# debbiemarkslab/BEAR

Hardware: AMD Instinct MI355X
Metric: k-mer contexts/sec (DM-marginal+grad h), k=13 (higher is better)
Workload: dtype f64

## Files before the change

bear_amd/csrc/bear_hip.hip:

```cpp
#include "bear_host.h"
#include "kernels_finalize.h"
#include "kernels_rows.h"
#include "kernels_sorted.h"
#include "kernels_plan.h"
#include "kernels_synth.h"
#include "kernels_refmix.h"
#include "kernels_mixplan.h"
#include "kernels_sample.h"
#include "kernels_shuffle.h"
#include "kernels_refplan.h"

#ifdef PLN_STAMPS
#define PLN_DBG_ARG , ws->dbg
#else
#define PLN_DBG_ARG
#endif

thread_local int g_last_hip_error = 0;

extern "C" {

int bear_abi_version(void) { return BEAR_ABI_VERSION; }

const char *bear_strerror(int status) {
  switch (status) {
    case BEAR_OK: return "ok";
    case BEAR_ERR_INVALID_ARG: return "invalid argument (null or misaligned pointer, bad flag)";
    case BEAR_ERR_NO_DEVICE: return "no usable HIP device";
    case BEAR_ERR_WRONG_DEVICE: return "current HIP device differs from the workspace device";
    case BEAR_ERR_HIP: return "HIP runtime call failed (see bear_last_hip_error)";
    case BEAR_ERR_NOMEM: return "out of memory";
    case BEAR_ERR_IO: return "file could not be opened or read";
    case BEAR_ERR_PARSE: return "malformed count-table row";
    default: return "unknown bear status";
  }
}

int bear_last_hip_error(void) { return g_last_hip_error; }

static int dm_kernels_setup() {
  int st = allow_dynamic_lds({BEAR_KFN(dm_prior_sorted_kernel<0>), BEAR_KFN(dm_prior_sorted_kernel<1>), BEAR_KFN(dm_prior_sorted_kernel<9>)},
                             sizeof(srt_lds_n));
  if (st == BEAR_OK) st = allow_dynamic_lds({BEAR_KFN(dm_ref_sorted_kernel)}, sizeof(srt_lds_r));
  if (st == BEAR_OK)
    st = allow_dynamic_lds({BEAR_KFN(dm_prior_plan_kernel<false, false>), BEAR_KFN(dm_prior_plan_kernel<true, false>),
                            BEAR_KFN(dm_prior_plan_kernel<true, true>)},
                           sizeof(pln_lds_n));
  if (st == BEAR_OK)
    st = allow_dynamic_lds({BEAR_KFN(dm_prior_plan_grad_kernel<false, false>), BEAR_KFN(dm_prior_plan_grad_kernel<true, true>),
                            BEAR_KFN(dm_refmix_plan_grad_kernel<false>), BEAR_KFN(dm_refmix_plan_grad_kernel<true>)},
                           sizeof(pln_lds_g));
  if (st == BEAR_OK) st = allow_dynamic_lds({BEAR_KFN(dm_prior_plan_grad_inplace_kernel)}, sizeof(pln_lds_gi));
  if (st == BEAR_OK) st = allow_dynamic_lds({BEAR_KFN(dm_ref_plan_kernel<false>), BEAR_KFN(dm_ref_plan_kernel<true>)}, sizeof(pln_lds_r));
  return st;
}

static void ws_release(bear_ws *ws) {
  (void)hipFree(ws->partials);
  (void)hipFree(ws->logtab);
  (void)hipFree(ws->dbg);
  (void)hipFree(ws->eval_partials);
  (void)hipFree(ws->eval_out);
  (void)hipFree(ws->lin_partials);
  (void)hipFree(ws->linw_partials);
  (void)hipFree(ws->linw_packed);
  (void)hipFree(ws->lin_accum);
  (void)hipFree(ws->cnn_partials);
  (void)hipFree(ws->cnnw_partials);
  (void)hipFree(ws->arrive);
  delete ws;
}

static int ws_setup(bear_ws *ws) {
  HIP_TRY(hipMalloc(&ws->partials, sizeof(double) * BEAR_MAX_OUT * (size_t)ws->max_blocks));
  HIP_TRY(hipMalloc(&ws->logtab, sizeof(double) * 2 * BEAR_LOGTAB_N));
  HIP_TRY(hipMalloc(&ws->dbg, sizeof(unsigned long long) * 48 * (size_t)ws->max_blocks));
  HIP_TRY(hipMalloc(&ws->arrive, sizeof(unsigned long long) * BEAR_ARRIVE_WORDS));
  HIP_TRY(hipMemset(ws->arrive, 0, sizeof(unsigned long long) * BEAR_ARRIVE_WORDS));
  double tab[2 * BEAR_LOGTAB_N];
  for (int i = 0; i < BEAR_LOGTAB_N; ++i) {
    const double r = 1.0 / ((BEAR_LOGTAB_N + i + 0.5) / (2.0 * BEAR_LOGTAB_N));
    tab[2 * i] = r;
    tab[2 * i + 1] = -log(r);
  }
  HIP_TRY(hipMemcpy(ws->logtab, tab, sizeof(tab), hipMemcpyHostToDevice));
  int st = dm_kernels_setup();
  if (st == BEAR_OK) st = linear_ws_setup(ws);
  if (st == BEAR_OK) st = cnn_ws_setup(ws);
  if (st == BEAR_OK) st = eval_ws_setup(ws);
  return st;
}

int bear_ws_create(int device, bear_ws **out) {
  if (!out) return BEAR_ERR_INVALID_ARG;
  *out = nullptr;
  int count = 0;
  if (hipGetDeviceCount(&count) != hipSuccess || count <= 0) return BEAR_ERR_NO_DEVICE;
  if (device < 0 || device >= count) return BEAR_ERR_INVALID_ARG;
  int prev = 0;
  HIP_TRY(hipGetDevice(&prev));
  HIP_TRY(hipSetDevice(device));
  hipDeviceProp_t prop;
  const hipError_t e = hipGetDeviceProperties(&prop, device);
  bear_ws *ws = e == hipSuccess ? new (std::nothrow) bear_ws() : nullptr;
  int st = ws ? BEAR_OK : BEAR_ERR_NOMEM;
  if (e != hipSuccess) {
    g_last_hip_error = (int)e;
    st = BEAR_ERR_HIP;
  }
  if (ws) {
    ws->device = device;
    ws->num_cu = prop.multiProcessorCount;
    ws->max_blocks = ws->num_cu * 8;
    ws->eval_blocks = ws->num_cu * 8;
    st = ws_setup(ws);
    if (st != BEAR_OK) {
      ws_release(ws);
      ws = nullptr;
    }
  }
  (void)hipSetDevice(prev);
  *out = ws;
  return st;
}

int bear_ws_destroy(bear_ws *ws) {
  if (!ws) return BEAR_OK;
  int prev = 0;
  (void)hipGetDevice(&prev);
  (void)hipSetDevice(ws->device);
  ws_release(ws);
  (void)hipSetDevice(prev);
  return BEAR_OK;
}

int bear_deterministic_build(void) {
#ifdef BEAR_DET_BUILD
  return 1;
#else
  return 0;
#endif
}

static int grid_rows(const bear_ws *ws, uint64_t n_rows) { return grid_capped((n_rows + BEAR_TILE_ROWS - 1) / BEAR_TILE_ROWS, ws_blocks(ws, 2)); }
static int grid_sorted(const bear_ws *ws, uint64_t n_rows) { return grid_capped((n_rows + SRT_TILE - 1) / SRT_TILE, ws_blocks(ws, 2)); }
static int grid_dense(const bear_ws *ws, uint64_t n_rows) {
  return grid_capped((n_rows + DPR_TILE_ROWS - 1) / DPR_TILE_ROWS, ws_blocks(ws, DPR_BLOCKS_PER_CU));
}

int bear_dm_prior_f64(bear_ws *ws, const uint32_t *counts, const double *prior, uint64_t n_rows,
                      double h_signed, double eps, int train_ar, double *out, double *grad_prior,
                      void *stream) {
  int st = check_ws(ws);
  if (st != BEAR_OK) return st;
  if (!out || (n_rows && (!counts || !prior))) return BEAR_ERR_INVALID_ARG;
  if (misaligned(counts) || misaligned(prior) || misaligned(grad_prior) || misaligned8(out)) return BEAR_ERR_INVALID_ARG;
  hipStream_t s = static_cast<hipStream_t>(stream);
  const bear_params prm = params_net(h_signed, eps);
  int grid = grid_rows(ws, n_rows);
  if (!train_ar && !grad_prior) {
    grid = grid_sorted(ws, n_rows);
    const char *dbg = getenv("BEAR_DEBUG_STOP");
    const int stop = dbg ? atoi(dbg) : 0;
    const double2 *lt = reinterpret_cast<const double2 *>(ws->logtab);
    if (stop == 1)
      hipLaunchKernelGGL(dm_prior_sorted_kernel<1>, dim3(grid), dim3(SRT_THREADS), sizeof(srt_lds_n), s, counts, prior, n_rows, prm, lt, ws->partials, ws->dbg);
    else if (stop == 9)
      hipLaunchKernelGGL(dm_prior_sorted_kernel<9>, dim3(grid), dim3(SRT_THREADS), sizeof(srt_lds_n), s, counts, prior, n_rows, prm, lt, ws->partials, ws->dbg);
    else
      hipLaunchKernelGGL(dm_prior_sorted_kernel<0>, dim3(grid), dim3(SRT_THREADS), sizeof(srt_lds_n), s, counts, prior, n_rows, prm, lt, ws->partials, ws->dbg);
  } else {
#define PRIOR_LAUNCH(AR, GRAD)                                                                                                          \
  hipLaunchKernelGGL((dm_prior_kernel<AR, GRAD>), dim3(grid), dim3(BEAR_THREADS), 0, s, counts, prior, n_rows, prm, grad_prior, \
                     reinterpret_cast<const double2 *>(ws->logtab), ws->partials)
    BEAR_DISPATCH_2(train_ar, grad_prior, PRIOR_LAUNCH);
#undef PRIOR_LAUNCH
  }
  HIP_TRY(hipGetLastError());
  hipLaunchKernelGGL(finalize_kernel, dim3(1), dim3(256), 0, s, ws->partials, grid, 2, out);
  HIP_TRY(hipGetLastError());
  return BEAR_OK;
}

int bear_dm_ref_f64(bear_ws *ws, const uint32_t *train, const uint32_t *ref, uint64_t n_rows,
                    double h_signed, double tau_signed, double nu_signed, double eps, int train_ar,
                    double *out, void *stream) {
  int st = check_ws(ws);
  if (st != BEAR_OK) return st;
  if (!out || (n_rows && (!train || !ref))) return BEAR_ERR_INVALID_ARG;
  if (misaligned(train) || misaligned(ref) || misaligned8(out)) return BEAR_ERR_INVALID_ARG;
  hipStream_t s = static_cast<hipStream_t>(stream);
  const bear_params prm = params_ref(h_signed, tau_signed, nu_signed, eps);
  const double2 *lt = reinterpret_cast<const double2 *>(ws->logtab);
  int grid = grid_rows(ws, n_rows);
  if (train_ar || getenv("BEAR_ROWS_KERNEL")) {
#define REF_LAUNCH(AR) hipLaunchKernelGGL((dm_ref_kernel<AR>), dim3(grid), dim3(BEAR_THREADS), 0, s, train, ref, n_rows, prm, lt, ws->partials)
    BEAR_DISPATCH_1(train_ar, REF_LAUNCH);
#undef REF_LAUNCH
  } else {
    grid = grid_sorted(ws, n_rows);
    hipLaunchKernelGGL(dm_ref_sorted_kernel, dim3(grid), dim3(SRT_THREADS), sizeof(srt_lds_r), s, train, ref, n_rows, prm, lt, ws->partials);
  }
  HIP_TRY(hipGetLastError());
  hipLaunchKernelGGL(finalize_kernel, dim3(1), dim3(256), 0, s, ws->partials, grid, 4, out);
  HIP_TRY(hipGetLastError());
  return BEAR_OK;
}

static void plan_free(bear_plan *p) {
  if (!p) return;
  (void)hipFree(p->tiles);
  (void)hipFree(p->stream);
  (void)hipFree(p->heavy_col);
  (void)hipFree(p->heavy_row);
  (void)hipFree(p->heavy_stop);
  (void)hipFree(p->hist);
  (void)hipFree(p->live);
  for (int k = 0; k < p->n_cnn_levels; ++k) bear_level_free(&p->cnn_levels[k]);
  for (int k = 0; k <= CNN_MAX_LAG; ++k)
    for (int q = 0; q < p->n_cnn_win[k]; ++q) bear_window_free(&p->cnn_win[k][q]);
  (void)hipFree(p->live2);
  (void)hipFree(p->tiles_p);
  (void)hipFree(p->tiles_u);
  (void)hipFree(p->ref_items);
  (void)hipFree(p->hist0_base);
  (void)hipFree(p->heavy0);
  (void)hipFree(p->sum0);
  delete p;
}

int bear_plan_create(bear_ws *ws, const uint32_t *counts, uint64_t n_rows, int ncol, bear_plan **out) {
  if (!out) return BEAR_ERR_INVALID_ARG;
  *out = nullptr;
  int st = check_ws(ws);
  if (st != BEAR_OK) return st;
  if ((ncol != 4 && ncol != 5) || (n_rows && !counts) || misaligned(counts)) return BEAR_ERR_INVALID_ARG;
  bear_plan *p = new (std::nothrow) bear_plan();
  if (!p) return BEAR_ERR_NOMEM;
  memset(p, 0, sizeof(*p));
  p->device = ws->device;
  p->ncol = ncol;
  p->n_rows = n_rows;
  p->counts = counts;
  hipError_t e = hipMalloc(&p->hist, sizeof(unsigned long long) * (2 * SRT_NKEY + PLN_NBIG + 1));
  if (e == hipSuccess) e = hipMemset(p->hist, 0, sizeof(unsigned long long) * (2 * SRT_NKEY + PLN_NBIG + 1));
  if (e != hipSuccess) {
    g_last_hip_error = (int)e;
    plan_free(p);
    return BEAR_ERR_HIP;
  }
  if (n_rows == 0) {
    *out = p;
    return BEAR_OK;
  }
  const uint64_t n_quads = (n_rows + PLN_QUAD - 1) / PLN_QUAD;
  uint8_t *d_quad = nullptr, *h_quad = nullptr;
  unsigned long long *d_cnt = nullptr;
  std::vector<pln_tile> tiles;
  e = hipMalloc(&d_quad, 3 * n_quads);
  if (e == hipSuccess) e = hipMalloc(&d_cnt, sizeof(unsigned long long) * 9);
  if (e == hipSuccess) e = hipMemset(d_cnt, 0, sizeof(unsigned long long) * 9);
  if (e == hipSuccess) {
    const int grid = grid_capped((n_quads + 255) / 256, (uint64_t)ws->num_cu * 8);
    hipLaunchKernelGGL(plan_scan_kernel, dim3(grid), dim3(256), 0, 0, counts, n_rows, ncol, d_quad, d_cnt, p->hist);
    e = hipGetLastError();
  }
  unsigned long long h_cnt[3] = {0, 0, 0}, h_total[3] = {0, 0, 0};
  if (e == hipSuccess) e = hipMemcpy(h_cnt, d_cnt, sizeof(h_cnt), hipMemcpyDeviceToHost);
  if (e == hipSuccess) e = hipMemcpy(h_total, d_cnt + 6, sizeof(h_total), hipMemcpyDeviceToHost);
  for (int k = 0; k < 3; ++k) p->count_total[k] = p->count_bound[k] = (double)h_total[k];
  uint64_t off16 = 0, n_tiles = 0;
  const char *cut_env = getenv("BEAR_PLAN_CUT");
  const bool host_cut = cut_env && cut_env[0] == 'h';
  if (e == hipSuccess && host_cut) {
    h_quad = (uint8_t *)malloc(3 * n_quads);
    if (!h_quad) e = hipErrorOutOfMemory;
    if (e == hipSuccess) e = hipMemcpy(h_quad, d_quad, 3 * n_quads, hipMemcpyDeviceToHost);
  }
  if (e == hipSuccess && host_cut) {
    uint64_t q = 0;
    while (q < n_quads) {
      uint32_t items = 0, rows = 0, hcol = 0, hrow = 0;
      const uint64_t q0 = q;
      while (q < n_quads && rows + PLN_QUAD <= PLN_RMAX && items + h_quad[q] <= PLN_NI_CUT) {
        items += h_quad[q];
        hcol += h_quad[n_quads + q];
        hrow += h_quad[2 * n_quads + q];
        rows += PLN_QUAD;
        ++q;
      }
      pln_tile ti;
      memset(&ti, 0, sizeof(ti));
      ti.row0 = q0 * PLN_QUAD;
      if (ti.row0 + rows > n_rows) rows = (uint32_t)(n_rows - ti.row0);
      const uint32_t hc = hcol < PLN_HCAP ? hcol : PLN_HCAP;
      const uint32_t hr = ncol == 5 ? (hrow < PLN_HCAP ? hrow : PLN_HCAP) : 0u;
      ti.rows_items = (rows << 16) | items;
      ti.off16 = (uint32_t)off16;
      ti.hc_hr = (hc << 16) | hr;
      ti.blk16 = pln_block_layout(rows, items, hc, hr).end / 16;
      off16 += ti.blk16;
      if (off16 > 0xffffffffull) {
        e = hipErrorOutOfMemory;
        break;
      }
      tiles.push_back(ti);
    }
    n_tiles = tiles.size();
  }
  free(h_quad);
  if (e == hipSuccess && !host_cut) {
    const uint32_t chunk = plan_cut_chunk(n_quads);
    const uint64_t n_chunks = (n_quads + chunk - 1) / chunk;
    uint32_t *d_walk = nullptr;
    uint16_t *d_step = nullptr;
    uint64_t *d_entry = nullptr;
    unsigned long long *d_meta = nullptr, h_meta[3] = {0, 0, 0};
    e = hipMalloc(&d_walk, sizeof(uint32_t) * n_chunks * PLN_CUT_SPAN);
    if (e == hipSuccess) e = hipMalloc(&d_step, sizeof(uint16_t) * n_quads);
    if (e == hipSuccess) e = hipMalloc(&d_entry, sizeof(uint64_t) * 2 * n_chunks);
    if (e == hipSuccess) e = hipMalloc(&d_meta, sizeof(h_meta));
    if (e == hipSuccess) e = hipMemset(d_meta, 0, sizeof(h_meta));
    if (e == hipSuccess) {
      const uint64_t wb = (n_chunks * PLN_CUT_SPAN + 255) / 256;
      hipLaunchKernelGGL(plan_cut_step_kernel, dim3((unsigned)((n_chunks + 255) / 256)), dim3(256), 0, 0, d_quad, n_quads, n_chunks, chunk, d_step);
      hipLaunchKernelGGL(plan_cut_walk_kernel, dim3((unsigned)wb), dim3(256), 0, 0, d_step, n_quads, n_chunks, chunk, d_walk);
      hipLaunchKernelGGL(plan_cut_chain_kernel, dim3(1), dim3(1), 0, 0, d_walk, n_chunks, chunk, d_entry, d_entry + n_chunks, d_meta);
      e = hipGetLastError();
    }
    if (e == hipSuccess) e = hipMemcpy(h_meta, d_meta, sizeof(unsigned long long), hipMemcpyDeviceToHost);
    n_tiles = h_meta[0];
    if (e == hipSuccess) e = hipMalloc(&p->tiles, sizeof(pln_tile) * (n_tiles + PLN_DESC_PAD));
    if (e == hipSuccess) e = hipMemset(p->tiles, 0, sizeof(pln_tile) * (n_tiles + PLN_DESC_PAD));
    if (e == hipSuccess) {
      hipLaunchKernelGGL(plan_cut_write_kernel, dim3((unsigned)((n_chunks + 255) / 256)), dim3(256), 0, 0, d_quad, n_quads, n_rows, ncol,
                         n_chunks, chunk, d_entry, d_entry + n_chunks, p->tiles);
      hipLaunchKernelGGL(plan_cut_offsets_kernel, dim3(1), dim3(1024), 0, 0, p->tiles, n_tiles, d_meta);
      e = hipGetLastError();
    }
    if (e == hipSuccess) e = hipMemcpy(h_meta, d_meta, sizeof(h_meta), hipMemcpyDeviceToHost);
    if (e == hipSuccess && h_meta[2]) e = hipErrorOutOfMemory;
    off16 = h_meta[1];
    (void)hipFree(d_walk);
    (void)hipFree(d_step);
    (void)hipFree(d_entry);
    (void)hipFree(d_meta);
  }
  (void)hipFree(d_quad);
  p->n_tiles = n_tiles;
  const uint64_t stream_bytes = off16 * 16 + 1024;
  for (int k = 0; k < 3; ++k) p->n_heavy[k] = h_cnt[k];
  if (host_cut) {
    if (e == hipSuccess) e = hipMalloc(&p->tiles, sizeof(pln_tile) * (tiles.size() + PLN_DESC_PAD));
    if (e == hipSuccess) e = hipMemset(p->tiles, 0, sizeof(pln_tile) * (tiles.size() + PLN_DESC_PAD));
    if (e == hipSuccess) e = hipMemcpy(p->tiles, tiles.data(), sizeof(pln_tile) * tiles.size(), hipMemcpyHostToDevice);
  }
  if (e == hipSuccess) e = hipMalloc(&p->stream, stream_bytes);
  if (e == hipSuccess) e = hipMemset(p->stream, 0, stream_bytes);
  if (e == hipSuccess && h_cnt[0]) e = hipMalloc(&p->heavy_col, sizeof(pln_heavy_col) * h_cnt[0]);
  if (e == hipSuccess && h_cnt[1]) e = hipMalloc(&p->heavy_row, sizeof(pln_heavy_row) * h_cnt[1]);
  if (e == hipSuccess && h_cnt[2]) e = hipMalloc(&p->heavy_stop, sizeof(uint64_t) * h_cnt[2]);
  if (e == hipSuccess) {
    const uint64_t nt = n_tiles;
    const int grid = grid_capped(nt, (uint64_t)ws->num_cu * 2);
    hipLaunchKernelGGL(plan_fill_kernel, dim3(grid), dim3(1024), 0, 0, counts, n_rows, ncol, p->tiles, nt, p->stream,
                       p->heavy_col, p->heavy_row, p->heavy_stop, d_cnt + 3);
    e = hipGetLastError();
  }
  const uint64_t live_bytes = ncol == 5 ? sizeof(uint16_t) * PLN_LIVE_STRIDE * (n_tiles + 1) : 0;
  if (e == hipSuccess && live_bytes) e = hipMalloc(&p->live, live_bytes);
  if (e == hipSuccess && live_bytes) e = hipMemset(p->live, 0, live_bytes);
  if (e == hipSuccess && live_bytes) {
    const uint64_t nt = n_tiles;
    const int grid = grid_capped(nt, (uint64_t)ws->num_cu * 2);
    hipLaunchKernelGGL(plan_live_kernel, dim3(grid), dim3(1024), 0, 0, p->tiles, nt, p->stream, p->live);
    e = hipGetLastError();
  }
  if (e == hipSuccess) e = hipDeviceSynchronize();
  unsigned long long h_used[3] = {0, 0, 0};
  if (e == hipSuccess) e = hipMemcpy(h_used, d_cnt + 3, sizeof(h_used), hipMemcpyDeviceToHost);
  for (int k = 0; k < 3; ++k) p->n_heavy[k] = h_used[k];
#ifdef BEAR_DET_BUILD
  const uint64_t sort_from = 2;
#else
  const uint64_t sort_from = 1u << 16;
#endif
  if (e == hipSuccess) {
    int cst = h_used[0] >= sort_from ? bear_canonical_order(p->heavy_col, h_used[0], 16, 0) : BEAR_OK;
    if (cst == BEAR_OK && h_used[1] >= sort_from) cst = bear_canonical_order(p->heavy_row, h_used[1], 16, 0);
    if (cst == BEAR_OK && h_used[2] >= sort_from) cst = bear_canonical_order(p->heavy_stop, h_used[2], 8, 0);
    if (cst != BEAR_OK) e = cst == BEAR_ERR_NOMEM ? hipErrorOutOfMemory : hipErrorUnknown;
  }
  p->n_live_rows = n_rows;
  if (e == hipSuccess && ncol == 5) {
    unsigned long long h_hist[SRT_NKEY];
    e = hipMemcpy(h_hist, p->hist, sizeof(h_hist), hipMemcpyDeviceToHost);
    unsigned long long live_rows = h_cnt[1];
    for (int k = 0; k < SRT_NKEY; ++k) live_rows += h_hist[k];
    p->n_live_rows = live_rows;
  }
  (void)hipFree(d_cnt);
  if (e != hipSuccess) {
    g_last_hip_error = (int)e;
    plan_free(p);
    return e == hipErrorOutOfMemory ? BEAR_ERR_NOMEM : BEAR_ERR_HIP;
  }
  p->bytes = stream_bytes + live_bytes + sizeof(pln_tile) * n_tiles + sizeof(pln_heavy_col) * h_cnt[0] +
             sizeof(pln_heavy_row) * h_cnt[1] + sizeof(uint64_t) * h_cnt[2];
  *out = p;
  return BEAR_OK;
}

int bear_plan_destroy(bear_plan *plan) {
  if (!plan) return BEAR_OK;
  int prev = 0;
  (void)hipGetDevice(&prev);
  (void)hipSetDevice(plan->device);
  plan_free(plan);
  (void)hipSetDevice(prev);
  return BEAR_OK;
}

uint64_t bear_plan_bytes(const bear_plan *plan) { return plan ? plan->bytes : 0; }

int bear_plan_create_auto(bear_ws *ws, const uint32_t *counts, uint64_t n_rows, int *rowwise, bear_plan **out) {
  if (rowwise) *rowwise = 0;
  int st = bear_plan_create(ws, counts, n_rows, 5, out);
  if (st != BEAR_OK) return st;
  bear_plan *p = *out;
  const double cells = p->count_total[1], listed = (double)p->n_heavy[0];
  if (!(cells > 0.0) || listed * 2.0 <= cells) return BEAR_OK;
  (void)hipFree(p->tiles);
  (void)hipFree(p->stream);
  (void)hipFree(p->heavy_col);
  (void)hipFree(p->heavy_row);
  (void)hipFree(p->heavy_stop);
  (void)hipFree(p->live);
  p->tiles = nullptr;
  p->stream = nullptr;
  p->heavy_col = nullptr;
  p->heavy_row = nullptr;
  p->heavy_stop = nullptr;
  p->live = nullptr;
  p->n_tiles = 0;
  p->n_heavy[0] = p->n_heavy[1] = p->n_heavy[2] = 0;
  p->ncol = PLAN_ROWS;
  p->bytes = sizeof(unsigned long long) * (2 * SRT_NKEY + PLN_NBIG + 1);
  if (rowwise) *rowwise = 1;
  return BEAR_OK;
}
static int launch_prior_rows(bear_ws *ws, const bear_plan *plan, const double *prior, const bear_params &prm, const double *theta,
                             int train_ar, double *out, double *grad_prior, hipStream_t s) {
  const int grid = grid_dense(ws, plan->n_rows);
  const double2 *lt = reinterpret_cast<const double2 *>(ws->logtab);
  const bear_step_io io = ws_io(ws, theta, BEAR_THETA_NET, out);
#define ROWS_LAUNCH(AR, GRAD) \
  hipLaunchKernelGGL((dm_prior_rows_kernel<AR, GRAD>), dim3(grid), dim3(BEAR_THREADS), 0, s, plan->counts, prior, plan->n_rows, prm, grad_prior, lt, \
                     ws->partials, io)
  BEAR_DISPATCH_2(train_ar, grad_prior, ROWS_LAUNCH);
#undef ROWS_LAUNCH
  HIP_TRY(hipGetLastError());
  return BEAR_OK;
}

uint64_t bear_plan_tile_count(const bear_plan *plan) { return plan ? plan->n_tiles : 0; }

int bear_plan_tile_info(const bear_plan *plan, uint64_t first, uint64_t count, uint64_t *row0, uint32_t *rows, uint32_t *items,
                        uint64_t *stream_offset) {
  if (!plan || first + count > plan->n_tiles || (count && (!row0 || !rows || !items || !stream_offset))) return BEAR_ERR_INVALID_ARG;
  if (!count) return BEAR_OK;
  std::vector<pln_tile> h(count);
  int prev = 0;
  (void)hipGetDevice(&prev);
  (void)hipSetDevice(plan->device);
  const hipError_t e = hipMemcpy(h.data(), plan->tiles + first, sizeof(pln_tile) * count, hipMemcpyDeviceToHost);
  (void)hipSetDevice(prev);
  if (e != hipSuccess) {
    g_last_hip_error = (int)e;
    return BEAR_ERR_HIP;
  }
  for (uint64_t k = 0; k < count; ++k) {
    row0[k] = h[k].row0;
    rows[k] = h[k].rows_items >> 16;
    items[k] = h[k].rows_items & 0xffffu;
    stream_offset[k] = (uint64_t)h[k].off16 * 16;
  }
  return BEAR_OK;
}

int bear_plan_create_ref(bear_ws *ws, const uint32_t *train, const uint32_t *ref, uint64_t n_rows, bear_plan **out) {
  if (!out) return BEAR_ERR_INVALID_ARG;
  *out = nullptr;
  if ((n_rows && !ref) || misaligned(ref)) return BEAR_ERR_INVALID_ARG;
  bear_plan *p = nullptr;
  int st = bear_plan_create(ws, train, n_rows, 4, &p);
  if (st != BEAR_OK) return st;
  p->ref = ref;
  if (p->count_total[1] > 0.0 && (double)p->n_heavy[0] * 2.0 > p->count_total[1]) {
    (void)hipFree(p->tiles);
    (void)hipFree(p->stream);
    (void)hipFree(p->heavy_col);
    (void)hipFree(p->heavy_row);
    (void)hipFree(p->heavy_stop);
    p->tiles = nullptr;
    p->stream = nullptr;
    p->heavy_col = nullptr;
    p->heavy_row = nullptr;
    p->heavy_stop = nullptr;
    p->n_tiles = 0;
    p->n_heavy[0] = p->n_heavy[1] = p->n_heavy[2] = 0;
    p->rows_ref = 1;
    p->bytes = sizeof(unsigned long long) * (2 * SRT_NKEY + PLN_NBIG + 1);
    *out = p;
    return BEAR_OK;
  }
  unsigned long long *d_meta = nullptr;
  hipError_t e = hipMalloc(&d_meta, sizeof(unsigned long long) * 72);
  if (e == hipSuccess) e = hipMemset(d_meta, 0, sizeof(unsigned long long) * 72);
  if (e == hipSuccess) e = hipMalloc(&p->sum0, sizeof(double));
  if (e == hipSuccess) e = hipMemset(p->sum0, 0, sizeof(double));
  p->hist0_base = d_meta;
  unsigned long long h_meta[72];
  memset(h_meta, 0, sizeof(h_meta));
  const int grid = grid_capped((n_rows + 1023) / 1024, (uint64_t)ws->num_cu * 8);
  if (e == hipSuccess && n_rows) {
    hipLaunchKernelGGL(rpl_build_kernel, dim3(grid), dim3(256), 0, 0, train, ref, n_rows, 0, d_meta, d_meta + 32, d_meta + 64, p->sum0,
                       static_cast<rpl_item *>(nullptr), static_cast<uint32_t *>(nullptr));
    e = hipGetLastError();
    if (e == hipSuccess) e = hipMemcpy(h_meta, d_meta, sizeof(h_meta), hipMemcpyDeviceToHost);
  }
  if (e == hipSuccess) {
    unsigned long long run = 0, cur[RPL_NKEY];
    for (int k = 0; k < RPL_NKEY; ++k) {
      cur[k] = run;
      run += h_meta[k];
    }
    p->n_ref_items = run;
    p->n_heavy0 = h_meta[64];
    if (run) e = hipMalloc(&p->ref_items, sizeof(rpl_item) * run);
    if (e == hipSuccess && p->n_heavy0) e = hipMalloc(&p->heavy0, sizeof(uint32_t) * p->n_heavy0);
    if (e == hipSuccess) e = hipMemcpy(d_meta, cur, sizeof(cur), hipMemcpyHostToDevice);
    if (e == hipSuccess) e = hipMemset(d_meta + 64, 0, sizeof(unsigned long long));
    if (e == hipSuccess && n_rows && (run || p->n_heavy0)) {
      hipLaunchKernelGGL(rpl_build_kernel, dim3(grid), dim3(256), 0, 0, train, ref, n_rows, 1, d_meta, d_meta + 32, d_meta + 64, p->sum0,
                         p->ref_items, p->heavy0);
      e = hipGetLastError();
    }
    if (e == hipSuccess) e = hipDeviceSynchronize();
#ifdef BEAR_DET_BUILD
    for (int k = 0; k < RPL_NKEY && e == hipSuccess; ++k)
      if (bear_canonical_order(p->ref_items + cur[k], h_meta[k], 16, 0) != BEAR_OK) e = hipErrorUnknown;
    if (e == hipSuccess && bear_canonical_order(p->heavy0, p->n_heavy0, 4, 0) != BEAR_OK) e = hipErrorUnknown;
#endif
  }
  if (e != hipSuccess) {
    g_last_hip_error = (int)e;
    plan_free(p);
    return e == hipErrorOutOfMemory ? BEAR_ERR_NOMEM : BEAR_ERR_HIP;
  }
  p->hist0 = d_meta + 32;
  p->bytes += sizeof(rpl_item) * p->n_ref_items + sizeof(uint32_t) * p->n_heavy0 + sizeof(unsigned long long) * 72;
  *out = p;
  return BEAR_OK;
}

static int launch_prior_plan(bear_ws *ws, const bear_plan *plan, const double *prior, uint64_t n_rows, const bear_params &prm,
                             const double *theta, int train_ar, int prior_normalized, double *out, hipStream_t s) {
  const int grid = grid_plan(ws, plan->n_tiles);
  const double2 *lt = reinterpret_cast<const double2 *>(ws->logtab);
  const bear_step_io io = ws_io(ws, theta, BEAR_THETA_NET, out);
  if (train_ar)
    hipLaunchKernelGGL((dm_prior_plan_kernel<true, true>), dim3(grid), dim3(PLN_THREADS), sizeof(pln_lds_n), s, prior, n_rows, prm,
                       plan_view(plan), lt, ws->partials, io PLN_DBG_ARG);
  else if (prior_normalized)
    hipLaunchKernelGGL((dm_prior_plan_kernel<true, false>), dim3(grid), dim3(PLN_THREADS), sizeof(pln_lds_n), s, prior, n_rows, prm,
                       plan_view(plan), lt, ws->partials, io PLN_DBG_ARG);
  else
    hipLaunchKernelGGL((dm_prior_plan_kernel<false, false>), dim3(grid), dim3(PLN_THREADS), sizeof(pln_lds_n), s, prior, n_rows, prm,
                       plan_view(plan), lt, ws->partials, io PLN_DBG_ARG);
  HIP_TRY(hipGetLastError());
  return BEAR_OK;
}

int bear_dm_prior_plan_f64(bear_ws *ws, const bear_plan *plan, const uint32_t *counts, const double *prior,
                           uint64_t n_rows, double h_signed, double eps, int train_ar, int prior_normalized,
                           double *out, void *stream) {
  int st = check_ws(ws);
  if (st != BEAR_OK) return st;
  if (!plan || !out || (n_rows && (!counts || !prior))) return BEAR_ERR_INVALID_ARG;
  if (check_plan_step(ws, plan, counts, n_rows, 5, true) != BEAR_OK || misaligned(prior) || misaligned8(out)) return BEAR_ERR_INVALID_ARG;
  const bear_params prm = params_net(h_signed, eps);
  if (plan_is_rows(plan)) return launch_prior_rows(ws, plan, prior, prm, nullptr, train_ar, out, nullptr, static_cast<hipStream_t>(stream));
  return launch_prior_plan(ws, plan, prior, n_rows, prm, nullptr, train_ar, prior_normalized, out, static_cast<hipStream_t>(stream));
}

int launch_prior_plan_grad(bear_ws *ws, const bear_plan *plan, const double *prior, const bear_params &prm,
                                  const double *theta, int train_ar, int prior_normalized, double *out, double *grad_prior,
                                  hipStream_t s) {
  const int grid = grid_plan(ws, plan->n_tiles);
  const double2 *lt = reinterpret_cast<const double2 *>(ws->logtab);
  const pln_view pv = plan_view(plan);
  const bear_step_io io = ws_io(ws, theta, BEAR_THETA_NET, out);
  if (train_ar)
    hipLaunchKernelGGL((dm_prior_plan_grad_kernel<true, true>), dim3(grid), dim3(PLN_THREADS), sizeof(pln_lds_g), s, prior, prm, pv, lt,
                       grad_prior, ws->partials, io);
  else if (prior_normalized)
    hipLaunchKernelGGL(dm_prior_plan_grad_inplace_kernel, dim3(grid), dim3(PLN_THREADS), sizeof(pln_lds_gi), s, prior, prm, pv, lt,
                       grad_prior, ws->partials, io);
  else
    hipLaunchKernelGGL((dm_prior_plan_grad_kernel<false, false>), dim3(grid), dim3(PLN_THREADS), sizeof(pln_lds_g), s, prior, prm, pv, lt,
                       grad_prior, ws->partials, io);
  HIP_TRY(hipGetLastError());
  auto fixup_grid = [&](uint64_t nh) { return grid_capped((nh + 255) / 256, (uint64_t)ws->num_cu * 8); };
#define FIXUP(NORM, AR, ROWS, N) \
  hipLaunchKernelGGL((dm_prior_grad_fixup_kernel<NORM, AR, ROWS>), dim3(fixup_grid(N)), dim3(256), 0, s, prior, prm, pv, lt, grad_prior, io)
  if (pv.n_heavy_row && !train_ar) {
    if (prior_normalized) FIXUP(true, false, true, pv.n_heavy_row);
    else FIXUP(false, false, true, pv.n_heavy_row);
  }
  if (pv.n_heavy_col) {
    if (train_ar) FIXUP(true, true, false, pv.n_heavy_col);
    else if (prior_normalized) FIXUP(true, false, false, pv.n_heavy_col);
    else FIXUP(false, false, false, pv.n_heavy_col);
  }
#undef FIXUP
  HIP_TRY(hipGetLastError());
  return BEAR_OK;
}

int bear_dm_prior_plan_grad_f64(bear_ws *ws, const bear_plan *plan, const uint32_t *counts, const double *prior,
                                uint64_t n_rows, double h_signed, double eps, int train_ar, int prior_normalized,
                                double *out, double *grad_prior, void *stream) {
  int st = check_ws(ws);
  if (st != BEAR_OK) return st;
  if (!plan || !out || !grad_prior || (n_rows && (!counts || !prior))) return BEAR_ERR_INVALID_ARG;
  if (check_plan_step(ws, plan, counts, n_rows, 5, true) != BEAR_OK) return BEAR_ERR_INVALID_ARG;
  if (misaligned(prior) || misaligned(grad_prior) || misaligned8(out)) return BEAR_ERR_INVALID_ARG;
  const bear_params prm = params_net(h_signed, eps);
  if (plan_is_rows(plan)) return launch_prior_rows(ws, plan, prior, prm, nullptr, train_ar, out, grad_prior, static_cast<hipStream_t>(stream));
  return launch_prior_plan_grad(ws, plan, prior, prm, nullptr, train_ar, prior_normalized, out, grad_prior,
                                static_cast<hipStream_t>(stream));
}

int bear_dm_prior_plan_dev_f64(bear_ws *ws, const bear_plan *plan, const uint32_t *counts, const double *prior, uint64_t n_rows,
                               const double *h_signed_dev, double eps, int train_ar, int prior_normalized, double *out,
                               double *grad_prior, void *stream) {
  int st = check_ws(ws);
  if (st != BEAR_OK) return st;
  if (!plan || !out || !h_signed_dev || (n_rows && (!counts || !prior))) return BEAR_ERR_INVALID_ARG;
  if (check_plan_step(ws, plan, counts, n_rows, 5, true) != BEAR_OK) return BEAR_ERR_INVALID_ARG;
  if (misaligned(prior) || misaligned(grad_prior) || misaligned8(out)) return BEAR_ERR_INVALID_ARG;
  hipStream_t s = static_cast<hipStream_t>(stream);
  const bear_params only_eps = params_eps(eps);
  if (plan_is_rows(plan)) return launch_prior_rows(ws, plan, prior, only_eps, h_signed_dev, train_ar, out, grad_prior, s);
  if (grad_prior) return launch_prior_plan_grad(ws, plan, prior, only_eps, h_signed_dev, train_ar, prior_normalized, out, grad_prior, s);
  return launch_prior_plan(ws, plan, prior, n_rows, only_eps, h_signed_dev, train_ar, prior_normalized, out, s);
}

int bear_dm_refmix_plan_grad_f64(bear_ws *ws, const bear_plan *plan, const uint32_t *counts, const double *net_rows,
                                 const double *ref_rows, uint64_t n_rows, const double *h_signed_dev, const double *tau_signed_dev,
                                 const double *net_weight_signed_dev, double eps, int train_ar, double *out, double *grad_net_rows,
                                 void *stream) {
  int st = check_ws(ws);
  if (st != BEAR_OK) return st;
  if (!plan || !out || !h_signed_dev || !tau_signed_dev || !net_weight_signed_dev) return BEAR_ERR_INVALID_ARG;
  if (n_rows && (!counts || !net_rows || !ref_rows || !grad_net_rows)) return BEAR_ERR_INVALID_ARG;
  if (check_plan_step(ws, plan, counts, n_rows, 5) != BEAR_OK) return BEAR_ERR_INVALID_ARG;
  if (misaligned(net_rows) || misaligned(ref_rows) || misaligned(grad_net_rows) || misaligned8(out) || misaligned8(h_signed_dev) ||
      misaligned8(tau_signed_dev) || misaligned8(net_weight_signed_dev) || !(eps >= 0.0))
    return BEAR_ERR_INVALID_ARG;
  hipStream_t s = static_cast<hipStream_t>(stream);
  const int grid = grid_plan(ws, plan->n_tiles);
  const double2 *lt = reinterpret_cast<const double2 *>(ws->logtab);
  const pln_view pv = plan_view(plan);
  const bear_step_io io = ws_io(ws, nullptr, BEAR_THETA_REF, out);
#define MIX_LAUNCH(AR)                                                                                                            \
  hipLaunchKernelGGL(dm_refmix_plan_grad_kernel<AR>, dim3(grid), dim3(PLN_THREADS), sizeof(pln_lds_g), s, net_rows, ref_rows, \
                     h_signed_dev, tau_signed_dev, net_weight_signed_dev, eps, pv, lt, grad_net_rows, ws->partials, io)
  BEAR_DISPATCH_1(train_ar, MIX_LAUNCH);
#undef MIX_LAUNCH
  HIP_TRY(hipGetLastError());
  if (pv.n_heavy_col + pv.n_heavy_row) {
    const uint64_t nh = pv.n_heavy_col + pv.n_heavy_row;
    const int g2 = grid_capped((nh + 255) / 256, (uint64_t)ws->num_cu * 4);
#define MIX_FIXUP(AR)                                                                                                      \
  hipLaunchKernelGGL(dm_refmix_fixup_kernel<AR>, dim3(g2), dim3(256), 0, s, net_rows, ref_rows, h_signed_dev, tau_signed_dev, \
                     net_weight_signed_dev, eps, pv, lt, grad_net_rows)
    BEAR_DISPATCH_1(train_ar, MIX_FIXUP);
#undef MIX_FIXUP
    HIP_TRY(hipGetLastError());
  }
  return BEAR_OK;
}


static int launch_ref_plan(bear_ws *ws, const bear_plan *plan, const uint32_t *ref, uint64_t n_rows, const bear_params &prm,
                           const double *theta, int train_ar, double *out, hipStream_t s, const bear_apply_io &apply = NO_APPLY) {
  const double2 *lt = reinterpret_cast<const double2 *>(ws->logtab);
  const bear_step_io io = ws_io(ws, theta, BEAR_THETA_REF, out);
  int grid;
  if (plan->rows_ref) {
    if (plan->ref != ref) return BEAR_ERR_INVALID_ARG;
    grid = grid_dense(ws, n_rows);
#define REF_ROWS(AR) \
  hipLaunchKernelGGL(dm_ref_rows_kernel<AR>, dim3(grid), dim3(BEAR_THREADS), 0, s, plan->counts, ref, n_rows, prm, lt, ws->partials, io, apply)
    BEAR_DISPATCH_1(train_ar, REF_ROWS);
#undef REF_ROWS
  } else if (plan->ref) {
    if (plan->ref != ref) return BEAR_ERR_INVALID_ARG;
    rpl_view rv;
    rv.items = plan->ref_items;
    rv.n_items = plan->n_ref_items;
    rv.hist0 = plan->hist0;
    rv.heavy0 = plan->heavy0;
    rv.n_heavy0 = plan->n_heavy0;
    rv.sum0 = plan->sum0;
    const uint64_t units = (plan->n_ref_items + 63) / 64, want = (units + 3) / 4 + 2, cap = (uint64_t)ws->num_cu * (units > 131072 ? 6 : 4);
    grid = grid_capped(want, cap);
#define REF_ITEMS(AR) \
  hipLaunchKernelGGL(dm_ref_items_kernel<AR>, dim3(grid), dim3(256), 0, s, prm, rv, plan_view(plan), lt, ws->partials, io, apply)
    BEAR_DISPATCH_1(train_ar, REF_ITEMS);
#undef REF_ITEMS
  } else {
    grid = grid_plan(ws, plan->n_tiles);
#define REF_PLAN(AR)                                                                                                                     \
  hipLaunchKernelGGL(dm_ref_plan_kernel<AR>, dim3(grid), dim3(PLN_THREADS), sizeof(pln_lds_r), s, ref, n_rows, prm, plan_view(plan), lt, \
                     ws->partials, io, apply)
    BEAR_DISPATCH_1(train_ar, REF_PLAN);
#undef REF_PLAN
  }
  HIP_TRY(hipGetLastError());
  return BEAR_OK;
}

int bear_dm_ref_plan_f64(bear_ws *ws, const bear_plan *plan, const uint32_t *train, const uint32_t *ref,
                         uint64_t n_rows, double h_signed, double tau_signed, double nu_signed, double eps,
                         int train_ar, double *out, void *stream) {
  int st = check_ws(ws);
  if (st != BEAR_OK) return st;
  if (!plan || !out || (n_rows && (!train || !ref))) return BEAR_ERR_INVALID_ARG;
  if (check_plan_step(ws, plan, train, n_rows, 4) != BEAR_OK || misaligned(ref) || misaligned8(out)) return BEAR_ERR_INVALID_ARG;
  return launch_ref_plan(ws, plan, ref, n_rows, params_ref(h_signed, tau_signed, nu_signed, eps), nullptr, train_ar, out,
                         static_cast<hipStream_t>(stream));
}

static int ref_reduce(bear_ws *ws, const bear_plan *plan, const uint32_t *train, const uint32_t *ref, uint64_t n_rows, const double *theta,
                      double eps, int train_ar, double *packed, hipStream_t s, const bear_apply_io &apply) {
  int st = check_ws(ws);
  if (st != BEAR_OK) return st;
  if (!plan || !packed || !theta || !n_rows || !train || !ref) return BEAR_ERR_INVALID_ARG;
  if (check_plan_step(ws, plan, train, n_rows, 4) != BEAR_OK || misaligned(ref) || misaligned8(packed)) return BEAR_ERR_INVALID_ARG;
  return launch_ref_plan(ws, plan, ref, n_rows, params_eps(eps), theta, train_ar, packed, s, apply);
}

int bear_ref_train_reduce_f64(bear_ws *ws, const bear_plan *plan, const uint32_t *train, const uint32_t *ref, uint64_t n_rows,
                              const double *theta, double eps, int train_ar, double *packed, void *stream) {
  return ref_reduce(ws, plan, train, ref, n_rows, theta, eps, train_ar, packed, static_cast<hipStream_t>(stream), NO_APPLY);
}

int bear_ref_train_step_f64(bear_ws *ws, const bear_plan *plan, const uint32_t *train, const uint32_t *ref, uint64_t n_rows,
                            double *theta, double *adam_m, double *adam_v, double *adam_t, double eps, int train_ar,
                            double learning_rate, double scale, double *out, double *loss_buf, uint64_t loss_cap, void *stream) {
  if (!adam_m || !adam_v || !adam_t) return BEAR_ERR_INVALID_ARG;
  hipStream_t s = static_cast<hipStream_t>(stream);
  if (two_launch_step()) {
    int st = ref_reduce(ws, plan, train, ref, n_rows, theta, eps, train_ar, out, s, NO_APPLY);
    if (st != BEAR_OK) return st;
    return launch_train_apply(theta, 3, out, adam_m, adam_v, adam_t, learning_rate, scale, train_ar, loss_buf, loss_cap, s);
  }
  return ref_reduce(ws, plan, train, ref, n_rows, theta, eps, train_ar, out, s,
                    make_apply(theta, 3, adam_m, adam_v, adam_t, learning_rate, scale, train_ar, loss_buf, loss_cap));
}

int bear_dm_items_f64(bear_ws *ws, const double *x, const uint32_t *c, uint64_t n, int path, double *D, double *P,
                      void *stream) {
  int st = check_ws(ws);
  if (st != BEAR_OK) return st;
  if (n == 0) return BEAR_OK;
  if (!x || !c || !D || !P || path < 0 || path > 2) return BEAR_ERR_INVALID_ARG;
  uint64_t blocks = (n + 255) / 256;
  if (blocks > 0x7fffffffull) return BEAR_ERR_INVALID_ARG;
  hipLaunchKernelGGL(dm_items_kernel, dim3((unsigned)blocks), dim3(256), 0, static_cast<hipStream_t>(stream), x, c, n, path,
                     reinterpret_cast<const double2 *>(ws->logtab), D, P);
  HIP_TRY(hipGetLastError());
  return BEAR_OK;
}

int bear_plan_count_total(const bear_plan *plan, double *total, double *bound) {
// ... 189 lines not shown
```

bear_amd/csrc/bear_host.h:

```cpp
#pragma once
#include <hip/hip_runtime.h>
#include <math.h>
#include <stdint.h>
#include <stdlib.h>
#include <string.h>

#include <initializer_list>
#include <new>
#include <vector>

#include "bear_common.h"
#include "bear_levels.h"
#include "plan_common.h"

#define BEAR_INTERNAL __attribute__((visibility("hidden")))

static inline int check_ws(const bear_ws *ws) {
  if (!ws) return BEAR_ERR_INVALID_ARG;
  int dev = -1;
  if (hipGetDevice(&dev) != hipSuccess) return BEAR_ERR_NO_DEVICE;
  if (dev != ws->device) return BEAR_ERR_WRONG_DEVICE;
  return BEAR_OK;
}

static inline bool misaligned(const void *p) { return (reinterpret_cast<uintptr_t>(p) & 15u) != 0; }
static inline bool misaligned8(const void *p) { return (reinterpret_cast<uintptr_t>(p) & 7u) != 0; }
static inline bool wide_width_ok(int width) { return width == 5 || width == 21; }

#define BEAR_DISPATCH_2(a, b, F) \
  do {                           \
    if (a) {                     \
      if (b) F(true, true);      \
      else F(true, false);       \
    } else {                     \
      if (b) F(false, true);     \
      else F(false, false);      \
    }                            \
  } while (0)

#define BEAR_DISPATCH_1(a, F) \
  do {                        \
    if (a) F(true);           \
    else F(false);            \
  } while (0)

static inline bear_params params_eps(double eps) {
  bear_params prm;
  memset(&prm, 0, sizeof(prm));
  prm.eps = eps;
  return prm;
}
static inline bear_params params_net(double h_signed, double eps) {
  bear_params prm = params_eps(eps);
  prm.inv_h = 1.0 / exp(h_signed);
  return prm;
}
static inline bear_params params_ref(double h_signed, double tau_signed, double nu_signed, double eps) {
  bear_params prm = params_net(h_signed, eps);
  const double tau = exp(tau_signed), nw = exp(nu_signed);
  prm.E = exp(-tau);
  prm.tauE = tau * prm.E;
  prm.tau = tau;
  prm.V = 1.0 / (nw + 1.0);
  prm.nw = nw;
  return prm;
}

static inline int grid_capped(uint64_t work, uint64_t cap) {
  const uint64_t g = work < cap ? work : cap;
  return g < 1 ? 1 : (int)g;
}
static inline uint64_t ws_blocks(const bear_ws *ws, int per_cu) {
  const uint64_t g = (uint64_t)ws->num_cu * per_cu;
  return g > (uint64_t)ws->max_blocks ? (uint64_t)ws->max_blocks : g;
}

static inline int grid_plan(const bear_ws *ws, uint64_t n_tiles) { return grid_capped(n_tiles, ws_blocks(ws, PLN_BLOCKS_PER_CU)); }

#define BEAR_KFN(...) reinterpret_cast<const void *>(__VA_ARGS__)
static inline int allow_dynamic_lds(std::initializer_list<const void *> kernels, size_t bytes) {
  for (const void *fn : kernels) HIP_TRY(hipFuncSetAttribute(fn, hipFuncAttributeMaxDynamicSharedMemorySize, (int)bytes));
  return BEAR_OK;
}

static inline bear_arrival ws_arrival(bear_ws *ws) {
  if (++ws->epoch == 0u) ws->epoch = 1u;
  return bear_arrival{ws->arrive, ws->epoch};
}

static inline bear_step_io ws_io(bear_ws *ws, const double *theta, int kind, double *out) {
  const bear_arrival a = ws_arrival(ws);
  bear_step_io io;
  io.theta = theta;
  io.kind = kind;
  io.epoch = a.epoch;
  io.out = out;
  io.arrive_word = a.word;
  return io;
}

static inline bool bear_deterministic() {
#ifdef BEAR_DET_BUILD
  return true;
#else
  const char *e = getenv("BEAR_AMD_DETERMINISTIC");
  return e && e[0] && e[0] != '0';
#endif
}

static const bear_apply_io NO_APPLY = {};

static inline bear_apply_io make_apply(double *theta, int n_theta, double *adam_m, double *adam_v, double *adam_t, double learning_rate,
                                       double scale, int train_ar, double *loss_buf, uint64_t loss_cap) {
  bear_apply_io A;
  A.theta = theta;
  A.m = adam_m;
  A.v = adam_v;
  A.t_state = adam_t;
  A.loss_buf = loss_buf;
  A.loss_cap = (unsigned long long)loss_cap;
  A.lr = learning_rate;
  A.scale = scale;
  A.n_theta = n_theta;
  A.train_ar = train_ar;
  return A;
}

static inline bool two_launch_step() {
  const char *e = getenv("BEAR_AMD_TWO_LAUNCH_STEP");
  return e && e[0] && e[0] != '0';
}

struct rpl_item;
struct bear_plan {
  int device;
  int ncol;
  uint64_t n_rows;
  const uint32_t *counts;
  pln_tile *tiles;
  unsigned char *stream;
  pln_heavy_col *heavy_col;
  pln_heavy_row *heavy_row;
  uint64_t *heavy_stop;
  unsigned long long *hist;
  uint16_t *live;
  uint64_t n_tiles;
  uint64_t n_heavy[3];
  int rows_ref;
  uint64_t n_live_rows;
  double count_total[3];
  double count_bound[3];
  uint64_t bytes;
  bear_level_dev cnn_levels[CNN_MAX_LAG];
  int n_cnn_levels, cnn_lag, cnn_fw;
  bear_window_dev cnn_win[CNN_MAX_LAG + 1][CNN_MAX_WIN];
  int n_cnn_win[CNN_MAX_LAG + 1];
  int n_cnn_windows;
  const uint64_t *cnn_codes;
  uint16_t *live2;
  pln_tile *tiles_p, *tiles_u;
  uint64_t n_tiles_p, n_tiles_u;
  const uint64_t *pair_codes;
  int pair_lag;
  const uint32_t *ref;
  rpl_item *ref_items;
  uint64_t n_ref_items, n_heavy0;
  unsigned long long *hist0;
  unsigned long long *hist0_base;
  uint32_t *heavy0;
  double *sum0;
};

static inline pln_view plan_view(const bear_plan *p) {
  pln_view v;
  v.tiles = p->tiles;
  v.stream = p->stream;
  v.heavy_col = p->heavy_col;
  v.heavy_row = p->heavy_row;
  v.heavy_stop = p->heavy_stop;
  v.hist = p->hist;
  v.hist_big = p->hist + 2 * SRT_NKEY;
  v.big_in_hist = 1;
  v.live = p->live;
  v.live2 = p->live2;
  v.subset = 0;
  v.n_tiles = p->n_tiles;
  v.n_heavy_col = p->n_heavy[0];
  v.n_heavy_row = p->n_heavy[1];
  v.n_heavy_stop = p->n_heavy[2];
  return v;
}

#define PLAN_ROWS 15
static inline bool plan_is_rows(const bear_plan *p) { return p->ncol == PLAN_ROWS; }
static inline int check_plan_step(const bear_ws *ws, const bear_plan *plan, const uint32_t *counts, uint64_t n_rows, int ncol,
                                  bool or_rows = false) {
  if (plan->ncol != ncol && !(or_rows && plan_is_rows(plan))) return BEAR_ERR_INVALID_ARG;
  if (plan->counts != counts || plan->n_rows != n_rows || plan->device != ws->device) return BEAR_ERR_INVALID_ARG;
  return BEAR_OK;
}

BEAR_INTERNAL int linear_ws_setup(bear_ws *ws);
BEAR_INTERNAL int cnn_ws_setup(bear_ws *ws);
BEAR_INTERNAL int eval_ws_setup(bear_ws *ws);

extern "C" {
BEAR_INTERNAL int launch_prior_plan_grad(bear_ws *ws, const bear_plan *plan, const double *prior, const bear_params &prm,
                                         const double *theta, int train_ar, int prior_normalized, double *out, double *grad_prior,
                                         hipStream_t s);
BEAR_INTERNAL int launch_train_apply(double *theta, int n_theta, const double *packed, double *adam_m, double *adam_v, double *adam_t,
                                     double learning_rate, double scale, int train_ar, double *loss_buf, uint64_t loss_cap, hipStream_t s);
}
```

bear_amd/csrc/kernels_plan.h:

```cpp
#pragma once
#include "plan_common.h"

__global__ __launch_bounds__(256) void plan_scan_kernel(const uint32_t *__restrict__ counts, uint64_t n_rows, int ncol,
                                                        uint8_t *__restrict__ quad_light,
                                                        unsigned long long *__restrict__ heavy_counts,
                                                        unsigned long long *__restrict__ hist) {
  __shared__ uint32_t s_heavy[3];
  __shared__ uint32_t s_hist[2 * SRT_NKEY];
  __shared__ uint32_t s_big[PLN_NBIG + 1];
  __shared__ unsigned long long s_total, s_cells;
  __shared__ uint32_t s_cmax;
  unsigned long long my_total = 0ull;
  uint32_t my_cells = 0u, my_cmax = 0u;
  if (threadIdx.x == 0) {
    s_total = s_cells = 0ull;
    s_cmax = 0u;
  }
  if (threadIdx.x < 3) s_heavy[threadIdx.x] = 0;
  if (threadIdx.x < 2 * SRT_NKEY) s_hist[threadIdx.x] = 0;
  for (uint32_t k = threadIdx.x; k <= PLN_NBIG; k += 256) s_big[k] = 0;
  __syncthreads();
  const uint64_t n_quads = (n_rows + PLN_QUAD - 1) / PLN_QUAD;
  for (uint64_t g = (uint64_t)blockIdx.x * 256 + threadIdx.x; g < n_quads; g += (uint64_t)gridDim.x * 256) {
    uint32_t light = 0, qhc = 0, qhr = 0;
    for (uint64_t r = PLN_QUAD * g; r < PLN_QUAD * g + PLN_QUAD && r < n_rows; ++r) {
      uint32_t nsat = 0, hcol = 0;
#pragma unroll
      for (int b = 0; b < 5; ++b) {
        const uint32_t c = counts[r * 5 + b];
        const uint32_t s = nsat + c;
        nsat = s < nsat ? 0xffffffffu : s;
        my_total += c;
        my_cells += c != 0u;
        my_cmax = c > my_cmax ? c : my_cmax;
        if (b < ncol) {
          light += (c != 0 && c <= SRT_CL);
          hcol += (c > SRT_CL);
        }
      }
      qhc += hcol;
      qhr += nsat > SRT_CL;
      if (hcol) atomicAdd(&s_heavy[0], hcol);
      if (nsat > SRT_CL) {
        atomicAdd(&s_heavy[1], 1u);
        if (nsat <= PLN_NBIG) atomicAdd(&s_big[nsat], 1u);
      } else if (nsat != 0) atomicAdd(&s_hist[nsat - 1], 1u);
      const uint32_t c4 = counts[r * 5 + 4];
      if (ncol == 4 && c4 > SRT_CL) atomicAdd(&s_heavy[2], 1u);
      else if (ncol == 4 && c4 != 0) atomicAdd(&s_hist[SRT_NKEY + c4 - 1], 1u);
    }
    quad_light[g] = (uint8_t)light;
    quad_light[n_quads + g] = (uint8_t)qhc;
    quad_light[2 * n_quads + g] = (uint8_t)qhr;
  }
  if (my_total) {
    atomicAdd(&s_total, my_total);
    atomicAdd(&s_cells, (unsigned long long)my_cells);
    atomicMax(&s_cmax, my_cmax);
  }
  __syncthreads();
  if (threadIdx.x == 0 && s_total) {
    atomicAdd(&heavy_counts[6], s_total);
    atomicAdd(&heavy_counts[7], s_cells);
    atomicMax(&heavy_counts[8], (unsigned long long)s_cmax);
  }
  if (threadIdx.x < 3 && s_heavy[threadIdx.x]) atomicAdd(&heavy_counts[threadIdx.x], (unsigned long long)s_heavy[threadIdx.x]);
  if (threadIdx.x < 2 * SRT_NKEY && s_hist[threadIdx.x]) atomicAdd(&hist[threadIdx.x], (unsigned long long)s_hist[threadIdx.x]);
  for (uint32_t k = threadIdx.x; k <= PLN_NBIG; k += 256)
    if (s_big[k]) atomicAdd(&hist[2 * SRT_NKEY + k], (unsigned long long)s_big[k]);
}

#define PLN_CUT_CHUNK_MAX 8192
static inline uint32_t plan_cut_chunk(uint64_t n_quads) { return n_quads <= 50000000ull ? 2048u : (uint32_t)PLN_CUT_CHUNK_MAX; }
#define PLN_CUT_SPAN (PLN_RMAX / PLN_QUAD)

__device__ __forceinline__ uint64_t plan_cut_one(const uint8_t *__restrict__ quad, uint64_t n_quads, uint64_t q0, uint32_t *items,
                                                 uint32_t *hcol, uint32_t *hrow) {
  uint32_t it = 0, hc = 0, hr = 0, rows = 0;
  uint64_t q = q0;
  while (q < n_quads && rows + PLN_QUAD <= PLN_RMAX && it + quad[q] <= PLN_NI_CUT) {
    it += quad[q];
    if (hcol) {
      hc += quad[n_quads + q];
      hr += quad[2 * n_quads + q];
    }
    rows += PLN_QUAD;
    ++q;
  }
  *items = it;
  if (hcol) {
    *hcol = hc;
    *hrow = hr;
  }
  return q;
}
__global__ __launch_bounds__(256) void plan_cut_step_kernel(const uint8_t *__restrict__ quad, uint64_t n_quads, uint64_t n_chunks,
                                                            uint32_t chunk, uint16_t *__restrict__ step) {
  const uint64_t k = (uint64_t)blockIdx.x * 256 + threadIdx.x;
  if (k >= n_chunks) return;
  const uint64_t q0 = k * chunk, q_end = q0 + chunk < n_quads ? q0 + chunk : n_quads;
  uint64_t r = q0;
  uint32_t items = 0;
  for (uint64_t q = q0; q < q_end; ++q) {
    if (r < q) {
      r = q;
      items = 0;
    }
    while (r < n_quads && (uint32_t)(r - q + 1) * PLN_QUAD <= PLN_RMAX && items + quad[r] <= PLN_NI_CUT) items += quad[r++];
    step[q] = (uint16_t)(r - q);
    items -= quad[q];
  }
}
__global__ __launch_bounds__(256) void plan_cut_walk_kernel(const uint16_t *__restrict__ step, uint64_t n_quads, uint64_t n_chunks,
                                                            uint32_t chunk, uint32_t *__restrict__ walk) {
  const uint64_t id = (uint64_t)blockIdx.x * 256 + threadIdx.x;
  if (id >= n_chunks * PLN_CUT_SPAN) return;
  const uint64_t k = id / PLN_CUT_SPAN, j = id - k * PLN_CUT_SPAN, end = (k + 1) * chunk;
  uint64_t q = k * chunk + j;
  uint32_t cnt = 0;
  while (q < end && q < n_quads) {
    q += step[q];
    ++cnt;
  }
  walk[id] = (uint32_t)(q >= end ? q - end : 0) | (cnt << 16);
}
static_assert(PLN_CUT_CHUNK_MAX < 65536 && PLN_CUT_SPAN < 65536 && PLN_CUT_SPAN <= 2048, "walk table: 16-bit fields; a tile is shorter than a chunk");
__global__ void plan_cut_chain_kernel(const uint32_t *__restrict__ walk, uint64_t n_chunks, uint32_t chunk, uint64_t *__restrict__ entry,
                                      uint64_t *__restrict__ base, unsigned long long *__restrict__ meta) {
  if (blockIdx.x || threadIdx.x) return;
  uint64_t j = 0, tiles = 0;
  for (uint64_t k = 0; k < n_chunks; ++k) {
    entry[k] = k * chunk + j;
    base[k] = tiles;
    const uint32_t w = walk[k * PLN_CUT_SPAN + j];
    tiles += w >> 16;
    j = w & 0xffffu;
  }
  meta[0] = tiles;
}
__global__ __launch_bounds__(256) void plan_cut_write_kernel(const uint8_t *__restrict__ quad, uint64_t n_quads, uint64_t n_rows, int ncol,
                                                             uint64_t n_chunks, uint32_t chunk, const uint64_t *__restrict__ entry,
                                                             const uint64_t *__restrict__ base, pln_tile *__restrict__ tiles) {
  const uint64_t k = (uint64_t)blockIdx.x * 256 + threadIdx.x;
  if (k >= n_chunks) return;
  const uint64_t end = (k + 1) * chunk;
  uint64_t q = entry[k], t = base[k];
  while (q < end && q < n_quads) {
    uint32_t items, hcol, hrow;
    const uint64_t q1 = plan_cut_one(quad, n_quads, q, &items, &hcol, &hrow);
    pln_tile ti;
    ti.row0 = q * PLN_QUAD;
    uint32_t rows = (uint32_t)(q1 - q) * PLN_QUAD;
    if (ti.row0 + rows > n_rows) rows = (uint32_t)(n_rows - ti.row0);
    const uint32_t hc = hcol < PLN_HCAP ? hcol : PLN_HCAP;
    const uint32_t hr = ncol == 5 ? (hrow < PLN_HCAP ? hrow : PLN_HCAP) : 0u;
    ti.rows_items = (rows << 16) | items;
    ti.off16 = 0;
    ti.hc_hr = (hc << 16) | hr;
    ti.blk16 = pln_block_layout(rows, items, hc, hr).end / 16;
    ti.pad = 0;
    tiles[t++] = ti;
    q = q1;
  }
}
__global__ __launch_bounds__(1024) void plan_cut_offsets_kernel(pln_tile *__restrict__ tiles, uint64_t n_tiles,
                                                                unsigned long long *__restrict__ meta) {
  __shared__ unsigned long long part[1024];
  const uint64_t per = (n_tiles + 1023) / 1024, lo = per * threadIdx.x, hi = lo + per < n_tiles ? lo + per : n_tiles;
  unsigned long long s = 0;
  for (uint64_t t = lo; t < hi; ++t) s += tiles[t].blk16;
  part[threadIdx.x] = s;
  __syncthreads();
  if (threadIdx.x == 0) {
    unsigned long long run = 0;
    for (int k = 0; k < 1024; ++k) {
      const unsigned long long v = part[k];
      part[k] = run;
      run += v;
    }
    meta[1] = run;
    meta[2] = run > 0xffffffffull ? 1ull : 0ull;
  }
  __syncthreads();
  unsigned long long off = part[threadIdx.x];
  for (uint64_t t = lo; t < hi; ++t) {
    tiles[t].off16 = (uint32_t)off;
    off += tiles[t].blk16;
  }
}

__global__ __launch_bounds__(1024) void plan_fill_kernel(const uint32_t *__restrict__ counts, uint64_t n_rows, int ncol,
                                                         const pln_tile *__restrict__ tiles, uint64_t n_tiles,
                                                         unsigned char *__restrict__ stream,
                                                         pln_heavy_col *__restrict__ heavy_col,
                                                         pln_heavy_row *__restrict__ heavy_row,
                                                         uint64_t *__restrict__ heavy_stop,
                                                         unsigned long long *__restrict__ cursors) {
  constexpr int RPT = (PLN_RMAX + 1023) / 1024;
  __shared__ uint32_t hist[SRT_NHIST];
  __shared__ uint32_t offs[SRT_NHIST];
  __shared__ uint32_t scan[16];
  __shared__ uint16_t sorted[PLN_NI + 64];
  __shared__ uint32_t s_hc, s_hr;
#ifdef BEAR_DET_BUILD
  __shared__ uint32_t comp[PLN_NI];
  static_assert((PLN_NI & (PLN_NI - 1)) == 0 && PLN_NI <= 2048, "bitonic sort over the tile's items: PLN_NI / 2 pairs, at most one per thread");
  __shared__ unsigned long long hkey[PLN_HCAP], htmp[PLN_HCAP];
#endif
  const uint32_t tid = threadIdx.x, rep = tid & (SRT_REP - 1);
  for (uint64_t t = blockIdx.x; t < n_tiles; t += gridDim.x) {
    const pln_tile ti = tiles[t];
    const uint32_t rows = ti.rows_items >> 16, n_light = ti.rows_items & 0xffffu;
    const uint32_t hc_cap = ti.hc_hr >> 16, hr_cap = ti.hc_hr & 0xffffu;
    const pln_layout L = pln_block_layout(rows, n_light, hc_cap, hr_cap);
    unsigned char *blk = stream + (size_t)ti.off16 * 16;
    uint16_t *E = reinterpret_cast<uint16_t *>(blk);
    uint8_t *nrow = blk + L.nrow;
    uint16_t *items = reinterpret_cast<uint16_t *>(blk + L.items);
    uint16_t *hoff = reinterpret_cast<uint16_t *>(blk + L.hoff);
    uint32_t *hcnt = reinterpret_cast<uint32_t *>(blk + L.hcnt);
    uint16_t *hrow = reinterpret_cast<uint16_t *>(blk + L.hrow);
    double *hn = reinterpret_cast<double *>(blk + L.hn);
    if (tid < SRT_NHIST) hist[tid] = 0;
    if (tid == 0) {
      s_hc = 0;
      s_hr = 0;
    }
    __syncthreads();
#ifdef BEAR_DET_BUILD
    uint32_t det_hc[RPT], det_hr[RPT];
    {
      uint32_t base_c = 0, base_r = 0;
#pragma unroll
      for (int k = 0; k < RPT; ++k) {
        const uint32_t lr = tid + 1024u * k;
        uint32_t nc = 0, nr = 0;
        if (lr < rows) {
          double n = 0.0;
          for (int b = 0; b < 5; ++b) {
            const uint32_t cv = counts[(ti.row0 + lr) * 5 + b];
            n += (double)cv;
            nc += (b < ncol && cv > SRT_CL) ? 1u : 0u;
          }
          nr = n > (double)SRT_CL ? 1u : 0u;
        }
        const uint32_t packed = nc | (nr << 16);
        const int lane = tid & 63, wave = tid >> 6;
        uint32_t incl = packed;
#pragma unroll
        for (int off = 1; off < 64; off <<= 1) {
          const uint32_t o = (uint32_t)__shfl_up((int)incl, off, 64);
          if (lane >= off) incl += o;
        }
        __syncthreads();
        if (lane == 63) scan[wave] = incl;
        __syncthreads();
        uint32_t before = 0, total = 0;
        for (int w = 0; w < 16; ++w) {
          if (w < wave) before += scan[w];
          total += scan[w];
        }
        const uint32_t excl = before + incl - packed;
        det_hc[k] = base_c + (excl & 0xffffu);
        det_hr[k] = base_r + (excl >> 16);
        base_c += total & 0xffffu;
        base_r += total >> 16;
      }
      __syncthreads();
      if (tid == 0) {
        s_hc = base_c;
        s_hr = base_r;
      }
    }
#endif
    uint32_t c[RPT][5], rank[RPT][5];
#pragma unroll
    for (int k = 0; k < RPT; ++k) {
      const uint32_t lr = tid + 1024u * k;
#pragma unroll
      for (int b = 0; b < 5; ++b) {
        c[k][b] = 0;
        rank[k][b] = 0;
      }
      if (lr < rows) {
        const uint64_t r = ti.row0 + lr;
        double n = 0.0;
#pragma unroll
        for (int b = 0; b < 5; ++b) {
          c[k][b] = counts[r * 5 + b];
          n += (double)c[k][b];
        }
        nrow[lr] = n < 1.0 ? (uint8_t)0 : (n <= (double)SRT_CL ? (uint8_t)n : (uint8_t)255);
        if (n > (double)SRT_CL) {
#ifdef BEAR_DET_BUILD
          const uint32_t k2 = hr_cap ? det_hr[k] : 0xffffffffu;
#else
          const uint32_t k2 = hr_cap ? atomicAdd(&s_hr, 1u) : 0xffffffffu;
#endif
          if (k2 < hr_cap) {
            hrow[k2] = (uint16_t)lr;
            hn[k2] = n;
          } else {
            const unsigned long long q = atomicAdd(&cursors[1], 1ull);
            heavy_row[q].row = r;
            heavy_row[q].n = n;
          }
        }
        if (ncol == 4 && c[k][4] > SRT_CL) heavy_stop[atomicAdd(&cursors[2], 1ull)] = c[k][4];
#pragma unroll
        for (int b = 0; b < 5; ++b) {
          if (b >= ncol) c[k][b] = 0;
          if (c[k][b] > SRT_CL) {
#ifdef BEAR_DET_BUILD
            const uint32_t k2 = hc_cap ? det_hc[k]++ : 0xffffffffu;
#else
            const uint32_t k2 = hc_cap ? atomicAdd(&s_hc, 1u) : 0xffffffffu;
#endif
            if (k2 < hc_cap) {
              hoff[k2] = (uint16_t)(lr * 5 + b);
              hcnt[k2] = c[k][b];
            } else {
              const unsigned long long q = atomicAdd(&cursors[0], 1ull);
              heavy_col[q].off = r * 5 + b;
              heavy_col[q].c = c[k][b];
            }
            c[k][b] = 0;
          }
          if (c[k][b] != 0) rank[k][b] = atomicAdd(&hist[(c[k][b] - 1) * SRT_REP + rep], 1u);
        }
      } else if (lr < ((rows + 15u) & ~15u)) {
        nrow[lr] = 0;
      }
    }
    __syncthreads();
    {
      const uint32_t v = tid < SRT_NHIST ? hist[tid] : 0u;
      const int lane = tid & 63, wave = tid >> 6;
      uint32_t incl = v;
#pragma unroll
      for (int off = 1; off < 64; off <<= 1) {
        uint32_t o = (uint32_t)__shfl_up((int)incl, off, 64);
        if (lane >= off) incl += o;
      }
      if (lane == 63) scan[wave] = incl;
      __syncthreads();
      uint32_t base = 0;
      for (int w = 0; w < wave; ++w) base += scan[w];
      if (tid < SRT_NHIST) offs[tid] = base + incl - v;
    }
    __syncthreads();
    if (tid < 30) E[tid] = (uint16_t)(tid < SRT_CL ? offs[tid * SRT_REP] : n_light);
    if (tid == 30) E[30] = (uint16_t)hc_cap;
    if (tid == 31) E[31] = (uint16_t)hr_cap;
#pragma unroll
    for (int k = 0; k < RPT; ++k)
#pragma unroll
      for (int b = 0; b < 5; ++b)
        if (c[k][b] != 0) sorted[offs[(c[k][b] - 1) * SRT_REP + rep] + rank[k][b]] = (uint16_t)((tid + 1024u * k) * 5 + b);
    __syncthreads();
#ifdef BEAR_DET_BUILD
    {
      for (uint32_t i = tid; i < PLN_NI; i += 1024) {
        uint32_t key = 0;
        for (uint32_t q = 1; q < SRT_CL; ++q) key += offs[q * SRT_REP] <= i ? 1u : 0u;
        comp[i] = i < n_light ? (key << 16) | sorted[i] : 0xffffffffu;
      }
      __syncthreads();
      for (uint32_t size = 2; size <= PLN_NI; size <<= 1)
        for (uint32_t stride = size >> 1; stride > 0; stride >>= 1) {
          const uint32_t lo = 2u * tid - (tid & (stride - 1u)), hi = lo + stride;
          if (tid < PLN_NI / 2) {
            const bool up = (lo & size) == 0u;
            const uint32_t a = comp[lo], bq = comp[hi];
            if ((a > bq) == up) {
              comp[lo] = bq;
              comp[hi] = a;
            }
          }
          __syncthreads();
        }
      for (uint32_t i = tid; i < n_light; i += 1024) sorted[i] = (uint16_t)(comp[i] & 0xffffu);
      __syncthreads();
      const uint32_t nhc = s_hc < hc_cap ? s_hc : hc_cap, nhr = s_hr < hr_cap ? s_hr : hr_cap;
      if (tid < nhc) hkey[tid] = ((unsigned long long)hoff[tid] << 32) | hcnt[tid];
      __syncthreads();
      if (tid < nhc) {
        uint32_t r = 0;
        for (uint32_t q = 0; q < nhc; ++q) r += hkey[q] < hkey[tid] ? 1u : 0u;
        htmp[r] = hkey[tid];
      }
      __syncthreads();
      if (tid < nhc) {
        hoff[tid] = (uint16_t)(htmp[tid] >> 32);
        hcnt[tid] = (uint32_t)htmp[tid];
      }
      __syncthreads();
      if (tid < nhr) hkey[tid] = ((unsigned long long)hrow[tid] << 48) | tid;
      if (tid < nhr) htmp[tid] = (unsigned long long)__double_as_longlong(hn[tid]);
      __syncthreads();
      uint32_t r = 0;
      unsigned long long mine = 0ull, myn = 0ull;
      if (tid < nhr) {
        for (uint32_t q = 0; q < nhr; ++q) r += hkey[q] < hkey[tid] ? 1u : 0u;
        mine = hkey[tid];
        myn = htmp[tid];
      }
      __syncthreads();
      if (tid < nhr) {
        hrow[r] = (uint16_t)(mine >> 48);
        hn[r] = __longlong_as_double((long long)myn);
      }
      __syncthreads();
    }
#endif
    const uint32_t padded = (n_light + 63u) & ~63u;
    for (uint32_t i = tid; i < padded; i += 1024) items[i] = i < n_light ? sorted[i] : (uint16_t)PLN_SENTINEL;
    __syncthreads();
  }
}

__global__ __launch_bounds__(1024) void plan_live_kernel(const pln_tile *__restrict__ tiles, uint64_t n_tiles,
                                                         const unsigned char *__restrict__ stream, uint16_t *__restrict__ live) {
  constexpr int RPT = (PLN_RMAX + 1023) / 1024;
  __shared__ uint32_t cnt[RPT * 16];
  const uint32_t tid = threadIdx.x, lane = tid & 63, wave = tid >> 6;
  for (uint64_t t = blockIdx.x; t < n_tiles; t += gridDim.x) {
    const pln_tile ti = tiles[t];
    const uint32_t rows = ti.rows_items >> 16;
    const uint8_t *nrow = stream + (size_t)ti.off16 * 16 + 64;
    uint16_t *out = live + t * PLN_LIVE_STRIDE;
    unsigned long long mask[RPT];
#pragma unroll
    for (int k = 0; k < RPT; ++k) {
      const uint32_t lr = tid + 1024u * k;
      mask[k] = __builtin_amdgcn_ballot_w64(lr < rows && nrow[lr] != 0);
      if (lane == 0) cnt[k * 16 + wave] = (uint32_t)__builtin_popcountll(mask[k]);
    }
    __syncthreads();
    uint32_t total = 0;
#pragma unroll
    for (int k = 0; k < RPT; ++k) {
      uint32_t base = total;
      for (int w = 0; w < 16; ++w) {
        const uint32_t c = cnt[k * 16 + w];
        if (w < (int)wave) base += c;
        total += c;
      }
      if ((mask[k] >> lane) & 1ull) out[1 + base + (uint32_t)__builtin_popcountll(mask[k] & ((1ull << lane) - 1ull))] = (uint16_t)(tid + 1024u * k);
    }
    if (tid == 0) out[0] = (uint16_t)total;
    __syncthreads();
  }
}

template <bool NORM, bool AR>
__global__ __launch_bounds__(PLN_THREADS, 4) void dm_prior_plan_kernel(const double *__restrict__ prior,
                                                                                    uint64_t n_rows, bear_params prm_arg,
                                                                                    pln_view pv,
                                                                                    const double2 *__restrict__ logtab_g,
                                                                                    double *__restrict__ partials,
                                                                                    const bear_step_io io
#ifdef PLN_STAMPS
                                                                                    , unsigned long long *__restrict__ dbg
#endif
                                                                                    ) {
  extern __shared__ __attribute__((aligned(16))) unsigned char srt_smem[];
  pln_lds_n &S = *reinterpret_cast<pln_lds_n *>(srt_smem);
  const bear_params prm = bear_params_of(prm_arg, io);
  const uint32_t tid = threadIdx.x, lane = tid & 63, wave = srt_uniform(tid >> 6);
  const double u = prm.inv_h, eps = prm.eps, eps5 = 5.0 * prm.eps;
  double acc[2] = {0.0, 0.0};

  if (tid < BEAR_LOGTAB_N) S.logtab[tid] = logtab_g[tid];
  if (tid < SRT_NKEY) {
    const bear_dp o = srt_general_fast(u + eps5, (double)(tid + 1), logtab_g);
    S.tabD[tid] = o.D;
    S.tabP[tid] = o.P;
  }
  if (tid < PLN_NBUF) {
    S.buf[tid].pri[PLN_SENTINEL] = 1.0;
    S.ticket[tid] = PLN_TICKET_START(PLN_WAVES - PLN_DMA_WAVES);
    S.sum_fail[tid] = 0xffffffffu;
  }

  const bool dma_wave = wave >= PLN_WAVES - PLN_DMA_WAVES;
  const uint32_t dw = wave - (PLN_WAVES - PLN_DMA_WAVES);
  constexpr bool GEN = !NORM && !AR;
  constexpr bool NT = GEN && PLN_GEN_NT;
  auto stage = [&](const pln_tile &ti, uint32_t b, bool with_nrow) {
    const uint32_t rows = ti.rows_items >> 16;
    if (rows == 0) return;
    const uint32_t pbytes = (rows * 40u) & ~15u, bbytes = ti.blk16 * 16u;
    const unsigned char *psrc = reinterpret_cast<const unsigned char *>(prior + ti.row0 * 5);
    const unsigned char *bsrc = pv.stream + (size_t)ti.off16 * 16;
    if (GEN && dw == 0 && lane == 0) S.nrow_in[b] = with_nrow ? 1u : 0u;
    if (!GEN || with_nrow) {
      for (uint32_t pc = dw; (pc << 10) < bbytes; pc += PLN_DMA_WAVES) pln_dma_piece<NT>(S.buf[b].blk, bsrc, bbytes, pc, lane);
    } else {
      const uint32_t items0 = pln_block_layout(rows, ti.rows_items & 0xffffu, ti.hc_hr >> 16, ti.hc_hr & 0xffffu).items;
      if (dw == PLN_DMA_WAVES - 1) pln_dma_piece<NT>(S.buf[b].blk, bsrc, 64u, 0u, lane);
      for (uint32_t pc = dw; (pc << 10) < bbytes - items0; pc += PLN_DMA_WAVES)
        pln_dma_piece<NT>(S.buf[b].blk + items0, bsrc + items0, bbytes - items0, pc, lane);
    }
    for (uint32_t pc = dw; (pc << 10) < pbytes; pc += PLN_DMA_WAVES) pln_dma_piece<NT>(S.buf[b].pri, psrc, pbytes, pc, lane);
    if (dw == 0 && ((rows * 40u) & 15u)) {
      const __attribute__((address_space(4))) double *tail =
          (const __attribute__((address_space(4))) double *)(uintptr_t)(prior + (ti.row0 + rows) * 5 - 1);
      const double v = *tail;
      if (lane == 0) S.buf[b].pri[rows * 5 - 1] = v;
    }
  };

  constexpr uint32_t PF_INSTR = (NORM || AR || PLN_GEN_PREFETCH) ? PLN_PREFETCH_KIB / 8u : 0u;
  auto prefetch_behind = [&](const pln_tile &ti) -> uint32_t {
    const uint32_t rows = ti.rows_items >> 16;
    if (PF_INSTR == 0 || rows == 0) return 0u;
    const uint64_t end_bytes = n_rows * 40ull, base = (ti.row0 + rows) * 40ull;
    const uint32_t m = srt_uniform((uint32_t)(uintptr_t)S.pf_scratch);
    uint32_t issued = 0;
    for (uint32_t k = dw; k < PF_INSTR; k += PLN_DMA_WAVES) {
      uint64_t off = base + ((uint64_t)(k * 64u + lane) << 7);
      if (off + 4u > end_bytes) off = end_bytes - 4u;
      const unsigned char *g = reinterpret_cast<const unsigned char *>(prior) + off;
      uint32_t keep_m0;
      asm volatile("s_mov_b32 %0, m0\n\ts_mov_b32 m0, %2\n\ts_nop 0\n\tglobal_load_lds_dword %1, off\n\ts_mov_b32 m0, %0"
                   : "=&s"(keep_m0)
                   : "v"(g), "s"(m)
                   : "memory");
      ++issued;
    }
    return issued;
  };
  uint32_t pf_young = 0;
#ifdef PLN_STAMPS
  unsigned long long tph[8] = {0, 0, 0, 0, 0, 0, 0, 0}, t_prev = __builtin_amdgcn_s_memtime();
  int prev_kind = 0;
#define PLN_STAMP(k)                                              \
  {                                                               \
    const unsigned long long now = __builtin_amdgcn_s_memtime();  \
    tph[k] += now - t_prev;                                       \
    t_prev = now;                                                 \
  }
#else
#define PLN_STAMP(k)
#endif
  static_assert(PLN_NBUF == 2, "the DMA-wave protocol below is written for a two-slot ring");
  const uint64_t G = gridDim.x;
  const uint64_t first = (pv.n_tiles * (uint64_t)blockIdx.x) / G, count = (pv.n_tiles * ((uint64_t)blockIdx.x + 1)) / G - first;
  auto fetch_desc = [&](uint64_t j0) {
    if (dw == 0 && j0 < count)
      pln_dma_piece(S.desc[(j0 >> 5) & 1u], pv.tiles + first + j0, PLN_DESC_CHUNK * (uint32_t)sizeof(pln_tile), 0u, lane);
  };
  if (dma_wave) {
    __builtin_amdgcn_s_setprio(3);
    fetch_desc(0);
    fetch_desc(PLN_DESC_CHUNK);
    srt_wait_dma();
  }
  __syncthreads();
  pln_tile cur = pln_desc(S.desc, 0, count), nxt = pln_desc(S.desc, 1, count);
  if (dma_wave) stage(cur, 0, !PLN_GEN_NROW_ON_DEMAND);
  uint32_t slot = 0;
  for (uint64_t j = 0; j < count; ++j) {
#ifdef PLN_STAMPS
    PLN_STAMP(prev_kind)
    prev_kind = 4;
#endif
    if (dma_wave) pln_wait_all_but(pf_young);
    PLN_STAMP(1)
    srt_sync();
    PLN_STAMP(2)
    const pln_tile nn = pln_desc(S.desc, j + 2, count);
    if (dma_wave) {
      if ((j & (PLN_DESC_CHUNK - 1)) == 0 && j != 0) fetch_desc(j + PLN_DESC_CHUNK);
      stage(nxt, slot ^ 1u, !GEN || !PLN_GEN_NROW_ON_DEMAND || srt_uniform(S.sum_fail[slot ^ 1u]) == (uint32_t)j);
      pf_young = prefetch_behind(nxt);
      cur = nxt;
      nxt = nn;
      slot ^= 1u;
      continue;
    }
    PLN_STAMP(3)

    const pln_buf_n &B = S.buf[slot];
    const uint32_t rows = cur.rows_items >> 16, n_light = cur.rows_items & 0xffffu;
    const uint32_t hc = cur.hc_hr >> 16, hr = cur.hc_hr & 0xffffu;
    const pln_layout L = pln_block_layout(rows, n_light, hc, hr);
    const uint16_t *E = reinterpret_cast<const uint16_t *>(B.blk);
    const uint8_t *nrow = B.blk + L.nrow;
    const uint16_t *items = reinterpret_cast<const uint16_t *>(B.blk + L.items);
    if (tid == 0) S.ticket[(slot + 1) % PLN_NBUF] = PLN_TICKET_START(PLN_WAVES - PLN_DMA_WAVES);
    const uint32_t n_hcu = (hc + 63u) >> 6, n_hru = AR ? 0u : (hr + 63u) >> 6, n_heavy = n_hcu + n_hru;
    const uint32_t n_units = (n_light + 63u) >> 6;
    const uint32_t n_work = n_heavy + n_units;
    static_assert(PLN_CHUNK == 128, "two adjacent contexts per lane");
    for (uint32_t c = wave; GEN && c * PLN_CHUNK < rows; c += PLN_WAVES - PLN_DMA_WAVES) {
      const uint32_t row0c = c * PLN_CHUNK + 2u * lane;
      const uint32_t rr = row0c < rows ? row0c : 0u;
      const double2 *src = reinterpret_cast<const double2 *>(&B.pri[rr * 5]);
      const double2 v0 = src[0], v1 = src[1], v2 = src[2], v3 = src[3], v4 = src[4];
      const double S5[2] = {((v0.x + v0.y) + (v1.x + v1.y)) + v2.x, ((v2.y + v3.x) + (v3.y + v4.x)) + v4.y};
      bool bad[2];
#pragma unroll
      for (int q = 0; q < 2; ++q) bad[q] = row0c + q < rows && !(__builtin_fabs(S5[q] - 1.0) <= SRT_SUM1_TOL);
      if (__builtin_amdgcn_ballot_w64(bad[0] || bad[1])) {
        if (lane == 0) S.sum_fail[slot] = (uint32_t)(j + 1);
        uint32_t nn_[2];
        if (!PLN_GEN_NROW_ON_DEMAND || srt_uniform(S.nrow_in[slot])) {
#pragma unroll
          for (int q = 0; q < 2; ++q) nn_[q] = bad[q] ? (uint32_t)nrow[rr + q] : 0u;
        } else {
          const uint8_t *g = pv.stream + (size_t)cur.off16 * 16 + L.nrow;
#pragma unroll
          for (int q = 0; q < 2; ++q) nn_[q] = bad[q] ? (uint32_t)g[rr + q] : 0u;
        }
#pragma unroll
        for (int q = 0; q < PLN_CHUNK / 64; ++q) {
          const uint32_t own = nn_[q] == 255u ? 0u : nn_[q];
          if (__builtin_amdgcn_ballot_w64(own != 0)) {
            uint32_t cm = own;
#pragma unroll
            for (int off = 32; off > 0; off >>= 1) {
              const uint32_t o2 = (uint32_t)__shfl_xor((int)cm, off, 64);
              cm = o2 > cm ? o2 : cm;
            }
            const double xa[1] = {own ? __builtin_fma(S5[q], u, eps5) : 1.0};
            const uint32_t ca[1] = {own};
            bear_dp o[1];
            srt_light<1>(xa, ca, 0u, srt_uniform(cm), S.logtab, o);
            if (own) {
              acc[0] += S.tabD[own - 1] - o[0].D;
              acc[1] = __builtin_fma(xa[0] - eps5, o[0].P, __builtin_fma(-u, S.tabP[own - 1], acc[1]));
            }
          }
        }
      }
    }
    PLN_FOR_UNITS_F(w, &S.ticket[slot], n_work, wave, PLN_WAVES - PLN_DMA_WAVES) {
#ifdef PLN_STAMPS
      {
        const unsigned long long now = __builtin_amdgcn_s_memtime();
        tph[prev_kind] += now - t_prev;
        t_prev = now;
        prev_kind = w < n_heavy ? 5 : 6;
      }
#endif
      if (w < n_hcu) {
        const uint32_t i = w * 64u + lane;
        if (i < hc) {
          const uint32_t off = reinterpret_cast<const uint16_t *>(B.blk + L.hoff)[i];
          const double cnt = (double)reinterpret_cast<const uint32_t *>(B.blk + L.hcnt)[i];
          if (AR) {
            acc[0] = __builtin_fma(cnt, bear_log_tab(B.pri[off] + eps, S.logtab), acc[0]);
          } else {
            const double x = __builtin_fma(B.pri[off], u, eps);
            const bear_dp o = srt_general_fast(x, cnt, S.logtab);
            acc[0] += o.D;
            acc[1] = __builtin_fma(eps - x, o.P, acc[1]);
          }
        }
        continue;
      }
      if (w < n_heavy) {
        const uint32_t i = (w - n_hcu) * 64u + lane;
        if (i < hr) {
          const double *f = &B.pri[(uint32_t)reinterpret_cast<const uint16_t *>(B.blk + L.hrow)[i] * 5u];
          const double A = NORM ? u + eps5 : __builtin_fma(((f[0] + f[1]) + (f[2] + f[3])) + f[4], u, eps5);
          const bear_dp o = srt_general_fast(A, reinterpret_cast<const double *>(B.blk + L.hn)[i], S.logtab);
          acc[0] -= o.D;
          acc[1] = __builtin_fma(A - eps5, o.P, acc[1]);
        }
        continue;
      }
      {
        const uint32_t un = n_heavy + n_units - 1u - w;
        uint32_t cmin, cmax;
        const uint32_t ci[1] = {pln_unit_counts(E, n_light, un, lane, &cmin, &cmax)};
        const uint32_t off = items[un * 64u + lane];
        if (AR) {
          acc[0] = __builtin_fma((double)ci[0], bear_log_tab(B.pri[off] + eps, S.logtab), acc[0]);
          continue;
        }
        const double x[1] = {__builtin_fma(B.pri[off], u, eps)};
        bear_dp o[1];
        srt_light<1>(x, ci, cmin, cmax, S.logtab, o);
        acc[0] += o[0].D;
        acc[1] = __builtin_fma(eps - x[0], o[0].P, acc[1]);
        continue;
      }
    }
    cur = nxt;
    nxt = nn;
    slot ^= 1u;
  }
  srt_wait_dma();
#ifdef PLN_STAMPS
  if (lane == 0 && dbg) {
    for (int k = 0; k < 8; ++k) dbg[((size_t)blockIdx.x * PLN_WAVES + wave) * 8 + k] = tph[k];
  }
#endif
  const uint64_t gtid = (uint64_t)blockIdx.x * PLN_THREADS + tid, gsz = (uint64_t)gridDim.x * PLN_THREADS;
  for (uint64_t i = gtid; i < pv.n_heavy_col; i += gsz) {
    const pln_heavy_col h = pv.heavy_col[i];
    if (AR) {
      acc[0] = __builtin_fma((double)h.c, bear_log_tab(prior[h.off] + eps, S.logtab), acc[0]);
      continue;
    }
    const double x = __builtin_fma(prior[h.off], u, eps);
    const bear_dp o = srt_general_fast(x, (double)h.c, S.logtab);
    acc[0] += o.D;
    acc[1] = __builtin_fma(eps - x, o.P, acc[1]);
  }
  for (uint64_t i = gtid; !AR && i < pv.n_heavy_row; i += gsz) {
    const pln_heavy_row h = pv.heavy_row[i];
    const double *f = prior + h.row * 5;
    const double A = __builtin_fma(((f[0] + f[1]) + (f[2] + f[3])) + f[4], u, eps5);
    const bear_dp o = srt_general_fast(A, h.n, S.logtab);
    acc[0] -= o.D;
    acc[1] = __builtin_fma(A - eps5, o.P, acc[1]);
  }
  if (!AR && blockIdx.x == 0 && tid < SRT_CL) {
    const double m = (double)pv.hist[tid];
    acc[0] -= m * S.tabD[tid];
    acc[1] = __builtin_fma(u * m, S.tabP[tid], acc[1]);
  }
  __syncthreads();
  block_finish<2>(acc, partials, io);
}

struct pln_buf_r {
  uint32_t ref[PLN_RMAX * 5 + 4];
  __attribute__((aligned(16))) unsigned char blk[PLN_BLOCK_MAX];
};
#define PLN_RSLOT 3
struct pln_lds_r {
  pln_buf_r buf[PLN_RSLOT];
  double2 logtab[BEAR_LOGTAB_N];
  double tabD[2][SRT_NKEY];
  double tabP[2][SRT_NKEY];
  uint32_t meta[PLN_RSLOT][2];
  uint32_t ticket[PLN_RSLOT];
  uint32_t landed[PLN_RSLOT];
  uint32_t left[PLN_RSLOT];
};

template <bool AR>
__global__ __launch_bounds__(PLN_THREADS, 4) void dm_ref_plan_kernel(const uint32_t *__restrict__ ref,
                                                                                  uint64_t n_rows, bear_params prm_arg,
                                                                                  pln_view pv,
                                                                                  const double2 *__restrict__ logtab_g,
                                                                                  double *__restrict__ partials,
                                                                                  const bear_step_io io, const bear_apply_io apply) {
  extern __shared__ __attribute__((aligned(16))) unsigned char srt_smem[];
// ... 555 lines not shown
```

bear_amd/kernels.py:

```python
import ctypes
import warnings

import numpy as np
import torch

from . import _lib

EPSILON = 1e-7


class _Handle:
    _destroy = None

    def _create(self, name, *args, after=()):
        h = ctypes.c_void_p()
        _lib.call(name, *args, ctypes.byref(h), *after)
        self._h = h

    def __del__(self):
        h, self._h = getattr(self, "_h", None), None
        if h:
            try:
                getattr(_lib.lib(), self._destroy)(h)
            except Exception:
                pass


class Workspace(_Handle):
    _destroy = "bear_ws_destroy"

    def __init__(self, device=None):
        if not torch.cuda.is_available():
            raise RuntimeError("bear_amd requires an MI355X (HIP) device; there is no CPU fallback")
        self.device = torch.device("cuda", torch.cuda.current_device() if device is None else torch.device(device).index or 0)
        self._create("bear_ws_create", self.device.index)

    @property
    def handle(self):
        return self._h


_default_ws = {}


def default_workspace(device, for_capture=False):
    idx = torch.device(device).index
    if idx is None:
        idx = torch.cuda.current_device()
    stream = torch.cuda.current_stream(idx)
    key = (idx, 0 if (for_capture or stream == torch.cuda.default_stream(idx) or torch.cuda.is_current_stream_capturing())
           else stream.cuda_stream)
    ws = _default_ws.get(key)
    if ws is None:
        ws = _default_ws[key] = Workspace(torch.device("cuda", idx))
    return ws


def _ptr(t):
    return ctypes.c_void_p(t.data_ptr()) if t is not None else ctypes.c_void_p(0)


def _stream():
    return ctypes.c_void_p(torch.cuda.current_stream().cuda_stream)


def _launch(device, name, *args):
    with torch.cuda.device(device):
        _lib.call(name, *args, _stream())


WIDE_WIDTHS = (5, 21)


def _check_rows(t, dtype, name, width=5, n=None, clone=True):
    if width is None and t.dim() == 2:
        width = t.shape[1]
    if not (t.is_cuda and t.dtype == dtype and t.dim() == 2 and t.shape[1] == width and t.is_contiguous()
            and (n is None or t.shape[0] == n)):
        raise ValueError(f"{name} must be a contiguous CUDA tensor of shape [{'N' if n is None else n}, {width or 'W'}] and dtype {dtype}")
    if width not in WIDE_WIDTHS:
        raise ValueError(f"{name}: rows of width {width}; the kernels take {WIDE_WIDTHS}")
    if t.data_ptr() % 16:
        if not clone:
            raise ValueError(f"{name} must be 16-byte aligned")
        t = t.clone()
    return t


def counts_dtype():
    return torch.int32


def dm_prior(counts, prior, h_signed, eps=EPSILON, train_ar=False, want_grad=False, out=None, ws=None):
    counts = _check_rows(counts, torch.int32, "counts")
    prior = _check_rows(prior, torch.float64, "prior")
    if counts.shape[0] != prior.shape[0]:
        raise ValueError("counts and prior must have the same number of rows")
    ws = ws or default_workspace(counts.device)
    if out is None:
        out = torch.empty(2, dtype=torch.float64, device=counts.device)
    grad = torch.empty_like(prior) if want_grad else None
    _launch(counts.device, "bear_dm_prior_f64", ws.handle, _ptr(counts), _ptr(prior), counts.shape[0], float(h_signed), float(eps),
            int(bool(train_ar)), _ptr(out), _ptr(grad))
    return out, grad


def dm_prior_wide(counts, prior, h_signed_dev, eps=EPSILON, train_ar=False, want_grad=False, out=None, ws=None):
    counts = _check_rows(counts, torch.int32, "counts", None)
    width = counts.shape[1]
    prior = _check_rows(prior, torch.float64, "prior", width)
    if counts.shape[0] != prior.shape[0]:
        raise ValueError("counts and prior must have the same number of rows")
    if h_signed_dev is not None:
        _f64_vec(h_signed_dev, 1, "h_signed_dev")
    elif not train_ar:
        raise ValueError("h_signed_dev is needed in BEAR mode")
    ws = ws or default_workspace(counts.device)
    if out is None:
        out = torch.empty(2, dtype=torch.float64, device=counts.device)
    grad = torch.empty_like(prior) if want_grad else None
    _launch(counts.device, "bear_dm_prior_wide_f64", ws.handle, _ptr(counts), _ptr(prior), counts.shape[0], width, _ptr(h_signed_dev),
            float(eps), int(bool(train_ar)), _ptr(out), _ptr(grad))
    return out, grad


REF_WIDE_TILE = {21: 256, 5: 512}
REFMIX_WIDE_TILE = {21: 128, 5: 512}
REF_WIDE_BLOCKS_PER_CU = 3
REFMIX_WIDE_BLOCKS_PER_CU = 3


def _check_ref_wide(train, ref):
    train = _check_rows(train, torch.int32, "train", None)
    ref = _check_rows(ref, torch.int32, "ref", train.shape[1])
    if train.shape[0] != ref.shape[0]:
        raise ValueError("train and ref must have the same number of rows")
    return train, ref


def dm_ref_wide(train, ref, h_signed, tau_signed, nu_signed, eps=EPSILON, train_ar=False, out=None, ws=None):
    train, ref = _check_ref_wide(train, ref)
    ws = ws or default_workspace(train.device)
    if out is None:
        out = torch.empty(4, dtype=torch.float64, device=train.device)
    _f64_vec(out, 4, "out")
    _launch(train.device, "bear_dm_ref_wide_f64", ws.handle, _ptr(train), _ptr(ref), train.shape[0], train.shape[1], float(h_signed),
            float(tau_signed), float(nu_signed), float(eps), int(bool(train_ar)), _ptr(out))
    return out


def ref_train_reduce_wide(train, ref, theta, packed, eps=EPSILON, train_ar=False, ws=None):
    train, ref = _check_ref_wide(train, ref)
    _f64_vec(theta, 3, "theta")
    _f64_vec(packed, 4, "packed")
    ws = ws or default_workspace(train.device)
    _launch(train.device, "bear_ref_train_reduce_wide_f64", ws.handle, _ptr(train), _ptr(ref), train.shape[0], train.shape[1], _ptr(theta),
            float(eps), int(bool(train_ar)), _ptr(packed))


def ref_train_step_wide(train, ref, theta, adam_m, adam_v, adam_t, learning_rate, scale, out, loss_buf=None, eps=EPSILON, train_ar=False,
                        ws=None):
    train, ref = _check_ref_wide(train, ref)
    for t, n, name in ((theta, 3, "theta"), (adam_m, 3, "adam_m"), (adam_v, 3, "adam_v"), (adam_t, 1, "adam_t"), (out, 4, "out")):
        _f64_vec(t, n, name)
    if loss_buf is not None:
        _f64_vec(loss_buf, loss_buf.numel(), "loss_buf")
    ws = ws or default_workspace(train.device)
    _launch(train.device, "bear_ref_train_step_wide_f64", ws.handle, _ptr(train), _ptr(ref), train.shape[0], train.shape[1], _ptr(theta),
            _ptr(adam_m), _ptr(adam_v), _ptr(adam_t), float(eps), int(bool(train_ar)), float(learning_rate), float(scale), _ptr(out),
            *_loss(loss_buf))


def dm_refmix_wide_dev(counts, net_rows, ref, h_signed_dev, tau_signed_dev, net_weight_signed_dev, eps=EPSILON, out=None, train_ar=False,
                       ws=None):
    counts, ref = _check_ref_wide(counts, ref)
    net_rows = _check_rows(net_rows, torch.float64, "net_rows", counts.shape[1])
    if net_rows.shape[0] != counts.shape[0]:
        raise ValueError("counts and net_rows must have the same number of rows")
    _check_scalar_param(h_signed_dev=h_signed_dev, tau_signed_dev=tau_signed_dev, net_weight_signed_dev=net_weight_signed_dev)
    ws = ws or default_workspace(counts.device)
    if out is None:
        out = torch.empty(4, dtype=torch.float64, device=counts.device)
    _f64_vec(out, 4, "out")
    grad = torch.empty_like(net_rows)
    _launch(counts.device, "bear_dm_refmix_wide_grad_f64", ws.handle, _ptr(counts), _ptr(net_rows), _ptr(ref), counts.shape[0],
            counts.shape[1], _ptr(h_signed_dev), _ptr(tau_signed_dev), _ptr(net_weight_signed_dev), float(eps), int(bool(train_ar)),
            _ptr(out), _ptr(grad))
    return out, grad


def dm_ref(train, ref, h_signed, tau_signed, nu_signed, eps=EPSILON, train_ar=False, out=None, ws=None):
    train = _check_rows(train, torch.int32, "train")
    ref = _check_rows(ref, torch.int32, "ref")
    if train.shape[0] != ref.shape[0]:
        raise ValueError("train and ref must have the same number of rows")
    ws = ws or default_workspace(train.device)
    if out is None:
        out = torch.empty(4, dtype=torch.float64, device=train.device)
    _launch(train.device, "bear_dm_ref_f64", ws.handle, _ptr(train), _ptr(ref), train.shape[0], float(h_signed), float(tau_signed),
            float(nu_signed), float(eps), int(bool(train_ar)), _ptr(out))
    return out


class Plan(_Handle):
    _destroy = "bear_plan_destroy"

    def __init__(self, counts, ncol, ws=None, ref=None, rows_if_dense=False):
        counts = _check_rows(counts, torch.int32, "counts")
        self.counts = counts
        self.ncol = int(ncol)
        self.ref = None
        self.rowwise = False
        self.ws = ws or default_workspace(counts.device)
        with torch.cuda.device(counts.device):
            torch.cuda.current_stream().synchronize()
            if ref is not None:
                if self.ncol != 4:
                    raise ValueError("a reference-aware plan needs ncol = 4")
                self.ref = ref = _check_rows(ref, torch.int32, "ref", n=counts.shape[0], clone=False)
                self._create("bear_plan_create_ref", self.ws.handle, _ptr(counts), _ptr(ref), counts.shape[0])
            elif rows_if_dense:
                if self.ncol != 5:
                    raise ValueError("rows_if_dense: five-column plans")
                rw = ctypes.c_int(0)
                self._create("bear_plan_create_auto", self.ws.handle, _ptr(counts), counts.shape[0], ctypes.byref(rw))
                self.rowwise = bool(rw.value)
            else:
                self._create("bear_plan_create", self.ws.handle, _ptr(counts), counts.shape[0], self.ncol)

    @property
    def nbytes(self):
        return int(_lib.lib().bear_plan_bytes(self._h))

    def _optional(self, name, *args):
        with torch.cuda.device(self.counts.device):
            st = getattr(_lib.lib(), name)(self._h, *args, _stream())
            if st == _lib.ERR_NOMEM:
                torch.cuda.empty_cache()
                st = getattr(_lib.lib(), name)(self._h, *args, _stream())
        if st != _lib.ERR_NOMEM:
            _lib.check(st, name)
        return st == 0

    def pair_contexts(self, kmer_index, lag):
        _check_codes(kmer_index)
        if kmer_index.shape[0] != self.counts.shape[0] or kmer_index.data_ptr() % 16:
            raise ValueError("kmer_index: one 16-byte aligned index word per row of the plan's count slab")
        ok = ctypes.c_int(0)
        if not self._optional("bear_plan_pair_contexts", _ptr(kmer_index), int(lag), ctypes.byref(ok)):
            warnings.warn("bear_plan_pair_contexts: out of device memory, the linear step keeps its plain lists")
            self.paired_codes = None
            return False
        self.paired_codes = kmer_index if ok.value else None
        return bool(ok.value)

    def count_total(self):
        a, b = (ctypes.c_double * 3)(), (ctypes.c_double * 3)()
        _lib.call("bear_plan_count_total", self._h, a, b)
        return list(a), list(b)

    def set_count_bound(self, bound):
        _lib.call("bear_plan_set_count_bound", self._h, (ctypes.c_double * 3)(*[float(x) for x in bound]))

    def pair_info(self):
        a, b = ctypes.c_uint64(0), ctypes.c_uint64(0)
        _lib.lib().bear_plan_pair_info(self._h, ctypes.byref(a), ctypes.byref(b))
        return int(a.value), int(b.value)

    def attach_cnn_levels(self, kmer_code, lag, filter_width):
        _check_codes(kmer_code)
        if kmer_code.shape[0] != self.counts.shape[0] or kmer_code.data_ptr() % 16:
            raise ValueError("kmer_code: one 16-byte aligned packed context per row of the plan's count slab")
        n = ctypes.c_int(0)
        if not self._optional("bear_plan_attach_cnn_levels", _ptr(kmer_code), int(lag), int(filter_width), ctypes.byref(n)):
            warnings.warn("bear_plan_attach_cnn_levels: out of device memory, the convolutional step runs without prefix levels")
            self.cnn_codes = None
            return 0
        self.cnn_codes = kmer_code if (n.value or self.cnn_window_rows()) else None
        return int(n.value)

    def cnn_window_rows(self):
        n = int(_lib.lib().bear_plan_cnn_window_rows(self._h, None, None, None, 0))
        if n <= 0:
            return []
        rows, pos, lev = (ctypes.c_uint64 * n)(), (ctypes.c_int * n)(), (ctypes.c_int * n)()
        _lib.lib().bear_plan_cnn_window_rows(self._h, rows, pos, lev, n)
        return [(int(lev[q]), int(pos[q]), int(rows[q])) for q in range(n)]

    def cnn_level_rows(self, with_letters=False):
        n = int(_lib.lib().bear_plan_cnn_level_rows(self._h, None, None, 0))
        if n <= 0:
            return ([], []) if with_letters else []
        rows, letters = (ctypes.c_uint64 * n)(), (ctypes.c_int * n)()
        _lib.lib().bear_plan_cnn_level_rows(self._h, rows, letters, n)
        return ([int(r) for r in rows], [int(x) for x in letters]) if with_letters else [int(r) for r in rows]

    def tiles(self):
        n = int(_lib.lib().bear_plan_tile_count(self._h))
        row0, rows, items, off = np.empty(n, np.uint64), np.empty(n, np.uint32), np.empty(n, np.uint32), np.empty(n, np.uint64)
        _lib.call("bear_plan_tile_info", self._h, 0, n, row0.ctypes.data, rows.ctypes.data, items.ctypes.data, off.ctypes.data)
        return row0, rows, items, off


def _check_planned(plan, ncol, rows, dtype, name):
    if plan.ncol != ncol:
        raise ValueError(f"a plan with ncol={ncol} is needed, this one has ncol={plan.ncol}")
    _check_rows(rows, dtype, name, n=plan.counts.shape[0], clone=False)


def dm_prior_planned(plan, prior, h_signed, eps=EPSILON, out=None, normalized=False, want_grad=False, train_ar=False):
    counts = plan.counts
    _check_planned(plan, 5, prior, torch.float64, "prior")
    if out is None:
        out = torch.empty(2, dtype=torch.float64, device=counts.device)
    if want_grad:
        grad = torch.empty_like(prior)
        _launch(counts.device, "bear_dm_prior_plan_grad_f64", plan.ws.handle, plan._h, _ptr(counts), _ptr(prior), counts.shape[0],
                float(h_signed), float(eps), int(bool(train_ar)), int(bool(normalized)), _ptr(out), _ptr(grad))
        return out, grad
    _launch(counts.device, "bear_dm_prior_plan_f64", plan.ws.handle, plan._h, _ptr(counts), _ptr(prior), counts.shape[0], float(h_signed),
            float(eps), int(bool(train_ar)), int(bool(normalized)), _ptr(out))
    return out


def dm_ref_planned(plan, ref, h_signed, tau_signed, nu_signed, eps=EPSILON, out=None, train_ar=False):
    train = plan.counts
    _check_planned(plan, 4, ref, torch.int32, "ref")
    if out is None:
        out = torch.empty(4, dtype=torch.float64, device=train.device)
    _launch(train.device, "bear_dm_ref_plan_f64", plan.ws.handle, plan._h, _ptr(train), _ptr(ref), train.shape[0], float(h_signed),
            float(tau_signed), float(nu_signed), float(eps), int(bool(train_ar)), _ptr(out))
    return out


def dm_items(x, c, path=0, ws=None):
    if not (x.is_cuda and x.dtype == torch.float64 and x.is_contiguous() and c.is_cuda and c.dtype == torch.int32
            and c.is_contiguous() and x.shape == c.shape and x.dim() == 1):
        raise ValueError("x: contiguous CUDA float64 [n]; c: contiguous CUDA int32 [n]")
    ws = ws or default_workspace(x.device)
    D, P = torch.empty_like(x), torch.empty_like(x)
    _launch(x.device, "bear_dm_items_f64", ws.handle, _ptr(x), _ptr(c), x.shape[0], int(path), _ptr(D), _ptr(P))
    return D, P


LINEAR_MAX_LAG = 21


def pack_kmers(codes):
    if not (codes.is_cuda and codes.dtype == torch.int8 and codes.dim() == 2 and codes.is_contiguous()):
        raise ValueError("codes must be a contiguous CUDA int8 tensor [n, lag]")
    out = torch.empty(codes.shape[0], dtype=torch.int64, device=codes.device)
    _launch(codes.device, "bear_pack_kmers_u64", _ptr(codes), codes.shape[0], codes.shape[1], _ptr(out))
    return out


def linear_index(kmer_code, lag):
    _check_codes(kmer_code)
    out = torch.empty_like(kmer_code)
    _launch(kmer_code.device, "bear_linear_index_u64", _ptr(kmer_code), kmer_code.shape[0], int(lag), _ptr(out))
    return out


def dm_linear(plan, kmer_index, mat, h_signed, eps=EPSILON, train_ar=False, out=None):
    n = plan.counts.shape[0]
    kmer_code = kmer_index
    if not (kmer_code.is_cuda and kmer_code.dtype == torch.int64 and kmer_code.dim() == 1 and kmer_code.is_contiguous()
            and kmer_code.shape[0] == n):
        raise ValueError("kmer_index must be a contiguous CUDA int64 tensor [n_rows] (linear_index)")
    if kmer_code.data_ptr() % 16:
        kmer_code = kmer_code.clone()
    if not (mat.is_cuda and mat.dtype == torch.float64 and mat.dim() == 3 and mat.shape[1:] == (5, 5) and mat.is_contiguous()):
        raise ValueError("mat must be a contiguous CUDA float64 tensor [lag, 5, 5]")
    if out is None:
        out = torch.empty(2, dtype=torch.float64, device=mat.device)
    grad = torch.empty_like(mat)
    _launch(mat.device, "bear_dm_linear_f64", plan.ws.handle, plan._h, _ptr(plan.counts), _ptr(kmer_code), _ptr(mat), mat.shape[0], n,
            float(h_signed), float(eps), int(bool(train_ar)), _ptr(out), _ptr(grad))
    return out, grad


def _host_f64(values):
    if values is None or not np.size(values):
        return np.zeros(0), ctypes.c_void_p(0)
    a = np.ascontiguousarray(np.atleast_1d(np.asarray(values, dtype=np.float64)))
    return a, a.ctypes.data_as(ctypes.c_void_p)


def _evaluate(wide, test, prior, h, van_reg, train, eps, with_ar, noise_seed, row_base, ws):
    test = _check_rows(test, torch.int32, "test", None if wide else 5)
    n, width = test.shape
    if train is not None:
        train = _check_rows(train, torch.int32, "train", width)
    if prior is not None:
        prior = _check_rows(prior, torch.float64, "prior", width)
    for t in (train, prior):
        if t is not None and t.shape[0] != n:
            raise ValueError("test, train and prior must have the same number of rows")
    (hs, hp), (vs, vp) = _host_f64(h), _host_f64(van_reg)
    ws = ws or default_workspace(test.device)
    out = torch.empty(2 * (hs.size + vs.size) + 3, dtype=torch.float64, device=test.device)
    _launch(test.device, "bear_eval_wide_f64" if wide else "bear_eval_f64", ws.handle, _ptr(test), _ptr(train), _ptr(prior), n,
            *((width,) if wide else ()), hp, hs.size, int(bool(with_ar)), vp, vs.size, float(eps), int(noise_seed), int(row_base), _ptr(out))
    return out


def evaluate(test, prior, h, van_reg, train=None, eps=EPSILON, with_ar=True, noise_seed=0, row_base=0, ws=None):
    return _evaluate(False, test, prior, h, van_reg, train, eps, with_ar, noise_seed, row_base, ws)


def evaluate_wide(test, prior, h, van_reg, train=None, eps=EPSILON, with_ar=True, noise_seed=0, row_base=0, ws=None):
    return _evaluate(True, test, prior, h, van_reg, train, eps, with_ar, noise_seed, row_base, ws)


class EvalPlan(_Handle):
    _destroy = "bear_eval_plan_destroy"

    def __init__(self, test, train=None, ws=None):
        test = _check_rows(test, torch.int32, "test")
        if train is not None:
            train = _check_rows(train, torch.int32, "train")
            if train.shape[0] != test.shape[0]:
                raise ValueError("test and train must have the same number of rows")
        self.test, self.train = test, train
        self.ws = ws or default_workspace(test.device)
        with torch.cuda.device(test.device):
            self._create("bear_eval_plan_create", self.ws.handle, _ptr(test), _ptr(train), test.shape[0], after=(_stream(),))

    @property
    def nbytes(self):
        return int(_lib.lib().bear_eval_plan_bytes(self._h))


def evaluate_planned(plan, prior, h, van_reg, eps=EPSILON, with_ar=True, noise_seed=0, row_base=0, row_ids=None):
    test, train = plan.test, plan.train
    n = test.shape[0]
    if row_ids is not None and not (row_ids.is_cuda and row_ids.dtype == torch.int32 and row_ids.is_contiguous()
                                    and row_ids.shape == (n,) and row_ids.data_ptr() % 16 == 0):
        raise ValueError("row_ids must be a contiguous, 16-byte aligned CUDA int32 tensor [n_rows]")
    if prior is not None:
        _check_rows(prior, torch.float64, "prior", n=n, clone=False)
    (hs, hp), (vs, vp) = _host_f64(h), _host_f64(van_reg)
    if vs.size and not (1750.0 * float(eps) < 0.5 and (vs >= 0.0).all() and (vs <= 2.0 ** 30).all()):
        raise ValueError("a planned evaluation decides the vanilla models' arg-max on the integer counts: it needs 1750 eps < 0.5 "
                         "and 0 <= van_reg <= 2^30 (kernels.evaluate takes any values)")
    out = torch.empty(2 * (hs.size + vs.size) + 3, dtype=torch.float64, device=test.device)
    _launch(test.device, "bear_eval_plan_f64", plan.ws.handle, plan._h, _ptr(test), _ptr(train), _ptr(prior), n, hp, hs.size,
            int(bool(with_ar)), vp, vs.size, float(eps), int(noise_seed), int(row_base), _ptr(row_ids), _ptr(out))
    return out


def bmm(counts, alpha, ws=None):
    counts = _check_rows(counts, torch.int32, "counts")
    al, ap = _host_f64(alpha)
    ws = ws or default_workspace(counts.device)
    out = torch.empty(al.size, dtype=torch.float64, device=counts.device)
    _launch(counts.device, "bear_bmm_f64", ws.handle, _ptr(counts), counts.shape[0], ap, al.size, _ptr(out))
    return out


def synth_counts(seed, row0, n_rows, device, dense=False, want=("train", "test", "ref")):
    bufs = {k: torch.empty((n_rows, 5), dtype=torch.int32, device=device) for k in want}
    _launch(device, "bear_synth_counts_u32", int(seed), int(row0), int(n_rows), int(bool(dense)), _ptr(bufs.get("train")),
            _ptr(bufs.get("test")), _ptr(bufs.get("ref")))
    return bufs


def synth_prior(seed, row0, n_rows, device):
    prior = torch.empty((n_rows, 5), dtype=torch.float64, device=device)
    _launch(device, "bear_synth_prior_f64", int(seed), int(row0), int(n_rows), _ptr(prior))
    return prior


def synth_kmer_ids(seed, row0, n_rows, lag, device):
    lag = int(lag)
    if not 1 <= lag <= 31:
        raise ValueError("synth_kmer_ids: 1 <= lag <= 31")
    bits = 2 * lag
    if row0 < 0 or row0 + n_rows > (1 << bits):
        raise ValueError(f"rows [{row0}, {row0 + n_rows}) of a table of distinct {lag}-mers: only 4^{lag} = {1 << bits} exist")
    mask = (1 << bits) - 1
    x = torch.arange(int(row0), int(row0) + int(n_rows), dtype=torch.int64, device=device)
    s = (int(seed) * 0x9E3779B97F4A7C15 + 0x632BE59BD9B4E019) & ((1 << 62) - 1)
    for r in range(4):
        mul = ((s >> (7 * r)) | 1) & mask | 1
        add = (s >> (5 * r + 3)) & mask
        x = (x * mul + add) & mask
        x = x ^ (x >> max(1, bits // 2 + (r & 1)))
    return x


def synth_kmer_codes(seed, row0, n_rows, lag, device, sort=False):
    ids = synth_kmer_ids(seed, row0, n_rows, lag, device)
    if sort:
        ids = torch.sort(ids).values
    shifts = torch.arange(2 * (int(lag) - 1), -1, -2, dtype=torch.int64, device=ids.device)
    return ((ids[:, None] >> shifts[None, :]) & 3).to(torch.int8).contiguous()


def log_gamma(conc, n_samples, seed):
    if not (conc.is_cuda and conc.dtype == torch.float64 and conc.dim() == 1 and conc.is_contiguous()):
        raise ValueError("conc must be a contiguous CUDA float64 vector")
    out = torch.empty((int(n_samples), conc.shape[0]), dtype=torch.float64, device=conc.device)
    _launch(conc.device, "bear_log_gamma_f64", _ptr(conc), conc.shape[0], int(n_samples), int(seed) & (2 ** 64 - 1), _ptr(out))
    return out


def _logdir_sample(wide, counts, prior, h, vans, mc_samples, get_map, with_ar, seed, row_base, n_rows, device, width):
    n = None
    if counts is not None:
        counts = _check_rows(counts, torch.int32, "counts", width)
        n, device, width = counts.shape[0], counts.device, counts.shape[1]
    if prior is not None:
        prior = _check_rows(prior, torch.float64, "prior", width)
        if n is not None and prior.shape[0] != n:
            raise ValueError("counts and prior must have the same number of rows")
        n, device, width = prior.shape[0], prior.device, prior.shape[1]
    if n is None:
        if width not in WIDE_WIDTHS:
            raise ValueError(f"width {width}: the wide kernels take {WIDE_WIDTHS}")
        n, device = int(n_rows), torch.device(device or "cuda")
    (hs, hp), (vs, vp) = _host_f64(h), _host_f64(vans)
    mc = 1 if get_map else int(mc_samples)
    M = int(bool(with_ar)) + hs.size + vs.size
    out = torch.empty((n, width, M, mc), dtype=torch.float64, device=device)
    _launch(device, "bear_logdir_sample_wide_f64" if wide else "bear_logdir_sample_f64", _ptr(counts), _ptr(prior), n,
            *((int(width),) if wide else ()), hp, hs.size, int(bool(with_ar)), vp, vs.size, mc, int(bool(get_map)),
            int(seed) & (2 ** 64 - 1), int(row_base), _ptr(out))
    return out


def logdir_sample(counts, prior, h, vans, mc_samples, get_map=False, with_ar=False, seed=0, row_base=0, n_rows=None,
                  device=None):
    return _logdir_sample(False, counts, prior, h, vans, mc_samples, get_map, with_ar, seed, row_base, n_rows, device, 5)


def logdir_sample_wide(counts, prior, h, vans, mc_samples, get_map=False, with_ar=False, seed=0, row_base=0, n_rows=None,
                       device=None, width=None):
    return _logdir_sample(True, counts, prior, h, vans, mc_samples, get_map, with_ar, seed, row_base, n_rows, device, width)


def shuffle_rows(src, seed):
    if not (src.is_cuda and src.is_contiguous() and src.dim() >= 1):
        raise ValueError("src must be a contiguous CUDA tensor")
    dst = torch.empty_like(src)
    n = src.shape[0]
    row_bytes = src.element_size() * (src.numel() // n) if n else 0
    _launch(src.device, "bear_shuffle_rows", _ptr(src), _ptr(dst), n, row_bytes, int(seed) & (2 ** 64 - 1))
    return dst


def kmer_order(kmer_code, lag):
    _check_codes(kmer_code)
    n = kmer_code.shape[0]
    perm = torch.empty(n, dtype=torch.int32, device=kmer_code.device)
    nbytes = ctypes.c_uint64(kmer_order_scratch_bytes(n, lag))
    scratch = torch.empty(max(int(nbytes.value), 1), dtype=torch.uint8, device=kmer_code.device)
    _launch(kmer_code.device, "bear_kmer_order_u64", _ptr(kmer_code), n, int(lag), _ptr(perm), _ptr(scratch), ctypes.byref(nbytes))
    return perm


def kmer_order_scratch_bytes(n_rows, lag):
    nbytes = ctypes.c_uint64(0)
    _lib.call("bear_kmer_order_u64", None, int(n_rows), int(lag), None, None, ctypes.byref(nbytes), None)
    return int(nbytes.value)


def gather_rows(src, perm):
    if not (src.is_cuda and src.is_contiguous() and src.dim() >= 1 and perm.is_cuda and perm.dtype == torch.int32
            and perm.is_contiguous() and perm.shape == (src.shape[0],)):
        raise ValueError("src: contiguous CUDA tensor; perm: contiguous CUDA int32 [n_rows]")
    dst = torch.empty_like(src)
    n = src.shape[0]
    row_bytes = src.element_size() * (src.numel() // n) if n else 1
    _launch(src.device, "bear_gather_rows", _ptr(src), _ptr(perm), _ptr(dst), n, row_bytes)
    return dst


def shuffle_source_row(i, n_rows, seed):
    return int(_lib.lib().bear_shuffle_source_row(int(i), int(n_rows), int(seed) & (2 ** 64 - 1)))


CNN_NUM_FILTERS, CNN_LAYER1_WIDTH, CNN_MAX_LAG = 30, 16, 21


CNN_WIDE_MAX_LAG = 16


def cnn_supported(lag, alphabet_size, filter_width, num_filters, kmer_layer1_width):
    if not (num_filters == CNN_NUM_FILTERS and kmer_layer1_width == CNN_LAYER1_WIDTH):
        return False
    if alphabet_size == 20:
        return 1 <= filter_width <= lag <= CNN_WIDE_MAX_LAG
    return alphabet_size == 4 and 1 <= filter_width <= lag <= CNN_MAX_LAG


def _count(name, *args):
    n = getattr(_lib.lib(), name)(*args)
    _lib.check(min(n, 0), name)
    return n


def cnn_param_count(lag, filter_width):
    return _count("bear_cnn_param_count", int(lag), int(filter_width), CNN_NUM_FILTERS, CNN_LAYER1_WIDTH)


# ... 383 lines not shown
```

include/bear_hip.h:

```cpp
#ifndef BEAR_HIP_H
#define BEAR_HIP_H

#include <stdint.h>

#ifdef __cplusplus
extern "C" {
#endif

#define BEAR_ABI_VERSION 12
#define BEAR_ROW_WIDTH 5

typedef enum bear_status {
  BEAR_OK = 0,
  BEAR_ERR_INVALID_ARG = -1,
  BEAR_ERR_NO_DEVICE = -2,
  BEAR_ERR_WRONG_DEVICE = -3,
  BEAR_ERR_HIP = -4,
  BEAR_ERR_NOMEM = -5,
  BEAR_ERR_IO = -6,
  BEAR_ERR_PARSE = -7
} bear_status;

typedef struct bear_ws bear_ws;

int bear_abi_version(void);
const char *bear_strerror(int status);
int bear_last_hip_error(void);

int bear_ws_create(int device, bear_ws **out);
int bear_ws_destroy(bear_ws *ws);

int bear_dm_prior_f64(bear_ws *ws, const uint32_t *counts, const double *prior, uint64_t n_rows,
                      double h_signed, double eps, int train_ar, double *out, double *grad_prior,
                      void *stream);

int bear_dm_ref_f64(bear_ws *ws, const uint32_t *train, const uint32_t *ref, uint64_t n_rows,
                    double h_signed, double tau_signed, double nu_signed, double eps, int train_ar,
                    double *out, void *stream);

typedef struct bear_plan bear_plan;
int bear_plan_create(bear_ws *ws, const uint32_t *counts, uint64_t n_rows, int ncol, bear_plan **out);
int bear_plan_create_auto(bear_ws *ws, const uint32_t *counts, uint64_t n_rows, int *rowwise, bear_plan **out);
int bear_plan_destroy(bear_plan *plan);
uint64_t bear_plan_bytes(const bear_plan *plan);
uint64_t bear_plan_tile_count(const bear_plan *plan);
int bear_plan_tile_info(const bear_plan *plan, uint64_t first, uint64_t count, uint64_t *row0, uint32_t *rows, uint32_t *items,
                        uint64_t *stream_offset);
int bear_plan_create_ref(bear_ws *ws, const uint32_t *train, const uint32_t *ref, uint64_t n_rows, bear_plan **out);
int bear_dm_prior_plan_f64(bear_ws *ws, const bear_plan *plan, const uint32_t *counts, const double *prior,
                           uint64_t n_rows, double h_signed, double eps, int train_ar, int prior_normalized,
                           double *out, void *stream);
int bear_dm_prior_plan_grad_f64(bear_ws *ws, const bear_plan *plan, const uint32_t *counts, const double *prior,
                                uint64_t n_rows, double h_signed, double eps, int train_ar, int prior_normalized,
                                double *out, double *grad_prior, void *stream);
int bear_dm_ref_plan_f64(bear_ws *ws, const bear_plan *plan, const uint32_t *train, const uint32_t *ref,
                         uint64_t n_rows, double h_signed, double tau_signed, double nu_signed, double eps,
                         int train_ar, double *out, void *stream);

int bear_dm_prior_plan_dev_f64(bear_ws *ws, const bear_plan *plan, const uint32_t *counts, const double *prior, uint64_t n_rows,
                               const double *h_signed_dev, double eps, int train_ar, int prior_normalized, double *out,
                               double *grad_prior, void *stream);

int bear_plan_attach_cnn_levels(bear_plan *plan, const uint64_t *kmer_code, int lag, int filter_width, int *n_levels, void *stream);
int bear_plan_cnn_level_rows(const bear_plan *plan, uint64_t *rows_out, int *letters_out, int capacity);
int bear_plan_cnn_window_rows(const bear_plan *plan, uint64_t *rows_out, int *pos_out, int *level_out, int capacity);
int bear_cnn_forward_plan_f64(bear_ws *ws, const bear_plan *plan, const uint64_t *kmer_code, uint64_t n_rows, int lag, int filter_width,
                              int num_filters, int layer1_width, const double *params, double *prior, double *t1_save, void *stream);
int bear_train_apply_f64(double *theta, int n_theta, const double *packed, double *adam_m, double *adam_v, double *adam_t,
                         double learning_rate, double scale, int train_ar, double *loss_buf, uint64_t loss_cap, void *stream);
int bear_ref_train_reduce_f64(bear_ws *ws, const bear_plan *plan, const uint32_t *train, const uint32_t *ref, uint64_t n_rows,
                              const double *theta, double eps, int train_ar, double *packed, void *stream);
int bear_net_linear_train_reduce_f64(bear_ws *ws, const bear_plan *plan, const uint32_t *counts, const uint64_t *kmer_index, int lag,
                                     uint64_t n_rows, const double *theta, double eps, int train_ar, double *packed, void *stream);
int bear_cnn_reserve(bear_ws *ws, uint64_t n_rows, int lag, int filter_width, int num_filters, int layer1_width);
int bear_net_cnn_train_reduce_f64(bear_ws *ws, const bear_plan *plan, const uint32_t *counts, const uint64_t *kmer_code, uint64_t n_rows,
                                  int lag, int filter_width, int num_filters, int layer1_width, const double *theta, double *prior_buf,
                                  double *t1_buf, double *grad_rows_buf, double eps, int train_ar, double *packed, void *stream);
int bear_ref_train_step_f64(bear_ws *ws, const bear_plan *plan, const uint32_t *train, const uint32_t *ref, uint64_t n_rows,
                            double *theta, double *adam_m, double *adam_v, double *adam_t, double eps, int train_ar,
                            double learning_rate, double scale, double *out, double *loss_buf, uint64_t loss_cap, void *stream);
int bear_net_linear_train_step_f64(bear_ws *ws, const bear_plan *plan, const uint32_t *counts, const uint64_t *kmer_index, int lag,
                                   uint64_t n_rows, double *theta, double *adam_m, double *adam_v, double *adam_t, double *packed,
                                   double eps, int train_ar, double learning_rate, double scale, double *loss_buf,
                                   uint64_t loss_cap, void *stream);
int bear_net_cnn_train_step_f64(bear_ws *ws, const bear_plan *plan, const uint32_t *counts, const uint64_t *kmer_code, uint64_t n_rows,
                                int lag, int filter_width, int num_filters, int layer1_width, double *theta, double *adam_m,
                                double *adam_v, double *adam_t, double *prior_buf, double *t1_buf, double *grad_rows_buf,
                                double *packed, double eps, int train_ar, double learning_rate, double scale, double *loss_buf,
                                uint64_t loss_cap, void *stream);

int bear_pack_kmers_u64(const int8_t *codes, uint64_t n_rows, int lag, uint64_t *packed, void *stream);
int bear_linear_index_u64(const uint64_t *kmer_code, uint64_t n_rows, int lag, uint64_t *kmer_index, void *stream);
int bear_encode_kmers_i8(const uint8_t *ascii, uint64_t n_rows, int lag, int rna, int8_t *codes, void *stream);
int bear_dm_linear_f64(bear_ws *ws, const bear_plan *plan, const uint32_t *counts, const uint64_t *kmer_index,
                       const double *mat, int lag, uint64_t n_rows, double h_signed, double eps, int train_ar,
                       double *out, double *grad_mat, void *stream);
int bear_plan_pair_contexts(bear_plan *plan, const uint64_t *kmer_index, int lag, int *paired, void *stream);
int bear_plan_count_total(const bear_plan *plan, double *total, double *bound);
int bear_deterministic_build(void);
int bear_plan_set_count_bound(bear_plan *plan, const double *bound);
int bear_plan_pair_info(const bear_plan *plan, uint64_t *paired_tiles, uint64_t *plain_tiles);

int bear_linear_forward_f64(bear_ws *ws, const uint64_t *kmer_code, uint64_t n_rows, int lag, const double *mat, double *prior,
                            void *stream);
int bear_linear_backward_f64(bear_ws *ws, const uint64_t *kmer_code, uint64_t n_rows, int lag, const double *prior,
                             const double *grad_prior, double *grad_mat, void *stream);

#define LINEAR_WIDE_MAX_LAG 16
int bear_linear_forward_wide_f64(bear_ws *ws, const int8_t *codes, uint64_t n_rows, int lag, int width, const double *mat,
                                 double *prior, void *stream);
int bear_linear_backward_wide_f64(bear_ws *ws, const int8_t *codes, uint64_t n_rows, int lag, int width, const double *prior,
                                  const double *grad_prior, double *grad_mat, void *stream);

int bear_dm_linear_wide_f64(bear_ws *ws, const uint32_t *counts, const int8_t *codes, uint64_t n_rows, int lag, int width,
                            const double *mat, double h_signed, double eps, int train_ar, double *out, double *grad_mat, void *stream);
int bear_net_linear_train_reduce_wide_f64(bear_ws *ws, const uint32_t *counts, const int8_t *codes, uint64_t n_rows, int lag, int width,
                                          const double *theta, double eps, int train_ar, double *packed, void *stream);
int bear_net_linear_train_step_wide_f64(bear_ws *ws, const uint32_t *counts, const int8_t *codes, uint64_t n_rows, int lag, int width,
                                        double *theta, double *adam_m, double *adam_v, double *adam_t, double eps, int train_ar,
                                        double learning_rate, double scale, double *packed, double *loss_buf, uint64_t loss_cap,
                                        void *stream);

int bear_ref_mix_forward_f64(bear_ws *ws, const double *net_rows, const double *ref_rows, uint64_t n_rows, const double *tau_signed,
                             const double *net_weight_signed, double *prior, void *stream);
int bear_ref_mix_backward_f64(bear_ws *ws, const double *net_rows, const double *ref_rows, const double *grad_prior, uint64_t n_rows,
                              const double *tau_signed, const double *net_weight_signed, double *grad_net_rows, double *grad_scalars,
                              void *stream);

int bear_dm_refmix_plan_grad_f64(bear_ws *ws, const bear_plan *plan, const uint32_t *counts, const double *net_rows,
                                 const double *ref_rows, uint64_t n_rows, const double *h_signed_dev, const double *tau_signed_dev,
                                 const double *net_weight_signed_dev, double eps, int train_ar, double *out, double *grad_net_rows,
                                 void *stream);

int bear_cnn_param_count(int lag, int filter_width, int num_filters, int layer1_width);
int bear_cnn_forward_f64(bear_ws *ws, const uint64_t *kmer_code, uint64_t n_rows, int lag, int filter_width, int num_filters,
                         int layer1_width, const double *params, double *prior, double *t1_save, void *stream);
int bear_cnn_backward_f64(bear_ws *ws, const uint64_t *kmer_code, uint64_t n_rows, int lag, int filter_width, int num_filters,
                          int layer1_width, const double *params, const double *t1_save, const double *prior,
                          const double *grad_prior, double *grad_params, void *stream);

#define CNN_WIDE_MAX_LAG 16
int bear_cnn_param_count_wide(int lag, int filter_width, int num_filters, int layer1_width, int width);
int bear_cnn_forward_wide_f64(bear_ws *ws, const int8_t *codes, uint64_t n_rows, int lag, int filter_width, int num_filters,
                              int layer1_width, int width, const double *params, double *prior, double *t1_save, void *stream);
int bear_cnn_backward_wide_f64(bear_ws *ws, const int8_t *codes, uint64_t n_rows, int lag, int filter_width, int num_filters,
                               int layer1_width, int width, const double *params, const double *t1_save, const double *prior,
                               const double *grad_prior, double *grad_params, void *stream);

int bear_eval_f64(bear_ws *ws, const uint32_t *test, const uint32_t *train, const double *prior, uint64_t n_rows,
                  const double *h, int n_h, int with_ar, const double *van_reg, int n_van, double eps,
                  uint64_t noise_seed, uint64_t row_base, double *out, void *stream);

int bear_dm_prior_wide_f64(bear_ws *ws, const uint32_t *counts, const double *prior, uint64_t n_rows, int width,
                           const double *h_signed_dev, double eps, int train_ar, double *out, double *grad_prior, void *stream);
int bear_eval_wide_f64(bear_ws *ws, const uint32_t *test, const uint32_t *train, const double *prior, uint64_t n_rows, int width,
                       const double *h, int n_h, int with_ar, const double *van_reg, int n_van, double eps,
                       uint64_t noise_seed, uint64_t row_base, double *out, void *stream);

int bear_dm_ref_wide_f64(bear_ws *ws, const uint32_t *train, const uint32_t *ref, uint64_t n_rows, int width, double h_signed,
                         double tau_signed, double nu_signed, double eps, int train_ar, double *out, void *stream);
int bear_ref_train_reduce_wide_f64(bear_ws *ws, const uint32_t *train, const uint32_t *ref, uint64_t n_rows, int width,
                                   const double *theta, double eps, int train_ar, double *packed, void *stream);
int bear_ref_train_step_wide_f64(bear_ws *ws, const uint32_t *train, const uint32_t *ref, uint64_t n_rows, int width, double *theta,
                                 double *adam_m, double *adam_v, double *adam_t, double eps, int train_ar, double learning_rate,
                                 double scale, double *out, double *loss_buf, uint64_t loss_cap, void *stream);
int bear_dm_refmix_wide_grad_f64(bear_ws *ws, const uint32_t *counts, const double *net_rows, const uint32_t *ref, uint64_t n_rows,
                                 int width, const double *h_signed_dev, const double *tau_signed_dev, const double *net_weight_signed_dev,
                                 double eps, int train_ar, double *out, double *grad_net_rows, void *stream);

typedef struct bear_eval_plan bear_eval_plan;
int bear_eval_plan_create(bear_ws *ws, const uint32_t *test, const uint32_t *train, uint64_t n_rows, bear_eval_plan **out, void *stream);
int bear_eval_plan_destroy(bear_eval_plan *plan);
uint64_t bear_eval_plan_bytes(const bear_eval_plan *plan);
int bear_eval_plan_f64(bear_ws *ws, const bear_eval_plan *plan, const uint32_t *test, const uint32_t *train, const double *prior,
                       uint64_t n_rows, const double *h, int n_h, int with_ar, const double *van_reg, int n_van, double eps,
                       uint64_t noise_seed, uint64_t row_base, const uint32_t *row_ids, double *out, void *stream);

int bear_bmm_f64(bear_ws *ws, const uint32_t *counts, uint64_t n_rows, const double *alpha, int n_alpha, double *out,
                 void *stream);

int bear_dm_items_f64(bear_ws *ws, const double *x, const uint32_t *c, uint64_t n, int path, double *D,
                      double *P, void *stream);

int bear_log_gamma_f64(const double *conc, uint64_t n, uint64_t n_samples, uint64_t seed, double *out, void *stream);
int bear_logdir_sample_f64(const uint32_t *counts, const double *prior, uint64_t n_rows, const double *h, int n_h,
                           int with_ar, const double *van, int n_van, int mc_samples, int map, uint64_t seed,
                           uint64_t row_base, double *out, void *stream);
int bear_logdir_sample_wide_f64(const uint32_t *counts, const double *prior, uint64_t n_rows, int width, const double *h,
                                int n_h, int with_ar, const double *van, int n_van, int mc_samples, int map, uint64_t seed,
                                uint64_t row_base, double *out, void *stream);

int bear_synth_counts_u32(uint64_t seed, uint64_t row0, uint64_t n_rows, int dense, uint32_t *train,
                          uint32_t *test, uint32_t *ref, void *stream);
int bear_stream_read(bear_ws *ws, const void *src, uint64_t n_bytes, void *stream);
int bear_synth_prior_f64(uint64_t seed, uint64_t row0, uint64_t n_rows, double *prior, void *stream);

int bear_count_rows(const char *path, uint64_t *n_rows_out);
int bear_count_newlines(const char *path, uint64_t *n_out);
int bear_parse_sparse_counts(const char *path, int num_ds, int width, int lag, uint64_t skip_lines, uint64_t max_rows,
                             char *kmers, uint32_t *counts, uint64_t *n_rows_out);
int bear_parse_counts_tsv(const char *path, int num_ds, int lag, uint64_t max_rows, char *kmers,
                          uint32_t *counts, uint64_t *n_rows_out);
int bear_shard_rows_count(uint64_t row_base, uint64_t file_rows, uint64_t total_rows, uint64_t batch_rows, int rank, int world,
                          uint64_t *n_local_out);
int bear_parse_counts_tsv_shard(const char *path, int num_ds, int lag, uint64_t skip_lines, uint64_t row_base, uint64_t total_rows,
                                uint64_t batch_rows, int rank, int world, uint64_t max_rows, char *kmers, uint32_t *counts,
                                uint64_t *n_local_out, uint64_t *n_file_rows_out);
int bear_parse_counts_tsv_wide(const char *path, int num_ds, int width, int lag, uint64_t max_rows, char *kmers, uint32_t *counts,
                               uint64_t *n_rows_out);
int bear_parse_counts_tsv_shard_wide(const char *path, int num_ds, int width, int lag, uint64_t skip_lines, uint64_t row_base,
                                     uint64_t total_rows, uint64_t batch_rows, int rank, int world, uint64_t max_rows, char *kmers,
                                     uint32_t *counts, uint64_t *n_local_out, uint64_t *n_file_rows_out);

int bear_stat_source(const char *path, uint64_t *size_out, int64_t *mtime_ns_out);
int bear_cache_write(const char *path, const char *kmers, const uint32_t *counts, uint64_t n_rows, int lag, int num_ds,
                     uint64_t src_size, int64_t src_mtime_ns);
int bear_cache_info(const char *path, uint64_t *n_rows, int *lag, int *num_ds, uint64_t *src_size, int64_t *src_mtime_ns);
int bear_cache_read(const char *path, uint64_t row0, uint64_t n_rows, char *kmers, uint32_t *counts);

int bear_shuffle_rows(const void *src, void *dst, uint64_t n_rows, uint32_t row_bytes, uint64_t seed, void *stream);
uint64_t bear_shuffle_source_row(uint64_t i, uint64_t n_rows, uint64_t seed);

int bear_kmer_order_u64(const uint64_t *kmer_code, uint64_t n_rows, int lag, uint32_t *perm, void *scratch, uint64_t *scratch_bytes,
                        void *stream);
int bear_gather_rows(const void *src, const uint32_t *perm, void *dst, uint64_t n_rows, uint32_t row_bytes, void *stream);

int bear_fastx_size(const char *path, int fastq, int reverse, uint64_t *n_pos_out, uint64_t *n_seqs_out);
int bear_fastx_encode(const char *path, int fastq, int reverse, int group, uint64_t capacity, uint8_t *text,
                      uint8_t *group_out, uint64_t *n_pos_out);
typedef struct bear_kmer_sort bear_kmer_sort;
int bear_kmer_sort_create(const uint8_t *text, const uint8_t *group, uint64_t n_pos, int lag, bear_kmer_sort **out,
                          uint64_t *n_rows_out, void *stream);
int bear_kmer_sort_reduce(const bear_kmer_sort *h, int n_groups, uint8_t *kmers, uint64_t *kmer_code, uint32_t *counts,
                          void *stream);
int bear_kmer_sort_destroy(bear_kmer_sort *h);
int bear_count_last_hip_error(void);
int bear_write_counts_tsv(const char *path, const char *kmers, const uint32_t *counts, uint64_t n_rows, int lag, int num_ds,
                          uint64_t row_begin, uint64_t row_step, int append);
int bear_fastx_size_wide(const char *path, int fastq, int reverse, int width, uint64_t *n_pos_out, uint64_t *n_seqs_out);
int bear_fastx_encode_wide(const char *path, int fastq, int reverse, int width, int group, uint64_t capacity, uint8_t *text,
                           uint8_t *group_out, uint64_t *n_pos_out);
int bear_kmer_sort_create_wide(const uint8_t *text, const uint8_t *group, uint64_t n_pos, int lag, int width, bear_kmer_sort **out,
                               uint64_t *n_rows_out, void *stream);
int bear_write_counts_tsv_wide(const char *path, const char *kmers, const uint32_t *counts, uint64_t n_rows, int lag, int num_ds,
                               int width, uint64_t row_begin, uint64_t row_step, int append);

#ifdef __cplusplus
}
#endif
#endif
```

Baseline: 139.6 billion.

## Parallelize plan construction: prefix-scan cut, hierarchical chain, fused fill/live kernel

Rewrites the plan-creation pipeline. Tile cutting now uses a block prefix scan with binary search, a set-level composition and expansion around the serial chain, and a per-tile starts/write/sizes/offsets sequence. The fill and live kernels are fused into one launch with a new in-block classification sort. Scratch buffers are merged into a single allocation, host syncs and memsets are cut down, and a stream readback API is added. These changes speed up plan building, but the measured metric is the marginal+grad throughput, which probably reuses a prebuilt plan, so the timed path may not change.

```diff
diff --git a/bear_amd/csrc/bear_hip.hip b/bear_amd/csrc/bear_hip.hip
--- a/bear_amd/csrc/bear_hip.hip
+++ b/bear_amd/csrc/bear_hip.hip
@@ -242,8 +242,9 @@
   p->ncol = ncol;
   p->n_rows = n_rows;
   p->counts = counts;
-  hipError_t e = hipMalloc(&p->hist, sizeof(unsigned long long) * (2 * SRT_NKEY + PLN_NBIG + 1));
-  if (e == hipSuccess) e = hipMemset(p->hist, 0, sizeof(unsigned long long) * (2 * SRT_NKEY + PLN_NBIG + 1));
+  constexpr size_t HIST_N = 2 * SRT_NKEY + PLN_NBIG + 1;
+  hipError_t e = hipMalloc(&p->hist, sizeof(unsigned long long) * (HIST_N + 3));
+  if (e == hipSuccess) e = hipMemset(p->hist, 0, sizeof(unsigned long long) * (HIST_N + 3));
   if (e != hipSuccess) {
     g_last_hip_error = (int)e;
     plan_free(p);
@@ -254,24 +255,57 @@
     return BEAR_OK;
   }
   const uint64_t n_quads = (n_rows + PLN_QUAD - 1) / PLN_QUAD;
-  uint8_t *d_quad = nullptr, *h_quad = nullptr;
-  unsigned long long *d_cnt = nullptr;
+  const char *cut_env = getenv("BEAR_PLAN_CUT");
+  const bool host_cut = cut_env && cut_env[0] == 'h';
+  const uint32_t chunk = plan_cut_chunk(n_quads);
+  const uint64_t n_chunks = (n_quads + chunk - 1) / chunk, n_sets = (n_chunks + PLN_CUT_SET - 1) / PLN_CUT_SET;
+  size_t scratch_bytes = 0;
+  auto take = [&scratch_bytes](size_t bytes) {
+    const size_t o = scratch_bytes;
+    scratch_bytes += (bytes + 255) & ~(size_t)255;
+    return o;
+  };
+  const size_t o_cnt = take(sizeof(unsigned long long) * 12);
+  const size_t o_quad = take(3 * n_quads);
+  const size_t o_step = host_cut ? 0 : take(sizeof(uint16_t) * n_quads);
+  const size_t o_walk = host_cut ? 0 : take(sizeof(uint32_t) * n_chunks * PLN_CUT_SPAN);
+  const size_t o_entry = host_cut ? 0 : take(sizeof(uint64_t) * 2 * n_chunks);
+  const size_t o_swalk = host_cut ? 0 : take(sizeof(uint2) * n_sets * PLN_CUT_SPAN);
+  const size_t o_sentry = host_cut ? 0 : take(sizeof(uint64_t) * 2 * n_sets);
+  const size_t o_sums = host_cut ? 0 : take(sizeof(unsigned long long) * (n_quads / 256 + 1));
+  unsigned char *scratch = nullptr;
+  uint8_t *h_quad = nullptr;
   std::vector<pln_tile> tiles;
-  e = hipMalloc(&d_quad, 3 * n_quads);
-  if (e == hipSuccess) e = hipMalloc(&d_cnt, sizeof(unsigned long long) * 9);
-  if (e == hipSuccess) e = hipMemset(d_cnt, 0, sizeof(unsigned long long) * 9);
+  e = hipMalloc(&scratch, scratch_bytes);
+  unsigned long long *d_cnt = reinterpret_cast<unsigned long long *>(scratch + o_cnt), *d_meta = d_cnt + 9;
+  uint8_t *d_quad = scratch + o_quad;
+  uint16_t *d_step = reinterpret_cast<uint16_t *>(scratch + o_step);
+  uint32_t *d_walk = reinterpret_cast<uint32_t *>(scratch + o_walk);
+  uint64_t *d_entry = reinterpret_cast<uint64_t *>(scratch + o_entry);
+  uint2 *d_swalk = reinterpret_cast<uint2 *>(scratch + o_swalk);
+  uint64_t *d_sentry = reinterpret_cast<uint64_t *>(scratch + o_sentry);
+  unsigned long long *d_sums = reinterpret_cast<unsigned long long *>(scratch + o_sums);
+  if (e == hipSuccess) e = hipMemset(d_cnt, 0, sizeof(unsigned long long) * 12);
   if (e == hipSuccess) {
     const int grid = grid_capped((n_quads + 255) / 256, (uint64_t)ws->num_cu * 8);
     hipLaunchKernelGGL(plan_scan_kernel, dim3(grid), dim3(256), 0, 0, counts, n_rows, ncol, d_quad, d_cnt, p->hist);
     e = hipGetLastError();
   }
-  unsigned long long h_cnt[3] = {0, 0, 0}, h_total[3] = {0, 0, 0};
-  if (e == hipSuccess) e = hipMemcpy(h_cnt, d_cnt, sizeof(h_cnt), hipMemcpyDeviceToHost);
-  if (e == hipSuccess) e = hipMemcpy(h_total, d_cnt + 6, sizeof(h_total), hipMemcpyDeviceToHost);
+  if (e == hipSuccess && !host_cut) {
+    const uint64_t wb = (n_chunks * PLN_CUT_SPAN + 255) / 256, sb = (n_sets * PLN_CUT_SPAN + 255) / 256;
+    hipLaunchKernelGGL(plan_cut_step_kernel, dim3((unsigned)((n_quads + PLN_CUT_SEG - 1) / PLN_CUT_SEG)), dim3(256), 0, 0, d_quad, n_quads, d_step);
+    hipLaunchKernelGGL(plan_cut_walk_kernel, dim3((unsigned)wb), dim3(256), 0, 0, d_step, n_quads, n_chunks, chunk, d_walk);
+    hipLaunchKernelGGL(plan_cut_compose_kernel, dim3((unsigned)sb), dim3(256), 0, 0, d_walk, n_chunks, n_sets, d_swalk);
+    hipLaunchKernelGGL(plan_cut_chain_kernel, dim3(1), dim3(1), 0, 0, d_swalk, n_sets, d_sentry, d_sentry + n_sets, d_meta);
+    hipLaunchKernelGGL(plan_cut_expand_kernel, dim3((unsigned)((n_sets + 63) / 64)), dim3(64), 0, 0, d_walk, n_chunks, n_sets, chunk, d_sentry,
+                       d_sentry + n_sets, d_entry, d_entry + n_chunks);
+    e = hipGetLastError();
+  }
+  unsigned long long h_all[12] = {0, 0, 0, 0, 0, 0, 0, 0, 0, 0, 0, 0};
+  if (e == hipSuccess) e = hipMemcpy(h_all, d_cnt, sizeof(h_all), hipMemcpyDeviceToHost);
+  const unsigned long long *h_cnt = h_all, *h_total = h_all + 6;
   for (int k = 0; k < 3; ++k) p->count_total[k] = p->count_bound[k] = (double)h_total[k];
   uint64_t off16 = 0, n_tiles = 0;
-  const char *cut_env = getenv("BEAR_PLAN_CUT");
-  const bool host_cut = cut_env && cut_env[0] == 'h';
   if (e == hipSuccess && host_cut) {
     h_quad = (uint8_t *)malloc(3 * n_quads);
     if (!h_quad) e = hipErrorOutOfMemory;
@@ -309,76 +343,46 @@
     n_tiles = tiles.size();
   }
   free(h_quad);
+  if (!host_cut) n_tiles = h_all[9];
+  if (e == hipSuccess) e = hipMalloc(&p->tiles, sizeof(pln_tile) * (n_tiles + PLN_DESC_PAD));
+  if (e == hipSuccess) e = hipMemset(p->tiles, 0, sizeof(pln_tile) * (n_tiles + PLN_DESC_PAD));
+  if (e == hipSuccess && host_cut) e = hipMemcpy(p->tiles, tiles.data(), sizeof(pln_tile) * tiles.size(), hipMemcpyHostToDevice);
   if (e == hipSuccess && !host_cut) {
-    const uint32_t chunk = plan_cut_chunk(n_quads);
-    const uint64_t n_chunks = (n_quads + chunk - 1) / chunk;
-    uint32_t *d_walk = nullptr;
-    uint16_t *d_step = nullptr;
-    uint64_t *d_entry = nullptr;
-    unsigned long long *d_meta = nullptr, h_meta[3] = {0, 0, 0};
-    e = hipMalloc(&d_walk, sizeof(uint32_t) * n_chunks * PLN_CUT_SPAN);
-    if (e == hipSuccess) e = hipMalloc(&d_step, sizeof(uint16_t) * n_quads);
-    if (e == hipSuccess) e = hipMalloc(&d_entry, sizeof(uint64_t) * 2 * n_chunks);
-    if (e == hipSuccess) e = hipMalloc(&d_meta, sizeof(h_meta));
-    if (e == hipSuccess) e = hipMemset(d_meta, 0, sizeof(h_meta));
-    if (e == hipSuccess) {
-      const uint64_t wb = (n_chunks * PLN_CUT_SPAN + 255) / 256;
-      hipLaunchKernelGGL(plan_cut_step_kernel, dim3((unsigned)((n_chunks + 255) / 256)), dim3(256), 0, 0, d_quad, n_quads, n_chunks, chunk, d_step);
-      hipLaunchKernelGGL(plan_cut_walk_kernel, dim3((unsigned)wb), dim3(256), 0, 0, d_step, n_quads, n_chunks, chunk, d_walk);
-      hipLaunchKernelGGL(plan_cut_chain_kernel, dim3(1), dim3(1), 0, 0, d_walk, n_chunks, chunk, d_entry, d_entry + n_chunks, d_meta);
-      e = hipGetLastError();
-    }
-    if (e == hipSuccess) e = hipMemcpy(h_meta, d_meta, sizeof(unsigned long long), hipMemcpyDeviceToHost);
-    n_tiles = h_meta[0];
-    if (e == hipSuccess) e = hipMalloc(&p->tiles, sizeof(pln_tile) * (n_tiles + PLN_DESC_PAD));
-    if (e == hipSuccess) e = hipMemset(p->tiles, 0, sizeof(pln_tile) * (n_tiles + PLN_DESC_PAD));
-    if (e == hipSuccess) {
-      hipLaunchKernelGGL(plan_cut_write_kernel, dim3((unsigned)((n_chunks + 255) / 256)), dim3(256), 0, 0, d_quad, n_quads, n_rows, ncol,
-                         n_chunks, chunk, d_entry, d_entry + n_chunks, p->tiles);
-      hipLaunchKernelGGL(plan_cut_offsets_kernel, dim3(1), dim3(1024), 0, 0, p->tiles, n_tiles, d_meta);
-      e = hipGetLastError();
-    }
+    unsigned long long h_meta[3] = {0, 0, 0};
+    hipLaunchKernelGGL(plan_cut_starts_kernel, dim3((unsigned)((n_chunks + 255) / 256)), dim3(256), 0, 0, d_step, n_quads, n_chunks, chunk,
+                       d_entry, d_entry + n_chunks, n_tiles, p->tiles);
+    hipLaunchKernelGGL(plan_cut_write_kernel, dim3((unsigned)((n_tiles + 3) / 4)), dim3(256), 0, 0, d_quad, d_step, n_quads, n_rows, ncol,
+                       n_tiles, p->tiles);
+    hipLaunchKernelGGL(plan_cut_sizes_kernel, dim3((unsigned)((n_tiles + 255) / 256)), dim3(256), 0, 0, p->tiles, n_tiles, d_sums);
+    hipLaunchKernelGGL(plan_cut_offsets_kernel, dim3((unsigned)((n_tiles + 255) / 256)), dim3(256), 0, 0, p->tiles, n_tiles, d_sums, d_meta);
+    e = hipGetLastError();
     if (e == hipSuccess) e = hipMemcpy(h_meta, d_meta, sizeof(h_meta), hipMemcpyDeviceToHost);
     if (e == hipSuccess && h_meta[2]) e = hipErrorOutOfMemory;
     off16 = h_meta[1];
-    (void)hipFree(d_walk);
-    (void)hipFree(d_step);
-    (void)hipFree(d_entry);
-    (void)hipFree(d_meta);
-  }
-  (void)hipFree(d_quad);
+  }
+  (void)hipFree(scratch);
   p->n_tiles = n_tiles;
   const uint64_t stream_bytes = off16 * 16 + 1024;
+  p->stream_len = off16 * 16;
   for (int k = 0; k < 3; ++k) p->n_heavy[k] = h_cnt[k];
-  if (host_cut) {
-    if (e == hipSuccess) e = hipMalloc(&p->tiles, sizeof(pln_tile) * (tiles.size() + PLN_DESC_PAD));
-    if (e == hipSuccess) e = hipMemset(p->tiles, 0, sizeof(pln_tile) * (tiles.size() + PLN_DESC_PAD));
-    if (e == hipSuccess) e = hipMemcpy(p->tiles, tiles.data(), sizeof(pln_tile) * tiles.size(), hipMemcpyHostToDevice);
-  }
+  unsigned long long *d_cursors = p->hist + HIST_N;
   if (e == hipSuccess) e = hipMalloc(&p->stream, stream_bytes);
-  if (e == hipSuccess) e = hipMemset(p->stream, 0, stream_bytes);
+  if (e == hipSuccess) e = hipMemset(p->stream + p->stream_len, 0, stream_bytes - p->stream_len);
   if (e == hipSuccess && h_cnt[0]) e = hipMalloc(&p->heavy_col, sizeof(pln_heavy_col) * h_cnt[0]);
   if (e == hipSuccess && h_cnt[1]) e = hipMalloc(&p->heavy_row, sizeof(pln_heavy_row) * h_cnt[1]);
   if (e == hipSuccess && h_cnt[2]) e = hipMalloc(&p->heavy_stop, sizeof(uint64_t) * h_cnt[2]);
-  if (e == hipSuccess) {
-    const uint64_t nt = n_tiles;
-    const int grid = grid_capped(nt, (uint64_t)ws->num_cu * 2);
-    hipLaunchKernelGGL(plan_fill_kernel, dim3(grid), dim3(1024), 0, 0, counts, n_rows, ncol, p->tiles, nt, p->stream,
-                       p->heavy_col, p->heavy_row, p->heavy_stop, d_cnt + 3);
-    e = hipGetLastError();
-  }
   const uint64_t live_bytes = ncol == 5 ? sizeof(uint16_t) * PLN_LIVE_STRIDE * (n_tiles + 1) : 0;
   if (e == hipSuccess && live_bytes) e = hipMalloc(&p->live, live_bytes);
-  if (e == hipSuccess && live_bytes) e = hipMemset(p->live, 0, live_bytes);
-  if (e == hipSuccess && live_bytes) {
-    const uint64_t nt = n_tiles;
-    const int grid = grid_capped(nt, (uint64_t)ws->num_cu * 2);
-    hipLaunchKernelGGL(plan_live_kernel, dim3(grid), dim3(1024), 0, 0, p->tiles, nt, p->stream, p->live);
+  if (e == hipSuccess && live_bytes) e = hipMemset(p->live + PLN_LIVE_STRIDE * n_tiles, 0, sizeof(uint16_t) * PLN_LIVE_STRIDE);
+  if (e == hipSuccess && n_tiles) {
+    const int grid = grid_capped((n_tiles + 3) / 4, (uint64_t)ws->num_cu * PLN_FILL_BLOCKS_PER_CU);
+    hipLaunchKernelGGL(plan_fill_kernel, dim3(grid), dim3(PLN_FILL_THREADS), 0, 0, counts, n_rows, ncol, p->tiles, n_tiles, p->stream, p->live,
+                       p->heavy_col, p->heavy_row, p->heavy_stop, d_cursors);
     e = hipGetLastError();
   }
-  if (e == hipSuccess) e = hipDeviceSynchronize();
-  unsigned long long h_used[3] = {0, 0, 0};
-  if (e == hipSuccess) e = hipMemcpy(h_used, d_cnt + 3, sizeof(h_used), hipMemcpyDeviceToHost);
+  std::vector<unsigned long long> h_hist(HIST_N + 3, 0ull);
+  if (e == hipSuccess) e = hipMemcpy(h_hist.data(), p->hist, sizeof(unsigned long long) * (HIST_N + 3), hipMemcpyDeviceToHost);
+  const unsigned long long *h_used = h_hist.data() + HIST_N;
   for (int k = 0; k < 3; ++k) p->n_heavy[k] = h_used[k];
 #ifdef BEAR_DET_BUILD
   const uint64_t sort_from = 2;
@@ -393,13 +397,10 @@
   }
   p->n_live_rows = n_rows;
   if (e == hipSuccess && ncol == 5) {
-    unsigned long long h_hist[SRT_NKEY];
-    e = hipMemcpy(h_hist, p->hist, sizeof(h_hist), hipMemcpyDeviceToHost);
     unsigned long long live_rows = h_cnt[1];
     for (int k = 0; k < SRT_NKEY; ++k) live_rows += h_hist[k];
     p->n_live_rows = live_rows;
   }
-  (void)hipFree(d_cnt);
   if (e != hipSuccess) {
     g_last_hip_error = (int)e;
     plan_free(p);
@@ -443,6 +444,7 @@
   p->heavy_stop = nullptr;
   p->live = nullptr;
   p->n_tiles = 0;
+  p->stream_len = 0;
   p->n_heavy[0] = p->n_heavy[1] = p->n_heavy[2] = 0;
   p->ncol = PLAN_ROWS;
   p->bytes = sizeof(unsigned long long) * (2 * SRT_NKEY + PLN_NBIG + 1);
@@ -484,6 +486,21 @@
     rows[k] = h[k].rows_items >> 16;
     items[k] = h[k].rows_items & 0xffffu;
     stream_offset[k] = (uint64_t)h[k].off16 * 16;
+  }
+  return BEAR_OK;
+}
+
+int bear_plan_read_stream(const bear_plan *plan, uint64_t offset, uint64_t bytes, void *dst_host) {
+  if (!plan || offset > plan->stream_len || bytes > plan->stream_len - offset || (bytes && !dst_host)) return BEAR_ERR_INVALID_ARG;
+  if (!bytes) return BEAR_OK;
+  int prev = 0;
+  (void)hipGetDevice(&prev);
+  (void)hipSetDevice(plan->device);
+  const hipError_t e = hipMemcpy(dst_host, plan->stream + offset, bytes, hipMemcpyDeviceToHost);
+  (void)hipSetDevice(prev);
+  if (e != hipSuccess) {
+    g_last_hip_error = (int)e;
+    return BEAR_ERR_HIP;
   }
   return BEAR_OK;
 }
diff --git a/bear_amd/csrc/bear_host.h b/bear_amd/csrc/bear_host.h
--- a/bear_amd/csrc/bear_host.h
+++ b/bear_amd/csrc/bear_host.h
@@ -145,6 +145,7 @@
   unsigned long long *hist;
   uint16_t *live;
   uint64_t n_tiles;
+  uint64_t stream_len;
   uint64_t n_heavy[3];
   int rows_ref;
   uint64_t n_live_rows;
diff --git a/bear_amd/csrc/kernels_plan.h b/bear_amd/csrc/kernels_plan.h
--- a/bear_amd/csrc/kernels_plan.h
+++ b/bear_amd/csrc/kernels_plan.h
@@ -73,42 +73,65 @@
 #define PLN_CUT_CHUNK_MAX 8192
 static inline uint32_t plan_cut_chunk(uint64_t n_quads) { return n_quads <= 50000000ull ? 2048u : (uint32_t)PLN_CUT_CHUNK_MAX; }
 #define PLN_CUT_SPAN (PLN_RMAX / PLN_QUAD)
-
-__device__ __forceinline__ uint64_t plan_cut_one(const uint8_t *__restrict__ quad, uint64_t n_quads, uint64_t q0, uint32_t *items,
-                                                 uint32_t *hcol, uint32_t *hrow) {
-  uint32_t it = 0, hc = 0, hr = 0, rows = 0;
-  uint64_t q = q0;
-  while (q < n_quads && rows + PLN_QUAD <= PLN_RMAX && it + quad[q] <= PLN_NI_CUT) {
-    it += quad[q];
-    if (hcol) {
-      hc += quad[n_quads + q];
-      hr += quad[2 * n_quads + q];
-    }
-    rows += PLN_QUAD;
-    ++q;
-  }
-  *items = it;
-  if (hcol) {
-    *hcol = hc;
-    *hrow = hr;
-  }
-  return q;
-}
-__global__ __launch_bounds__(256) void plan_cut_step_kernel(const uint8_t *__restrict__ quad, uint64_t n_quads, uint64_t n_chunks,
-                                                            uint32_t chunk, uint16_t *__restrict__ step) {
-  const uint64_t k = (uint64_t)blockIdx.x * 256 + threadIdx.x;
-  if (k >= n_chunks) return;
-  const uint64_t q0 = k * chunk, q_end = q0 + chunk < n_quads ? q0 + chunk : n_quads;
-  uint64_t r = q0;
-  uint32_t items = 0;
-  for (uint64_t q = q0; q < q_end; ++q) {
-    if (r < q) {
-      r = q;
-      items = 0;
-    }
-    while (r < n_quads && (uint32_t)(r - q + 1) * PLN_QUAD <= PLN_RMAX && items + quad[r] <= PLN_NI_CUT) items += quad[r++];
-    step[q] = (uint16_t)(r - q);
-    items -= quad[q];
+#define PLN_CUT_SET 64
+#define PLN_CUT_SEG 2048
+#define PLN_CUT_PER ((PLN_CUT_SEG + PLN_CUT_SPAN + 256) / 256)
+
+template <int NW>
+__device__ __forceinline__ uint32_t plan_block_scan(uint32_t v, uint32_t *part, uint32_t *total) {
+  const int lane = threadIdx.x & 63, wave = threadIdx.x >> 6;
+  uint32_t incl = v;
+#pragma unroll
+  for (int off = 1; off < 64; off <<= 1) {
+    const uint32_t o = (uint32_t)__shfl_up((int)incl, off, 64);
+    if (lane >= off) incl += o;
+  }
+  __syncthreads();
+  if (lane == 63) part[wave] = incl;
+  __syncthreads();
+  uint32_t before = 0, all = 0;
+#pragma unroll
+  for (int w = 0; w < NW; ++w) {
+    const uint32_t s = part[w];
+    before += w < wave ? s : 0u;
+    all += s;
+  }
+  *total = all;
+  return before + incl - v;
+}
+
+__global__ __launch_bounds__(256) void plan_cut_step_kernel(const uint8_t *__restrict__ quad, uint64_t n_quads, uint16_t *__restrict__ step) {
+  __shared__ uint32_t P[256 * PLN_CUT_PER + 1];
+  __shared__ uint32_t part[4];
+  static_assert(256 * PLN_CUT_PER >= PLN_CUT_SEG + PLN_CUT_SPAN && PLN_QUAD * 5 <= PLN_NI_CUT, "prefix window; a tile holds a group");
+  const uint32_t tid = threadIdx.x;
+  const uint64_t q0 = (uint64_t)blockIdx.x * PLN_CUT_SEG;
+  uint32_t v[PLN_CUT_PER], sum = 0;
+#pragma unroll
+  for (int j = 0; j < PLN_CUT_PER; ++j) {
+    const uint64_t q = q0 + (uint64_t)tid * PLN_CUT_PER + j;
+    v[j] = q < n_quads ? (uint32_t)quad[q] : 0u;
+    sum += v[j];
+  }
+  uint32_t total;
+  uint32_t run = plan_block_scan<4>(sum, part, &total);
+#pragma unroll
+  for (int j = 0; j < PLN_CUT_PER; ++j) {
+    P[tid * PLN_CUT_PER + j] = run;
+    run += v[j];
+  }
+  if (tid == 255) P[256 * PLN_CUT_PER] = run;
+  __syncthreads();
+  for (uint32_t l = tid; l < PLN_CUT_SEG && q0 + l < n_quads; l += 256) {
+    const uint64_t left = n_quads - (q0 + l);
+    const uint32_t smax = left < PLN_CUT_SPAN ? (uint32_t)left : (uint32_t)PLN_CUT_SPAN, base = P[l];
+    uint32_t lo = 1, hi = smax;
+    while (lo < hi) {
+      const uint32_t mid = (lo + hi + 1) >> 1;
+      if (P[l + mid] - base <= PLN_NI_CUT) lo = mid;
+      else hi = mid - 1;
+    }
+    step[q0 + l] = (uint16_t)lo;
   }
 }
 __global__ __launch_bounds__(256) void plan_cut_walk_kernel(const uint16_t *__restrict__ step, uint64_t n_quads, uint64_t n_chunks,
@@ -125,178 +148,229 @@
   walk[id] = (uint32_t)(q >= end ? q - end : 0) | (cnt << 16);
 }
 static_assert(PLN_CUT_CHUNK_MAX < 65536 && PLN_CUT_SPAN < 65536 && PLN_CUT_SPAN <= 2048, "walk table: 16-bit fields; a tile is shorter than a chunk");
-__global__ void plan_cut_chain_kernel(const uint32_t *__restrict__ walk, uint64_t n_chunks, uint32_t chunk, uint64_t *__restrict__ entry,
-                                      uint64_t *__restrict__ base, unsigned long long *__restrict__ meta) {
+__global__ __launch_bounds__(256) void plan_cut_compose_kernel(const uint32_t *__restrict__ walk, uint64_t n_chunks, uint64_t n_sets,
+                                                               uint2 *__restrict__ swalk) {
+  const uint64_t id = (uint64_t)blockIdx.x * 256 + threadIdx.x;
+  if (id >= n_sets * PLN_CUT_SPAN) return;
+  const uint64_t g = id / PLN_CUT_SPAN, k1 = (g + 1) * PLN_CUT_SET < n_chunks ? (g + 1) * PLN_CUT_SET : n_chunks;
+  uint32_t j = (uint32_t)(id - g * PLN_CUT_SPAN), tiles = 0;
+  for (uint64_t k = g * PLN_CUT_SET; k < k1; ++k) {
+    const uint32_t w = walk[k * PLN_CUT_SPAN + j];
+    tiles += w >> 16;
+    j = w & 0xffffu;
+  }
+  swalk[id] = make_uint2(j, tiles);
+}
+__global__ void plan_cut_chain_kernel(const uint2 *__restrict__ swalk, uint64_t n_sets, uint64_t *__restrict__ sentry,
+                                      uint64_t *__restrict__ sbase, unsigned long long *__restrict__ meta) {
   if (blockIdx.x || threadIdx.x) return;
   uint64_t j = 0, tiles = 0;
-  for (uint64_t k = 0; k < n_chunks; ++k) {
+  for (uint64_t g = 0; g < n_sets; ++g) {
+    sentry[g] = j;
+    sbase[g] = tiles;
+    const uint2 w = swalk[g * PLN_CUT_SPAN + j];
+    tiles += w.y;
+    j = w.x;
+  }
+  meta[0] = tiles;
+}
+__global__ __launch_bounds__(64) void plan_cut_expand_kernel(const uint32_t *__restrict__ walk, uint64_t n_chunks, uint64_t n_sets, uint32_t chunk,
+                                                             const uint64_t *__restrict__ sentry, const uint64_t *__restrict__ sbase,
+                                                             uint64_t *__restrict__ entry, uint64_t *__restrict__ base) {
+  const uint64_t g = (uint64_t)blockIdx.x * 64 + threadIdx.x;
+  if (g >= n_sets) return;
+  const uint64_t k1 = (g + 1) * PLN_CUT_SET < n_chunks ? (g + 1) * PLN_CUT_SET : n_chunks;
+  uint64_t j = sentry[g], tiles = sbase[g];
+  for (uint64_t k = g * PLN_CUT_SET; k < k1; ++k) {
     entry[k] = k * chunk + j;
     base[k] = tiles;
     const uint32_t w = walk[k * PLN_CUT_SPAN + j];
     tiles += w >> 16;
     j = w & 0xffffu;
   }
-  meta[0] = tiles;
-}
-__global__ __launch_bounds__(256) void plan_cut_write_kernel(const uint8_t *__restrict__ quad, uint64_t n_quads, uint64_t n_rows, int ncol,
-                                                             uint64_t n_chunks, uint32_t chunk, const uint64_t *__restrict__ entry,
-                                                             const uint64_t *__restrict__ base, pln_tile *__restrict__ tiles) {
+}
+__global__ __launch_bounds__(256) void plan_cut_starts_kernel(const uint16_t *__restrict__ step, uint64_t n_quads, uint64_t n_chunks,
+                                                              uint32_t chunk, const uint64_t *__restrict__ entry,
+                                                              const uint64_t *__restrict__ base, uint64_t n_tiles, pln_tile *__restrict__ tiles) {
   const uint64_t k = (uint64_t)blockIdx.x * 256 + threadIdx.x;
   if (k >= n_chunks) return;
   const uint64_t end = (k + 1) * chunk;
   uint64_t q = entry[k], t = base[k];
-  while (q < end && q < n_quads) {
-    uint32_t items, hcol, hrow;
-    const uint64_t q1 = plan_cut_one(quad, n_quads, q, &items, &hcol, &hrow);
-    pln_tile ti;
-    ti.row0 = q * PLN_QUAD;
-    uint32_t rows = (uint32_t)(q1 - q) * PLN_QUAD;
-    if (ti.row0 + rows > n_rows) rows = (uint32_t)(n_rows - ti.row0);
-    const uint32_t hc = hcol < PLN_HCAP ? hcol : PLN_HCAP;
-    const uint32_t hr = ncol == 5 ? (hrow < PLN_HCAP ? hrow : PLN_HCAP) : 0u;
-    ti.rows_items = (rows << 16) | items;
-    ti.off16 = 0;
-    ti.hc_hr = (hc << 16) | hr;
-    ti.blk16 = pln_block_layout(rows, items, hc, hr).end / 16;
-    ti.pad = 0;
-    tiles[t++] = ti;
-    q = q1;
-  }
-}
-__global__ __launch_bounds__(1024) void plan_cut_offsets_kernel(pln_tile *__restrict__ tiles, uint64_t n_tiles,
-                                                                unsigned long long *__restrict__ meta) {
-  __shared__ unsigned long long part[1024];
-  const uint64_t per = (n_tiles + 1023) / 1024, lo = per * threadIdx.x, hi = lo + per < n_tiles ? lo + per : n_tiles;
-  unsigned long long s = 0;
-  for (uint64_t t = lo; t < hi; ++t) s += tiles[t].blk16;
-  part[threadIdx.x] = s;
-  __syncthreads();
-  if (threadIdx.x == 0) {
-    unsigned long long run = 0;
-    for (int k = 0; k < 1024; ++k) {
-      const unsigned long long v = part[k];
-      part[k] = run;
-      run += v;
-    }
-    meta[1] = run;
-    meta[2] = run > 0xffffffffull ? 1ull : 0ull;
-  }
-  __syncthreads();
-  unsigned long long off = part[threadIdx.x];
-  for (uint64_t t = lo; t < hi; ++t) {
-    tiles[t].off16 = (uint32_t)off;
-    off += tiles[t].blk16;
-  }
-}
-
-__global__ __launch_bounds__(1024) void plan_fill_kernel(const uint32_t *__restrict__ counts, uint64_t n_rows, int ncol,
-                                                         const pln_tile *__restrict__ tiles, uint64_t n_tiles,
-                                                         unsigned char *__restrict__ stream,
-                                                         pln_heavy_col *__restrict__ heavy_col,
-                                                         pln_heavy_row *__restrict__ heavy_row,
-                                                         uint64_t *__restrict__ heavy_stop,
-                                                         unsigned long long *__restrict__ cursors) {
-  constexpr int RPT = (PLN_RMAX + 1023) / 1024;
-  __shared__ uint32_t hist[SRT_NHIST];
-  __shared__ uint32_t offs[SRT_NHIST];
-  __shared__ uint32_t scan[16];
-  __shared__ uint16_t sorted[PLN_NI + 64];
-  __shared__ uint32_t s_hc, s_hr;
-#ifdef BEAR_DET_BUILD
+  while (q < end && q < n_quads && t < n_tiles) {
+    tiles[t++].row0 = q * PLN_QUAD;
+    q += step[q];
+  }
+}
+__global__ __launch_bounds__(256) void plan_cut_write_kernel(const uint8_t *__restrict__ quad, const uint16_t *__restrict__ step, uint64_t n_quads,
+                                                             uint64_t n_rows, int ncol, uint64_t n_tiles, pln_tile *__restrict__ tiles) {
+  const uint64_t t = (uint64_t)blockIdx.x * 4 + (threadIdx.x >> 6);
+  const uint32_t lane = threadIdx.x & 63;
+  if (t >= n_tiles) return;
+  const uint64_t row0 = tiles[t].row0, q = row0 / PLN_QUAD;
+  const uint32_t len = step[q];
+  uint32_t items = 0, hcol = 0, hrow = 0;
+  for (uint32_t i = lane; i < len; i += 64) {
+    items += quad[q + i];
+    hcol += quad[n_quads + q + i];
+    hrow += quad[2 * n_quads + q + i];
+  }
+#pragma unroll
+  for (int off = 32; off > 0; off >>= 1) {
+    items += (uint32_t)__shfl_xor((int)items, off, 64);
+    hcol += (uint32_t)__shfl_xor((int)hcol, off, 64);
+    hrow += (uint32_t)__shfl_xor((int)hrow, off, 64);
+  }
+  if (lane) return;
+  pln_tile ti;
+  ti.row0 = row0;
+  uint32_t rows = len * PLN_QUAD;
+  if (row0 + rows > n_rows) rows = (uint32_t)(n_rows - row0);
+  const uint32_t hc = hcol < PLN_HCAP ? hcol : PLN_HCAP;
+  const uint32_t hr = ncol == 5 ? (hrow < PLN_HCAP ? hrow : PLN_HCAP) : 0u;
+  ti.rows_items = (rows << 16) | items;
+  ti.off16 = 0;
+  ti.hc_hr = (hc << 16) | hr;
+  ti.blk16 = pln_block_layout(rows, items, hc, hr).end / 16;
+  ti.pad = 0;
+  tiles[t] = ti;
+}
+__device__ __forceinline__ unsigned long long plan_block_sum64(unsigned long long v, unsigned long long *part4) {
+#pragma unroll
+  for (int off = 32; off > 0; off >>= 1) v += __shfl_xor(v, off, 64);
+  __syncthreads();
+  if ((threadIdx.x & 63) == 0) part4[threadIdx.x >> 6] = v;
+  __syncthreads();
+  return part4[0] + part4[1] + part4[2] + part4[3];
+}
+__global__ __launch_bounds__(256) void plan_cut_sizes_kernel(const pln_tile *__restrict__ tiles, uint64_t n_tiles, unsigned long long *__restrict__ sums) {
+  __shared__ unsigned long long part4[4];
+  const uint64_t t = (uint64_t)blockIdx.x * 256 + threadIdx.x;
+  const unsigned long long s = plan_block_sum64(t < n_tiles ? tiles[t].blk16 : 0u, part4);
+  if (threadIdx.x == 0) sums[blockIdx.x] = s;
+}
+__global__ __launch_bounds__(256) void plan_cut_offsets_kernel(pln_tile *__restrict__ tiles, uint64_t n_tiles, const unsigned long long *__restrict__ sums,
+                                                               unsigned long long *__restrict__ meta) {
+  __shared__ unsigned long long part4[4];
+  __shared__ uint32_t part[4];
+  unsigned long long before = 0;
+  for (uint32_t b = threadIdx.x; b < blockIdx.x; b += 256) before += sums[b];
+  before = plan_block_sum64(before, part4);
+  const uint64_t t = (uint64_t)blockIdx.x * 256 + threadIdx.x;
+  const uint32_t mine = t < n_tiles ? tiles[t].blk16 : 0u;
+  uint32_t total;
+  const uint32_t excl = plan_block_scan<4>(mine, part, &total);
+  if (t < n_tiles) tiles[t].off16 = (uint32_t)(before + excl);
+  if (blockIdx.x == gridDim.x - 1 && threadIdx.x == 0) {
+    meta[1] = before + total;
+    meta[2] = before + total > 0xffffffffull ? 1ull : 0ull;
+  }
+}
+
+#define PLN_FILL_THREADS 256
+#define PLN_FILL_WAVES (PLN_FILL_THREADS / 64)
+#define PLN_FILL_RPT ((PLN_RMAX + PLN_FILL_THREADS - 1) / PLN_FILL_THREADS)
+#define PLN_FILL_VEC ((PLN_RMAX * 20 / 16 + PLN_FILL_THREADS - 1) / PLN_FILL_THREADS)
+#define PLN_FILL_IPT (PLN_NI / PLN_FILL_THREADS)
+#define PLN_FILL_NCLS (SRT_CL * PLN_FILL_IPT * PLN_FILL_WAVES)
+#define PLN_FILL_CPT ((PLN_FILL_NCLS + PLN_FILL_THREADS - 1) / PLN_FILL_THREADS)
+#define PLN_FILL_BLOCKS_PER_CU 3
+
+__global__ __launch_bounds__(PLN_FILL_THREADS, PLN_FILL_BLOCKS_PER_CU) void plan_fill_kernel(const uint32_t *__restrict__ counts, uint64_t n_rows, int ncol,
+                                                                     const pln_tile *__restrict__ tiles, uint64_t n_tiles,
+                                                                     unsigned char *__restrict__ stream,
+                                                                     uint16_t *__restrict__ live,
+                                                                     pln_heavy_col *__restrict__ heavy_col,
+                                                                     pln_heavy_row *__restrict__ heavy_row,
+                                                                     uint64_t *__restrict__ heavy_stop,
+                                                                     unsigned long long *__restrict__ cursors) {
+  constexpr int RPT = PLN_FILL_RPT, IPT = PLN_FILL_IPT, NW = PLN_FILL_WAVES;
+  static_assert((PLN_RMAX * 20) % 16 == 0 && PLN_RMAX % 16 == 0 && PLN_NI % PLN_FILL_THREADS == 0 && PLN_NI % 64 == 0, "whole pieces");
+  static_assert(PLN_RMAX * 5 * 4 >= (PLN_NI + 64) * 2, "the sorted list reuses the rows' LDS");
+  static_assert(PLN_NI < 65536 && PLN_RMAX * 5 < 65536 && PLN_RMAX + 1 <= PLN_LIVE_STRIDE, "16-bit fields of the scans and the item list");
+  __shared__ __attribute__((aligned(16))) uint32_t raw[PLN_RMAX * 5];
   __shared__ uint32_t comp[PLN_NI];
-  static_assert((PLN_NI & (PLN_NI - 1)) == 0 && PLN_NI <= 2048, "bitonic sort over the tile's items: PLN_NI / 2 pairs, at most one per thread");
-  __shared__ unsigned long long hkey[PLN_HCAP], htmp[PLN_HCAP];
-#endif
-  const uint32_t tid = threadIdx.x, rep = tid & (SRT_REP - 1);
-  for (uint64_t t = blockIdx.x; t < n_tiles; t += gridDim.x) {
-    const pln_tile ti = tiles[t];
-    const uint32_t rows = ti.rows_items >> 16, n_light = ti.rows_items & 0xffffu;
-    const uint32_t hc_cap = ti.hc_hr >> 16, hr_cap = ti.hc_hr & 0xffffu;
+  __shared__ __attribute__((aligned(16))) uint16_t s_live[PLN_LIVE_STRIDE];
+  static_assert((PLN_LIVE_STRIDE * 2) % 16 == 0, "a slot of the live lists in 16-byte pieces");
+  __shared__ __attribute__((aligned(16))) uint8_t s_nrow[PLN_RMAX];
+  __shared__ uint32_t cls[PLN_FILL_CPT * PLN_FILL_THREADS];
+  __shared__ uint32_t part[3][NW];
+  uint16_t *sorted = reinterpret_cast<uint16_t *>(raw);
+  const uint32_t tid = threadIdx.x, lane = tid & 63, wave = tid >> 6;
+  uint64_t t = blockIdx.x;
+  if (t >= n_tiles) return;
+  const __attribute__((address_space(4))) pln_tile *tc = (const __attribute__((address_space(4))) pln_tile *)(uintptr_t)tiles;
+  for (; t < n_tiles; t += gridDim.x) {
+    const uint64_t row0 = tc[t].row0;
+    const uint32_t rows_items = tc[t].rows_items, hc_hr = tc[t].hc_hr, off16 = tc[t].off16;
+    const uint32_t rows = rows_items >> 16, n_light = rows_items & 0xffffu;
+    const uint32_t hc_cap = hc_hr >> 16, hr_cap = hc_hr & 0xffffu;
     const pln_layout L = pln_block_layout(rows, n_light, hc_cap, hr_cap);
-    unsigned char *blk = stream + (size_t)ti.off16 * 16;
+    unsigned char *blk = stream + (size_t)off16 * 16;
     uint16_t *E = reinterpret_cast<uint16_t *>(blk);
-    uint8_t *nrow = blk + L.nrow;
-    uint16_t *items = reinterpret_cast<uint16_t *>(blk + L.items);
     uint16_t *hoff = reinterpret_cast<uint16_t *>(blk + L.hoff);
     uint32_t *hcnt = reinterpret_cast<uint32_t *>(blk + L.hcnt);
     uint16_t *hrow = reinterpret_cast<uint16_t *>(blk + L.hrow);
     double *hn = reinterpret_cast<double *>(blk + L.hn);
-    if (tid < SRT_NHIST) hist[tid] = 0;
-    if (tid == 0) {
-      s_hc = 0;
-      s_hr = 0;
+    {
+      const uint32_t nvec = (rows * 20u) >> 4, ndw = rows * 5u;
+      const uint4 *src = reinterpret_cast<const uint4 *>(counts + row0 * 5);
+      uint4 pre[PLN_FILL_VEC];
+#pragma unroll
+      for (int v = 0; v < PLN_FILL_VEC; ++v) {
+        const uint32_t i = tid + PLN_FILL_THREADS * v;
+        pre[v] = i < nvec ? src[i] : make_uint4(0u, 0u, 0u, 0u);
+      }
+#pragma unroll
+      for (int v = 0; v < PLN_FILL_VEC; ++v) {
+        const uint32_t i = tid + PLN_FILL_THREADS * v;
+        if (i < nvec) reinterpret_cast<uint4 *>(raw)[i] = pre[v];
+      }
+      for (uint32_t d = nvec * 4u + tid; d < ndw; d += PLN_FILL_THREADS) raw[d] = counts[row0 * 5 + d];
+#pragma unroll
+      for (int j = 0; j < PLN_FILL_CPT; ++j) cls[tid + PLN_FILL_THREADS * j] = 0;
     }
     __syncthreads();
-#ifdef BEAR_DET_BUILD
-    uint32_t det_hc[RPT], det_hr[RPT];
+    uint32_t n_it = 0, n_hc = 0, n_hr = 0, n_live = 0;
+#pragma unroll
+    for (int k = 0; k < RPT; ++k) {
+      const uint32_t lr = tid * RPT + k;
+      uint32_t ntot = 0;
+#pragma unroll
+      for (int b = 0; b < 5; ++b) {
+        const uint32_t cb = lr < rows ? raw[lr * 5 + b] : 0u;
+        ntot += cb < SRT_CL + 1u ? cb : SRT_CL + 1u;
+        const uint32_t cv = (b < 4 || ncol == 5) ? cb : 0u;
+        n_it += cv - 1u < (uint32_t)SRT_CL ? 1u : 0u;
+        n_hc += cv > SRT_CL ? 1u : 0u;
+      }
+      n_hr += ntot > SRT_CL ? 1u : 0u;
+      n_live += ntot != 0u ? 1u : 0u;
+      if (lr < PLN_RMAX) s_nrow[lr] = ntot > SRT_CL ? (uint8_t)255 : (uint8_t)ntot;
+    }
+    uint32_t tot_a, tot_b;
+    const uint32_t ex_a = plan_block_scan<NW>(n_it | (n_hr << 16), part[0], &tot_a);
+    const uint32_t ex_b = plan_block_scan<NW>(n_hc | (n_live << 16), part[1], &tot_b);
     {
-      uint32_t base_c = 0, base_r = 0;
-#pragma unroll
-      for (int k = 0; k < RPT; ++k) {
-        const uint32_t lr = tid + 1024u * k;
-        uint32_t nc = 0, nr = 0;
-        if (lr < rows) {
+      uint32_t pos = ex_a & 0xffffu, hr_pos = ex_a >> 16, hc_pos = ex_b & 0xffffu, live_pos = 1u + (ex_b >> 16);
+      const uint32_t n_live_all = tot_b >> 16;
+      if (tid == 0) s_live[0] = (uint16_t)n_live_all;
+      for (uint32_t i = 1u + n_live_all + tid; i < PLN_LIVE_STRIDE; i += PLN_FILL_THREADS) s_live[i] = 0;
+      const uint32_t lr_end = tid * RPT + RPT < rows ? tid * RPT + RPT : rows;
+#pragma unroll 1
+      for (uint32_t lr = tid * RPT; lr < lr_end; ++lr) {
+        uint32_t c[5], ntot = 0;
+#pragma unroll
+        for (int b = 0; b < 5; ++b) {
+          c[b] = raw[lr * 5 + b];
+          ntot += c[b] < SRT_CL + 1u ? c[b] : SRT_CL + 1u;
+        }
+        if (ntot != 0u) s_live[live_pos++] = (uint16_t)lr;
+        if (ntot > SRT_CL) {
+          const uint64_t r = row0 + lr;
           double n = 0.0;
-          for (int b = 0; b < 5; ++b) {
-            const uint32_t cv = counts[(ti.row0 + lr) * 5 + b];
-            n += (double)cv;
-            nc += (b < ncol && cv > SRT_CL) ? 1u : 0u;
-          }
-          nr = n > (double)SRT_CL ? 1u : 0u;
-        }
-        const uint32_t packed = nc | (nr << 16);
-        const int lane = tid & 63, wave = tid >> 6;
-        uint32_t incl = packed;
-#pragma unroll
-        for (int off = 1; off < 64; off <<= 1) {
-          const uint32_t o = (uint32_t)__shfl_up((int)incl, off, 64);
-          if (lane >= off) incl += o;
-        }
-        __syncthreads();
-        if (lane == 63) scan[wave] = incl;
-        __syncthreads();
-        uint32_t before = 0, total = 0;
-        for (int w = 0; w < 16; ++w) {
-          if (w < wave) before += scan[w];
-          total += scan[w];
-        }
-        const uint32_t excl = before + incl - packed;
-        det_hc[k] = base_c + (excl & 0xffffu);
-        det_hr[k] = base_r + (excl >> 16);
-        base_c += total & 0xffffu;
-        base_r += total >> 16;
-      }
-      __syncthreads();
-      if (tid == 0) {
-        s_hc = base_c;
-        s_hr = base_r;
-      }
-    }
-#endif
-    uint32_t c[RPT][5], rank[RPT][5];
-#pragma unroll
-    for (int k = 0; k < RPT; ++k) {
-      const uint32_t lr = tid + 1024u * k;
-#pragma unroll
-      for (int b = 0; b < 5; ++b) {
-        c[k][b] = 0;
-        rank[k][b] = 0;
-      }
-      if (lr < rows) {
-        const uint64_t r = ti.row0 + lr;
-        double n = 0.0;
-#pragma unroll
-        for (int b = 0; b < 5; ++b) {
-          c[k][b] = counts[r * 5 + b];
-          n += (double)c[k][b];
-        }
-        nrow[lr] = n < 1.0 ? (uint8_t)0 : (n <= (double)SRT_CL ? (uint8_t)n : (uint8_t)255);
-        if (n > (double)SRT_CL) {
-#ifdef BEAR_DET_BUILD
-          const uint32_t k2 = hr_cap ? det_hr[k] : 0xffffffffu;
-#else
-          const uint32_t k2 = hr_cap ? atomicAdd(&s_hr, 1u) : 0xffffffffu;
-#endif
+#pragma unroll
+          for (int b = 0; b < 5; ++b) n += (double)c[b];
+          const uint32_t k2 = hr_pos++;
           if (k2 < hr_cap) {
             hrow[k2] = (uint16_t)lr;
             hn[k2] = n;
@@ -305,150 +379,89 @@
             heavy_row[q].row = r;
             heavy_row[q].n = n;
           }
+          if (ncol == 4 && c[4] > SRT_CL) heavy_stop[atomicAdd(&cursors[2], 1ull)] = c[4];
+#pragma unroll
+          for (int b = 0; b < 5; ++b) {
+            if ((b < 4 || ncol == 5) && c[b] > SRT_CL) {
+              const uint32_t k3 = hc_pos++;
+              if (k3 < hc_cap) {
+                hoff[k3] = (uint16_t)(lr * 5 + b);
+                hcnt[k3] = c[b];
+              } else {
+                const unsigned long long q = atomicAdd(&cursors[0], 1ull);
+                heavy_col[q].off = r * 5 + b;
+                heavy_col[q].c = c[b];
+              }
+            }
+          }
         }
-        if (ncol == 4 && c[k][4] > SRT_CL) heavy_stop[atomicAdd(&cursors[2], 1ull)] = c[k][4];
-#pragma unroll
-        for (int b = 0; b < 5; ++b) {
-          if (b >= ncol) c[k][b] = 0;
-          if (c[k][b] > SRT_CL) {
-#ifdef BEAR_DET_BUILD
-            const uint32_t k2 = hc_cap ? det_hc[k]++ : 0xffffffffu;
-#else
-            const uint32_t k2 = hc_cap ? atomicAdd(&s_hc, 1u) : 0xffffffffu;
-#endif
-            if (k2 < hc_cap) {
-              hoff[k2] = (uint16_t)(lr * 5 + b);
-              hcnt[k2] = c[k][b];
-            } else {
-              const unsigned long long q = atomicAdd(&cursors[0], 1ull);
-              heavy_col[q].off = r * 5 + b;
-              heavy_col[q].c = c[k][b];
-            }
-            c[k][b] = 0;
-          }
-          if (c[k][b] != 0) rank[k][b] = atomicAdd(&hist[(c[k][b] - 1) * SRT_REP + rep], 1u);
-        }
-      } else if (lr < ((rows + 15u) & ~15u)) {
-        nrow[lr] = 0;
+#pragma unroll
+        for (int b = 0; b < 5; ++b)
+          if ((b < 4 || ncol == 5) && c[b] - 1u < (uint32_t)SRT_CL && pos < PLN_NI)
+            comp[pos++] = (c[b] << 16) | (lr * 5 + b);
+      }
+      if (tid < 8) {
+        if (hc_cap + tid < ((hc_cap + 7u) & ~7u)) hoff[hc_cap + tid] = 0;
+        if (hc_cap + tid < ((hc_cap + 3u) & ~3u)) hcnt[hc_cap + tid] = 0u;
+        if (hr_cap + tid < ((hr_cap + 7u) & ~7u)) hrow[hr_cap + tid] = 0;
+        if (hr_cap + tid < ((hr_cap + 1u) & ~1u)) hn[hr_cap + tid] = 0.0;
+      }
+    }
+    __syncthreads();
+    uint32_t ent[IPT];
+    static_assert(SRT_CL < 256, "a count in eight bits");
+#pragma unroll
+    for (int j = 0; j < IPT; ++j) {
+      const uint32_t idx = (uint32_t)j * PLN_FILL_THREADS + tid;
+      ent[j] = idx < n_light ? comp[idx] : 0u;
+      const uint32_t cc = ent[j] >> 16;
+      unsigned long long rem = __builtin_amdgcn_ballot_w64(cc != 0u);
+      while (rem) {
+        const uint32_t cl = (uint32_t)__builtin_amdgcn_readlane((int)cc, __builtin_ctzll(rem));
+        const unsigned long long m = __builtin_amdgcn_ballot_w64(cc == cl);
+        if (cc == cl) ent[j] |= __builtin_amdgcn_mbcnt_hi((uint32_t)(m >> 32), __builtin_amdgcn_mbcnt_lo((uint32_t)m, 0u)) << 24;
+        if (lane == 0) cls[((cl - 1u) * IPT + (uint32_t)j) * NW + wave] = (uint32_t)__builtin_popcountll(m);
+        rem &= ~m;
       }
     }
     __syncthreads();
     {
-      const uint32_t v = tid < SRT_NHIST ? hist[tid] : 0u;
-      const int lane = tid & 63, wave = tid >> 6;
-      uint32_t incl = v;
-#pragma unroll
-      for (int off = 1; off < 64; off <<= 1) {
-        uint32_t o = (uint32_t)__shfl_up((int)incl, off, 64);
-        if (lane >= off) incl += o;
-      }
-      if (lane == 63) scan[wave] = incl;
-      __syncthreads();
-      uint32_t base = 0;
-      for (int w = 0; w < wave; ++w) base += scan[w];
-      if (tid < SRT_NHIST) offs[tid] = base + incl - v;
+      uint32_t v[PLN_FILL_CPT], sum = 0, total;
+#pragma unroll
+      for (int j = 0; j < PLN_FILL_CPT; ++j) {
+        v[j] = cls[tid * PLN_FILL_CPT + j];
+        sum += v[j];
+      }
+      uint32_t run = plan_block_scan<NW>(sum, part[2], &total);
+#pragma unroll
+      for (int j = 0; j < PLN_FILL_CPT; ++j) {
+        cls[tid * PLN_FILL_CPT + j] = run;
+        run += v[j];
+      }
     }
     __syncthreads();
-    if (tid < 30) E[tid] = (uint16_t)(tid < SRT_CL ? offs[tid * SRT_REP] : n_light);
+    if (tid < 30) E[tid] = (uint16_t)(tid < SRT_CL ? cls[tid * IPT * NW] : n_light);
     if (tid == 30) E[30] = (uint16_t)hc_cap;
     if (tid == 31) E[31] = (uint16_t)hr_cap;
 #pragma unroll
-    for (int k = 0; k < RPT; ++k)
-#pragma unroll
-      for (int b = 0; b < 5; ++b)
-        if (c[k][b] != 0) sorted[offs[(c[k][b] - 1) * SRT_REP + rep] + rank[k][b]] = (uint16_t)((tid + 1024u * k) * 5 + b);
+    for (int j = 0; j < IPT; ++j) {
+      const uint32_t cc = (ent[j] >> 16) & 0xffu;
+      if (cc) sorted[cls[((cc - 1u) * IPT + (uint32_t)j) * NW + wave] + (ent[j] >> 24)] = (uint16_t)(ent[j] & 0xffffu);
+    }
+    const uint32_t padded = (n_light + 63u) & ~63u;
+    if (tid < 64 && n_light + tid < padded) sorted[n_light + tid] = (uint16_t)PLN_SENTINEL;
     __syncthreads();
-#ifdef BEAR_DET_BUILD
     {
-      for (uint32_t i = tid; i < PLN_NI; i += 1024) {
-        uint32_t key = 0;
-        for (uint32_t q = 1; q < SRT_CL; ++q) key += offs[q * SRT_REP] <= i ? 1u : 0u;
-        comp[i] = i < n_light ? (key << 16) | sorted[i] : 0xffffffffu;
-      }
-      __syncthreads();
-      for (uint32_t size = 2; size <= PLN_NI; size <<= 1)
-        for (uint32_t stride = size >> 1; stride > 0; stride >>= 1) {
-          const uint32_t lo = 2u * tid - (tid & (stride - 1u)), hi = lo + stride;
-          if (tid < PLN_NI / 2) {
-            const bool up = (lo & size) == 0u;
-            const uint32_t a = comp[lo], bq = comp[hi];
-            if ((a > bq) == up) {
-              comp[lo] = bq;
-              comp[hi] = a;
-            }
-          }
-          __syncthreads();
-        }
-      for (uint32_t i = tid; i < n_light; i += 1024) sorted[i] = (uint16_t)(comp[i] & 0xffffu);
-      __syncthreads();
-      const uint32_t nhc = s_hc < hc_cap ? s_hc : hc_cap, nhr = s_hr < hr_cap ? s_hr : hr_cap;
-      if (tid < nhc) hkey[tid] = ((unsigned long long)hoff[tid] << 32) | hcnt[tid];
-      __syncthreads();
-      if (tid < nhc) {
-        uint32_t r = 0;
-        for (uint32_t q = 0; q < nhc; ++q) r += hkey[q] < hkey[tid] ? 1u : 0u;
-        htmp[r] = hkey[tid];
-      }
-      __syncthreads();
-      if (tid < nhc) {
-        hoff[tid] = (uint16_t)(htmp[tid] >> 32);
-        hcnt[tid] = (uint32_t)htmp[tid];
-      }
-      __syncthreads();
-      if (tid < nhr) hkey[tid] = ((unsigned long long)hrow[tid] << 48) | tid;
-      if (tid < nhr) htmp[tid] = (unsigned long long)__double_as_longlong(hn[tid]);
-      __syncthreads();
-      uint32_t r = 0;
-      unsigned long long mine = 0ull, myn = 0ull;
-      if (tid < nhr) {
-        for (uint32_t q = 0; q < nhr; ++q) r += hkey[q] < hkey[tid] ? 1u : 0u;
-        mine = hkey[tid];
-        myn = htmp[tid];
-      }
-      __syncthreads();
-      if (tid < nhr) {
-        hrow[r] = (uint16_t)(mine >> 48);
-        hn[r] = __longlong_as_double((long long)myn);
-      }
-      __syncthreads();
-    }
-#endif
-    const uint32_t padded = (n_light + 63u) & ~63u;
-    for (uint32_t i = tid; i < padded; i += 1024) items[i] = i < n_light ? sorted[i] : (uint16_t)PLN_SENTINEL;
-    __syncthreads();
-  }
-}
-
-__global__ __launch_bounds__(1024) void plan_live_kernel(const pln_tile *__restrict__ tiles, uint64_t n_tiles,
-                                                         const unsigned char *__restrict__ stream, uint16_t *__restrict__ live) {
-  constexpr int RPT = (PLN_RMAX + 1023) / 1024;
-  __shared__ uint32_t cnt[RPT * 16];
-  const uint32_t tid = threadIdx.x, lane = tid & 63, wave = tid >> 6;
-  for (uint64_t t = blockIdx.x; t < n_tiles; t += gridDim.x) {
-    const pln_tile ti = tiles[t];
-    const uint32_t rows = ti.rows_items >> 16;
-    const uint8_t *nrow = stream + (size_t)ti.off16 * 16 + 64;
-    uint16_t *out = live + t * PLN_LIVE_STRIDE;
-    unsigned long long mask[RPT];
-#pragma unroll
-    for (int k = 0; k < RPT; ++k) {
-      const uint32_t lr = tid + 1024u * k;
-      mask[k] = __builtin_amdgcn_ballot_w64(lr < rows && nrow[lr] != 0);
-      if (lane == 0) cnt[k * 16 + wave] = (uint32_t)__builtin_popcountll(mask[k]);
-    }
-    __syncthreads();
-    uint32_t total = 0;
-#pragma unroll
-    for (int k = 0; k < RPT; ++k) {
-      uint32_t base = total;
-      for (int w = 0; w < 16; ++w) {
-        const uint32_t c = cnt[k * 16 + w];
-        if (w < (int)wave) base += c;
-        total += c;
-      }
-      if ((mask[k] >> lane) & 1ull) out[1 + base + (uint32_t)__builtin_popcountll(mask[k] & ((1ull << lane) - 1ull))] = (uint16_t)(tid + 1024u * k);
-    }
-    if (tid == 0) out[0] = (uint16_t)total;
+      uint4 *dst = reinterpret_cast<uint4 *>(blk + L.items);
+      const uint4 *src = reinterpret_cast<const uint4 *>(sorted);
+      for (uint32_t i = tid; i < padded / 8u; i += PLN_FILL_THREADS) dst[i] = src[i];
+      uint4 *ndst = reinterpret_cast<uint4 *>(blk + L.nrow);
+      if (tid < ((rows + 15u) >> 4)) ndst[tid] = reinterpret_cast<const uint4 *>(s_nrow)[tid];
+      if (live) {
+        uint4 *ldst = reinterpret_cast<uint4 *>(live + t * PLN_LIVE_STRIDE);
+        for (uint32_t i = tid; i < PLN_LIVE_STRIDE * 2u / 16u; i += PLN_FILL_THREADS) ldst[i] = reinterpret_cast<const uint4 *>(s_live)[i];
+      }
+    }
     __syncthreads();
   }
 }
diff --git a/bear_amd/kernels.py b/bear_amd/kernels.py
--- a/bear_amd/kernels.py
+++ b/bear_amd/kernels.py
@@ -301,6 +301,28 @@
         _lib.call("bear_plan_tile_info", self._h, 0, n, row0.ctypes.data, rows.ctypes.data, items.ctypes.data, off.ctypes.data)
         return row0, rows, items, off
 
+    def stream_bytes(self):
+        _, rows, items, off = self.tiles()
+        if len(off) == 0:
+            return np.empty(0, np.uint8)
+        head = np.empty(32, np.uint16)
+        _lib.call("bear_plan_read_stream", self._h, int(off[-1]), 64, head.ctypes.data)
+        total = int(off[-1]) + plan_block_layout(int(rows[-1]), int(items[-1]), int(head[30]), int(head[31]))["end"]
+        out = np.empty(total, np.uint8)
+        _lib.call("bear_plan_read_stream", self._h, 0, total, out.ctypes.data)
+        return out
+
+
+def plan_block_layout(rows, n_light, hc, hr):
+    L = {"nrow": 64}
+    L["items"] = L["nrow"] + ((rows + 15) & ~15)
+    L["hoff"] = L["items"] + ((n_light + 63) & ~63) * 2
+    L["hcnt"] = L["hoff"] + ((hc + 7) & ~7) * 2
+    L["hrow"] = L["hcnt"] + ((hc + 3) & ~3) * 4
+    L["hn"] = L["hrow"] + ((hr + 7) & ~7) * 2
+    L["end"] = L["hn"] + ((hr + 1) & ~1) * 8
+    return L
+
 
 def _check_planned(plan, ncol, rows, dtype, name):
     if plan.ncol != ncol:
diff --git a/include/bear_hip.h b/include/bear_hip.h
--- a/include/bear_hip.h
+++ b/include/bear_hip.h
@@ -46,6 +46,7 @@
 uint64_t bear_plan_tile_count(const bear_plan *plan);
 int bear_plan_tile_info(const bear_plan *plan, uint64_t first, uint64_t count, uint64_t *row0, uint32_t *rows, uint32_t *items,
                         uint64_t *stream_offset);
+int bear_plan_read_stream(const bear_plan *plan, uint64_t offset, uint64_t bytes, void *dst_host);
 int bear_plan_create_ref(bear_ws *ws, const uint32_t *train, const uint32_t *ref, uint64_t n_rows, bear_plan **out);
 int bear_dm_prior_plan_f64(bear_ws *ws, const bear_plan *plan, const uint32_t *counts, const double *prior,
                            uint64_t n_rows, double h_signed, double eps, int train_ar, int prior_normalized,
```

Result: no change. 139.6 billion (median of 2 runs) (+0.0%).
